# Algy/fast-slic

Measured on AMD Instinct MI355X. Metric: megapixels/sec @10 iters (1280x720 & 4K, K=1600); % HBM roofline, higher is better.
Workload: dtype u8/u16/i32 (integer SLIC); 1 GPU; 1280x720 RGB, K=1600, 10 iters (configs[1]), 8 frames/GPU; frames_per_gpu=8, global_frames=8, slots_per_gpu=6, submissions_per_launch_group=up to 2 (dynamic batching of the pipeline), inputs=device-resident uint8 RGB, device int16 labels, parallelism=frames sharded across GPUs, no collective

## Files before the change

### fast_slic_amd/_binding.py

```python
import ctypes as C
import os
import subprocess
import threading

import numpy as np

ARCH_NAME = "hip/gfx950"
_HERE = os.path.dirname(os.path.abspath(__file__))
_LIB_PATH = os.path.join(_HERE, "libfslic_hip.so")

CLUSTER_DTYPE = np.dtype([
    ("y", "<f4"), ("x", "<f4"), ("r", "<f4"), ("g", "<f4"), ("b", "<f4"), ("a", "<f4"),
    ("number", "<u2"), ("is_active", "u1"), ("is_updatable", "u1"), ("num_members", "<u4"),
])
assert CLUSTER_DTYPE.itemsize == 32

FSLIC_OK, FSLIC_E_INVALID, FSLIC_E_UNSUPPORTED, FSLIC_E_HIP, FSLIC_E_INTERNAL = range(5)


class Params(C.Structure):
    _fields_ = [
        ("max_iter", C.c_int32), ("compactness", C.c_float), ("min_size_factor", C.c_float),
        ("subsample_stride", C.c_int32), ("convert_to_lab", C.c_int32),
        ("manhattan_spatial_dist", C.c_int32), ("preemptive", C.c_int32),
        ("preemptive_thres", C.c_float), ("num_threads", C.c_int32), ("debug_mode", C.c_int32),
        ("abi", C.c_int32), ("variant", C.c_int32), ("reserved", C.c_int32 * 4),
    ]


EXPORTS = [
    "fslic_hip_device_count", "fslic_hip_create", "fslic_hip_destroy", "fslic_hip_initialize_clusters",
    "fslic_hip_iterate", "fslic_hip_iterate_device", "fslic_hip_iterate_batch", "fslic_hip_submit_group",
    "fslic_hip_wait_group", "fslic_hip_rgb_to_lab",
    "fslic_hip_enforce_connectivity", "fslic_hip_enforce_connectivity_nodes", "fslic_hip_last_prelabels", "fslic_hip_last_timing_report",
    "fslic_hip_last_device_times", "fslic_hip_set_launch_timing", "fslic_hip_last_assign_loop", "fslic_hip_last_group_frames", "fslic_hip_last_path", "fslic_hip_last_launch_mode", "fslic_hip_group_done", "fslic_hip_last_error", "fslic_hip_version",
    "fslic_hip_get_connectivity", "fslic_hip_knn_connectivity", "fslic_hip_get_mask_density", "fslic_hip_cluster_density_to_mask",
    "fslic_hip_pipeline_submit", "fslic_hip_pipeline_drain", "fslic_hip_pipeline_batching", "fslic_hip_last_host_topk_frames",
    "fslic_hip_separate_pass_redos", "fslic_hip_copy_bandwidth", "fslic_hip_last_recorder_report",
    "fslic_hip_crf_new", "fslic_hip_crf_free", "fslic_hip_crf_copy", "fslic_hip_crf_get_params", "fslic_hip_crf_set_params",
    "fslic_hip_crf_set_compat", "fslic_hip_crf_get_compat", "fslic_hip_crf_num_classes", "fslic_hip_crf_first_time",
    "fslic_hip_crf_last_time", "fslic_hip_crf_num_frames", "fslic_hip_crf_pop_frame", "fslic_hip_crf_push_frame", "fslic_hip_crf_frame",
    "fslic_hip_crf_frame_time", "fslic_hip_crf_frame_set_clusters", "fslic_hip_crf_frame_get_clusters",
    "fslic_hip_crf_frame_set_connectivity", "fslic_hip_crf_frame_set_connectivity_csr", "fslic_hip_crf_frame_get_connectivity",
    "fslic_hip_crf_frame_set_mask", "fslic_hip_crf_frame_set_proba", "fslic_hip_crf_frame_set_unbiased", "fslic_hip_crf_frame_set_unary",
    "fslic_hip_crf_frame_get_unary", "fslic_hip_crf_frame_spatial_energy", "fslic_hip_crf_frame_temporal_energy",
    "fslic_hip_crf_frame_get_inferred", "fslic_hip_crf_frame_reset_inferred", "fslic_hip_crf_initialize", "fslic_hip_crf_inference",
    "fslic_hip_crf_expf_host", "fslic_hip_crf_expf_device",
    "fslic_hip_pool_workspace_size", "fslic_hip_pool", "fslic_hip_pool_finalize", "fslic_hip_unpool",
    "fslic_hip_rag_workspace_size", "fslic_hip_rag_accumulate", "fslic_hip_rag_compact",
    "fslic_hip_crf_tensor_workspace_size", "fslic_hip_crf_tensor_inference",
    "fslic_hip_crf_tensor_grad_workspace_size", "fslic_hip_crf_tensor_inference_saved", "fslic_hip_crf_tensor_backward",
]

_lib = None
_lib_lock = threading.Lock()


def build_library(force=False):
    csrc = os.path.join(_HERE, "csrc")
    args = ["make", "-s", "-C", csrc]
    if force:
        args.append("-B")
    subprocess.check_call(args)
    return _LIB_PATH


def _preload_torch_hip_runtime():
    import importlib.util
    import sys
    if "torch" in sys.modules:
        return
    try:
        spec = importlib.util.find_spec("torch")
    except (ImportError, ValueError):
        spec = None
    if spec is None or not spec.origin:
        return
    cand = os.path.join(os.path.dirname(spec.origin), "lib", "libamdhip64.so")
    if os.path.exists(cand):
        try:
            C.CDLL(cand, mode=C.RTLD_GLOBAL)
        except OSError:
            pass


def load_library():
    global _lib
    with _lib_lock:
        if _lib is not None:
            return _lib
        _preload_torch_hip_runtime()
        if not os.path.exists(_LIB_PATH):
            raise ImportError(
                "fast_slic_amd: %s is missing; build it with `python -c 'import __graft_entry__ as g; g.build()'` "
                "or `make -C fast_slic_amd/csrc` (there is no CPU fallback)" % _LIB_PATH)
        lib = C.CDLL(os.environ.get("FSLIC_LIB") or _LIB_PATH)
        vp, i32 = C.c_void_p, C.c_int
        lib.fslic_hip_device_count.restype = i32
        lib.fslic_hip_create.argtypes = [i32, i32, C.POINTER(vp)]
        lib.fslic_hip_destroy.argtypes = [vp]
        lib.fslic_hip_destroy.restype = None
        lib.fslic_hip_initialize_clusters.argtypes = [i32, i32, i32, vp, vp]
        lib.fslic_hip_iterate.argtypes = [vp, C.POINTER(Params), i32, i32, i32, vp, vp, vp]
        lib.fslic_hip_iterate_device.argtypes = [vp, i32, C.POINTER(Params), i32, i32, i32, vp, vp, vp]
        lib.fslic_hip_iterate_batch.argtypes = [vp, C.POINTER(Params), i32, i32, i32, i32, vp, vp, vp, i32]
        lib.fslic_hip_submit_group.argtypes = [vp, i32, C.POINTER(Params), i32, i32, i32, i32, vp, vp, vp]
        lib.fslic_hip_wait_group.argtypes = [vp, i32]
        lib.fslic_hip_pipeline_submit.argtypes = [vp, C.POINTER(Params), i32, i32, i32, i32, vp, vp, vp]
        lib.fslic_hip_pipeline_drain.argtypes = [vp, C.POINTER(C.c_double), C.POINTER(C.c_longlong), C.POINTER(C.c_longlong), C.POINTER(C.c_longlong)]
        lib.fslic_hip_pipeline_batching.argtypes = [vp, i32]
        lib.fslic_hip_last_host_topk_frames.argtypes = [vp, i32]
        lib.fslic_hip_separate_pass_redos.argtypes = [vp, i32]
        if hasattr(lib, "fslic_hip_copy_bandwidth"):
            lib.fslic_hip_copy_bandwidth.argtypes = [vp, C.c_size_t, i32, C.POINTER(C.c_double)]
        lib.fslic_hip_group_done.argtypes = [vp, i32]
        lib.fslic_hip_rgb_to_lab.argtypes = [vp, i32, i32, vp, i32, vp]
        lib.fslic_hip_enforce_connectivity.argtypes = [vp, vp, i32, i32, i32, i32]
        if hasattr(lib, "fslic_hip_enforce_connectivity_nodes"):
            lib.fslic_hip_enforce_connectivity_nodes.argtypes = [vp, vp, i32, i32, i32, i32, C.POINTER(C.c_uint32)]
        lib.fslic_hip_last_prelabels.argtypes = [vp, i32, vp]
        lib.fslic_hip_last_timing_report.argtypes = [vp]
        lib.fslic_hip_last_timing_report.restype = C.c_char_p
        if hasattr(lib, "fslic_hip_last_recorder_report"):
            lib.fslic_hip_last_recorder_report.argtypes = [vp, C.POINTER(C.c_char_p), C.POINTER(C.c_size_t)]
        lib.fslic_hip_last_device_times.argtypes = [vp, i32, C.POINTER(C.c_float), C.POINTER(C.c_float)]
        lib.fslic_hip_set_launch_timing.argtypes = [vp, i32]
        lib.fslic_hip_last_assign_loop.argtypes = [vp, i32, C.POINTER(C.c_float), C.POINTER(C.c_double), C.POINTER(C.c_int)]
        lib.fslic_hip_last_group_frames.argtypes = [vp, i32]
        lib.fslic_hip_last_path.argtypes = [vp, i32]
        lib.fslic_hip_last_launch_mode.argtypes = [vp, i32]
        if hasattr(lib, "fslic_hip_lab_force_generic"):
            lib.fslic_hip_lab_force_generic.argtypes = [vp, i32]
        lib.fslic_hip_last_error.restype = C.c_char_p
        lib.fslic_hip_version.restype = C.c_char_p
        lib.fslic_hip_get_connectivity.argtypes = [vp, i32, i32, i32, vp, vp, vp]
        lib.fslic_hip_knn_connectivity.argtypes = [i32, i32, i32, vp, C.c_size_t, vp, vp]
        lib.fslic_hip_get_mask_density.argtypes = [vp, i32, i32, i32, vp, vp, vp, vp]
        lib.fslic_hip_cluster_density_to_mask.argtypes = [vp, i32, i32, i32, vp, vp, vp]
        if hasattr(lib, "fslic_hip_crf_new"):
            _declare_crf(lib)
        if hasattr(lib, "fslic_hip_pool"):
            _declare_pool(lib)
        if hasattr(lib, "fslic_hip_rag_accumulate"):
            _declare_rag(lib)
        if hasattr(lib, "fslic_hip_crf_tensor_inference"):
            _declare_crf_tensor(lib)
        _lib = lib
        return lib


def _declare_crf(lib):
    vp, i32, sz, f32 = C.c_void_p, C.c_int, C.c_size_t, C.c_float
    for name, args in [
        ("new", [sz, sz, C.POINTER(vp)]), ("copy", [vp, C.POINTER(vp)]), ("get_params", [vp, vp]), ("set_params", [vp, vp]),
        ("set_compat", [vp, i32, f32]), ("get_compat", [vp, i32, C.POINTER(f32)]), ("num_classes", [vp, C.POINTER(sz), C.POINTER(sz)]),
        ("first_time", [vp]), ("last_time", [vp]), ("pop_frame", [vp]), ("push_frame", [vp, C.POINTER(vp)]),
        ("frame", [vp, i32, C.POINTER(vp)]), ("frame_time", [vp]), ("frame_set_clusters", [vp, vp]), ("frame_get_clusters", [vp, vp]),
        ("frame_set_connectivity", [vp, i32, vp, vp, sz]), ("frame_set_connectivity_csr", [vp, i32, vp, vp]),
        ("frame_get_connectivity", [vp, vp, vp]), ("frame_set_mask", [vp, vp, f32]), ("frame_set_proba", [vp, vp]),
        ("frame_set_unbiased", [vp]), ("frame_set_unary", [vp, vp]), ("frame_get_unary", [vp, vp]),
        ("frame_spatial_energy", [vp, i32, i32, C.POINTER(f32)]), ("frame_temporal_energy", [vp, vp, i32, C.POINTER(f32)]),
        ("frame_get_inferred", [vp, vp]), ("frame_reset_inferred", [vp]), ("initialize", [vp]), ("inference", [vp, vp, sz]),
        ("expf_host", [vp, vp, sz, i32]), ("expf_device", [vp, vp, vp, sz]),
    ]:
        f = getattr(lib, "fslic_hip_crf_" + name)
        f.argtypes = args
        f.restype = i32
    lib.fslic_hip_crf_free.argtypes = [vp]
    lib.fslic_hip_crf_free.restype = None
    lib.fslic_hip_crf_num_frames.argtypes = [vp]
    lib.fslic_hip_crf_num_frames.restype = sz


def _declare_pool(lib):
    vp, i32 = C.c_void_p, C.c_int
    lib.fslic_hip_pool_workspace_size.argtypes = [i32, i32, i32, i32, C.POINTER(C.c_size_t)]
    lib.fslic_hip_pool.argtypes = [i32, vp, i32, i32, i32, i32, i32, i32, vp, vp, i32, vp, C.c_size_t]
    lib.fslic_hip_pool_finalize.argtypes = [i32, vp, i32, i32, i32, i32, vp, C.c_size_t, vp, vp, vp]
    lib.fslic_hip_unpool.argtypes = [i32, vp, i32, i32, i32, i32, i32, vp, vp, i32, vp, C.c_float, vp]
    for name in ("pool_workspace_size", "pool", "pool_finalize", "unpool"):
        getattr(lib, "fslic_hip_" + name).restype = i32


def _declare_rag(lib):
    vp, i32, i64, sz = C.c_void_p, C.c_int, C.c_longlong, C.c_size_t
    lib.fslic_hip_rag_workspace_size.argtypes = [i32, i32, i32, i64, C.POINTER(sz)]
    lib.fslic_hip_rag_accumulate.argtypes = [i32, vp, i32, i32, i32, i32, i32, vp, i32, vp, i32, i64, vp, sz]
    lib.fslic_hip_rag_compact.argtypes = [i32, vp, i32, i32, i64, vp, sz, vp, vp, vp, i64]
    for name in ("rag_workspace_size", "rag_accumulate", "rag_compact"):
        getattr(lib, "fslic_hip_" + name).restype = i32


def _declare_crf_tensor(lib):
    vp, i32, i64, sz = C.c_void_p, C.c_int, C.c_longlong, C.c_size_t
    lib.fslic_hip_crf_tensor_workspace_size.argtypes = [i32, i32, i32, i64, C.POINTER(sz)]
    lib.fslic_hip_crf_tensor_inference.argtypes = [i32, vp, i32, i32, i32, i32, i32, vp, vp, vp, vp, vp, vp, i64, vp, vp, vp, vp, sz]
    for name in ("crf_tensor_workspace_size", "crf_tensor_inference"):
        getattr(lib, "fslic_hip_" + name).restype = i32
    if hasattr(lib, "fslic_hip_crf_tensor_backward"):
        lib.fslic_hip_crf_tensor_grad_workspace_size.argtypes = [i32, i32, i32, i64, i32, i32, C.POINTER(sz)]
        lib.fslic_hip_crf_tensor_inference_saved.argtypes = lib.fslic_hip_crf_tensor_inference.argtypes
        lib.fslic_hip_crf_tensor_backward.argtypes = [i32, vp, i32, i32, i32, i32, i32, vp, vp, vp, vp, vp, vp, i64, vp, vp, vp, vp, vp, vp, vp,
                                                      vp, vp, vp, sz]
        for name in ("crf_tensor_grad_workspace_size", "crf_tensor_inference_saved", "crf_tensor_backward"):
            getattr(lib, "fslic_hip_" + name).restype = i32


def _raise(rc):
    msg = load_library().fslic_hip_last_error().decode("utf-8", "replace")
    if rc == FSLIC_E_INVALID:
        raise ValueError(msg)
    if rc == FSLIC_E_UNSUPPORTED:
        raise NotImplementedError(msg)
    raise RuntimeError(msg)


def _check(rc):
    if rc != FSLIC_OK:
        _raise(rc)


class Engine(object):

    def __init__(self, device=0, n_slots=1):
        lib = load_library()
        h = C.c_void_p()
        _check(lib.fslic_hip_create(int(device), int(n_slots), C.byref(h)))
        self._h = h
        self.device = int(device)
        self.n_slots = int(n_slots)

    def close(self):
        if getattr(self, "_h", None):
            load_library().fslic_hip_destroy(self._h)
            self._h = None

    def __del__(self):
        try:
            self.close()
        except Exception:
            pass

    def rgb_to_lab(self, image, convert=True):
        image = np.ascontiguousarray(image, dtype=np.uint8)
        H, W, ch = image.shape
        if ch != 3:
            raise ValueError("nchan != 3")
        out = np.empty((H, W, 4), np.uint8)
        _check(load_library().fslic_hip_rgb_to_lab(self._h, H, W, image.ctypes.data, int(bool(convert)), out.ctypes.data))
        return out

    def enforce_connectivity(self, labels_u16, K, min_threshold):
        out = np.ascontiguousarray(labels_u16, dtype=np.uint16).copy()
        H, W = out.shape
        _check(load_library().fslic_hip_enforce_connectivity(self._h, out.ctypes.data, H, W, int(K), int(min_threshold)))
        return out

    def enforce_connectivity_nodes(self, labels_u16, K, min_threshold):
        out = np.ascontiguousarray(labels_u16, dtype=np.uint16).copy()
        H, W = out.shape
        n = C.c_uint32(0)
        _check(load_library().fslic_hip_enforce_connectivity_nodes(self._h, out.ctypes.data, H, W, int(K), int(min_threshold), C.byref(n)))
        return out, int(n.value)

    @staticmethod
    def _plane(a, dtype):
        if isinstance(a, (int, np.integer)):
            return C.c_void_p(int(a)), None
        arr = np.ascontiguousarray(a, dtype=dtype)
        return C.c_void_p(arr.ctypes.data), arr

    def get_connectivity(self, labels, H, W, K):
        ptr, keep = self._plane(labels, np.uint16)
        num = np.zeros(K, np.int32)
        nb = np.zeros((K, 12), np.uint32)
        _check(load_library().fslic_hip_get_connectivity(self._h, H, W, int(K), ptr, num.ctypes.data, nb.ctypes.data))
        return num, nb

    def get_mask_density(self, clusters, labels, mask, H, W):
        lp, k1 = self._plane(labels, np.uint16)
        mp, k2 = self._plane(mask, np.uint8)
        cl = np.ascontiguousarray(clusters)
        dens = np.zeros(cl.shape[0], np.uint8)
        _check(load_library().fslic_hip_get_mask_density(self._h, H, W, cl.shape[0], cl.ctypes.data, lp, mp, dens.ctypes.data))
        return dens

    def cluster_density_to_mask(self, labels, densities, H, W, out=None):
        lp, k1 = self._plane(labels, np.uint16)
        d = np.ascontiguousarray(densities, dtype=np.uint8)
        if out is None:
            res = np.empty((H, W), np.uint8)
            op = C.c_void_p(res.ctypes.data)
        else:
            res, op = out, C.c_void_p(int(out))
        _check(load_library().fslic_hip_cluster_density_to_mask(self._h, H, W, d.shape[0], lp, d.ctypes.data, op))
        return res

    def iterate(self, image, clusters, params):
        H, W, _ = image.shape
        labels = np.empty((H, W), np.uint16)
        _check(load_library().fslic_hip_iterate(self._h, C.byref(params), H, W, clusters.shape[0],
                                                image.ctypes.data, clusters.ctypes.data, labels.ctypes.data))
        return labels

    def iterate_device(self, d_rgb_ptr, d_labels_ptr, H, W, clusters, params, slot=0):
        _check(load_library().fslic_hip_iterate_device(self._h, int(slot), C.byref(params), H, W, clusters.shape[0],
                                                       C.c_void_p(d_rgb_ptr), clusters.ctypes.data, C.c_void_p(d_labels_ptr)))

    def iterate_batch(self, rgb_ptrs, cluster_arrays, label_ptrs, H, W, params, device_ptrs):
        n = len(rgb_ptrs)
        K = cluster_arrays[0].shape[0]
        PA = C.c_void_p * n
        a_rgb = PA(*[C.c_void_p(int(p)) for p in rgb_ptrs])
        a_cl = PA(*[C.c_void_p(c.ctypes.data) for c in cluster_arrays])
        a_lab = PA(*[C.c_void_p(int(p)) for p in label_ptrs])
        _check(load_library().fslic_hip_iterate_batch(self._h, C.byref(params), H, W, K, n,
                                                      C.cast(a_rgb, C.c_void_p), C.cast(a_cl, C.c_void_p),
                                                      C.cast(a_lab, C.c_void_p), int(bool(device_ptrs))))

    @staticmethod
    def pointer_array(ptrs):
        PA = C.c_void_p * len(ptrs)
        return PA(*[C.c_void_p(int(p)) for p in ptrs])

    def submit_group(self, slot, a_rgb, a_clusters, a_labels, n, H, W, K, params):
        _check(load_library().fslic_hip_submit_group(self._h, int(slot), C.byref(params), H, W, K, n,
                                                     C.cast(a_rgb, C.c_void_p), C.cast(a_clusters, C.c_void_p),
                                                     C.cast(a_labels, C.c_void_p)))

    def wait_group(self, slot):
        _check(load_library().fslic_hip_wait_group(self._h, int(slot)))

    def pipeline_submit(self, a_rgb, a_clusters, a_labels, n, H, W, K, params):
        _check(load_library().fslic_hip_pipeline_submit(self._h, C.byref(params), H, W, K, n,
                                                        C.cast(a_rgb, C.c_void_p), C.cast(a_clusters, C.c_void_p),
                                                        C.cast(a_labels, C.c_void_p)))

    def pipeline_batching(self, max_frames_per_group):
        _check(load_library().fslic_hip_pipeline_batching(self._h, int(max_frames_per_group)))

    def pipeline_drain(self):
        ms, g, f, h = C.c_double(), C.c_longlong(), C.c_longlong(), C.c_longlong()
        _check(load_library().fslic_hip_pipeline_drain(self._h, C.byref(ms), C.byref(g), C.byref(f), C.byref(h)))
        return {"device_ms": ms.value, "groups": g.value, "frames": f.value, "host_topk_frames": h.value}

    def last_host_topk_frames(self, slot=0):
        return int(load_library().fslic_hip_last_host_topk_frames(self._h, int(slot)))

    def separate_pass_redos(self):
        return sum(int(load_library().fslic_hip_separate_pass_redos(self._h, s)) for s in range(self.n_slots))

    def copy_bandwidth(self, nbytes=1 << 30, reps=5):
        v = C.c_double()
        _check(load_library().fslic_hip_copy_bandwidth(self._h, C.c_size_t(int(nbytes)), int(reps), C.byref(v)))
        return v.value

    def group_done(self, slot):
        return load_library().fslic_hip_group_done(self._h, int(slot)) != 0

    def last_launch_mode(self, slot=0):
        return int(load_library().fslic_hip_last_launch_mode(self._h, int(slot)))

    def last_prelabels(self, H, W, slot=0):
        out = np.empty((H, W), np.uint16)
        _check(load_library().fslic_hip_last_prelabels(self._h, int(slot), out.ctypes.data))
        return out

    def last_timing_report(self):
        return load_library().fslic_hip_last_timing_report(self._h).decode("utf-8")

    def last_recorder_report(self):
        p, n = C.c_char_p(), C.c_size_t()
        _check(load_library().fslic_hip_last_recorder_report(self._h, C.byref(p), C.byref(n)))
        return C.string_at(p, n.value) if n.value else b""

    def last_device_times(self, slot=0):
        t, f = C.c_float(), C.c_float()
        _check(load_library().fslic_hip_last_device_times(self._h, int(slot), C.byref(t), C.byref(f)))
        return t.value, f.value

    def set_launch_timing(self, on):
        _check(load_library().fslic_hip_set_launch_timing(self._h, int(bool(on))))

    def last_assign_loop(self, slot=0):
        ms, px, n = C.c_float(), C.c_double(), C.c_int()
        _check(load_library().fslic_hip_last_assign_loop(self._h, int(slot), C.byref(ms), C.byref(px), C.byref(n)))
        return ms.value, px.value, n.value

    def last_group_frames(self, slot=0):
        return load_library().fslic_hip_last_group_frames(self._h, int(slot))

    def last_path(self, slot=0):
        return load_library().fslic_hip_last_path(self._h, int(slot))

    def lab_force_generic(self, on):
        _check(load_library().fslic_hip_lab_force_generic(self._h, int(bool(on))))


_default_engines = {}
_engine_lock = threading.Lock()


DEFAULT_ENGINE_SLOTS = 8


def default_engine(device=0):
    with _engine_lock:
        e = _default_engines.get(device)
        if e is None:
            e = Engine(device, DEFAULT_ENGINE_SLOTS)
            _default_engines[device] = e
        return e


def device_count():
    return load_library().fslic_hip_device_count()


def is_supported_arch(arch_name):
    return arch_name == ARCH_NAME


def get_supported_archs():
    return [ARCH_NAME]


def make_params(max_iter, compactness, min_size_factor, subsample_stride, convert_to_lab=True,
                manhattan_spatial_dist=True, preemptive=False, preemptive_thres=0.05, num_threads=-1,
                debug_mode=False, variant=0):
    p = Params()
    p.abi = PARAMS_ABI
    p.variant = int(variant)
    p.max_iter = int(max_iter)
    p.compactness = float(compactness)
    p.min_size_factor = float(min_size_factor)
    p.subsample_stride = int(subsample_stride)
    p.convert_to_lab = int(bool(convert_to_lab))
    p.manhattan_spatial_dist = int(bool(manhattan_spatial_dist))
    p.preemptive = int(bool(preemptive))
    p.preemptive_thres = float(preemptive_thres)
    p.num_threads = int(num_threads)
    p.debug_mode = int(bool(debug_mode))
    return p


PARAMS_ABI = 0x46533033
VARIANT_SLIC, VARIANT_LSC, VARIANT_REALDIST, VARIANT_REALDIST_L2, VARIANT_REALDIST_NOQ = 0, 1, 2, 3, 4
_REAL_DIST_VARIANTS = {"standard": VARIANT_REALDIST, "l2": VARIANT_REALDIST_L2, "noq": VARIANT_REALDIST_NOQ, "lsc": VARIANT_LSC}


class SlicModel(object):

    def __init__(self, num_components, arch_name=ARCH_NAME, real_dist=False, device=0):
        if isinstance(arch_name, bytes):
            arch_name = arch_name.decode("utf-8")
        if not is_supported_arch(arch_name):
            raise NotImplementedError("Unsupported arch " + repr(arch_name))
        if num_components >= 65534:
            raise ValueError("num_components cannot exceed 65534")
        elif num_components <= 0:
            raise ValueError("num_components should be a non-negative integer")
        self.num_components = int(num_components)
        self.num_threads = -1
        self.arch_name = arch_name
        self.real_dist = real_dist
        self.real_dist_type = "standard"
        self.convert_to_lab = False
        self.float_color = True
        self.debug_mode = False
        self.initialized = False
        self.preemptive = False
        self.preemptive_thres = 0.05
        self.manhattan_spatial_dist = True
        self.last_timing_report = ""
        self.last_recorder_report = ""
        self.device = int(device)
        self._clusters = np.zeros(self.num_components, CLUSTER_DTYPE)
        self._engine = default_engine(self.device)

    def copy(self):
        result = SlicModel(self.num_components, self.arch_name, device=self.device)
        result.real_dist = self.real_dist
        result.real_dist_type = self.real_dist_type
        result._clusters[:] = self._clusters
        result.initialized = self.initialized
        return result

    @property
    def clusters(self):
        out = []
        for c in self._clusters:
            out.append(dict(
                number=int(c["number"]),
                yx=(float(c["y"]), float(c["x"])),
                color=(float(c["r"]), float(c["g"]), float(c["b"])),
                num_members=int(c["num_members"]),
            ))
        return out

    @clusters.setter
    def clusters(self, clusters):
        n = len(clusters)
        new = np.zeros(n, CLUSTER_DTYPE)
        for i, d in enumerate(clusters):
# ... 127 lines not shown
```

### fast_slic_amd/csrc/assign.hip

```cpp
#include "device_common.h"
#include <type_traits>

namespace fslic {



template <int R, bool FUSE, bool LUT>
__global__ __launch_bounds__(256) void k_assign(FrameDev f, int rem, int stride, int Hv, int buf, int sbuf) {
    extern __shared__ uint32_t s_lut[];
    __shared__ uint32_t s_rawbuf[kWavesPerBlock][3 * 64];
    __shared__ uint4 s_listbuf[kWavesPerBlock][64];
    __shared__ uint32_t s_accbuf[FUSE ? kWavesPerBlock * kAccSlots * 6 * kAccCopies : 1];

    f.select(blockIdx.z);
    const uint32_t gen = f.generation();
    const int tid = threadIdx.x;
    const int lane = tid & 63;
    const int wave = (int)rfl((uint32_t)(tid >> 6));
    uint32_t* const s_raw = s_rawbuf[wave];
    uint4* const s_list = s_listbuf[wave];
    uint32_t* const s_acc = s_accbuf + (FUSE ? wave * (kAccSlots * 6 * kAccCopies) : 0);
    const int W = f.W, S = f.S;
    const int x0 = blockIdx.x * kTileW;
    const int x = x0 + lane;
// ... 246 lines not shown
        const int nacc = min(n, kAccSlots) * 6;
        for (int i = lane; i < nacc; i += 64) {
            uint32_t v = 0;
#pragma unroll
            for (int c = 0; c < kAccCopies; ++c) v += s_acc[i * kAccCopies + c];
            if (v) {
                const int sl = i / 6;
                atomicAdd(f.sums[0] + 6 * (size_t)s_list[sl].z + (i - sl * 6), v);
            }
        }
    }
}

typedef unsigned short us2 __attribute__((ext_vector_type(2)));

constexpr uint32_t kNoSlot = 0xFFFFFFFFu;
constexpr int kRawBuffer = 0x00020000;
constexpr int kAuxSc1 = 16;

static __device__ __forceinline__ us2 key_pair(uint32_t dist01, uint32_t idx01) {
    uint32_t r;
    asm("v_pk_mad_u16 %0, %1, 64, %2 op_sel_hi:[1,0,1] clamp" : "=v"(r) : "v"(dist01), "s"(idx01));
    return __builtin_bit_cast(us2, r);
}


static __device__ __forceinline__ unsigned long long sbitrep(uint32_t v) {
    unsigned long long r;
    asm("s_bitreplicate_b64_b32 %0, %1" : "=s"(r) : "s"(v));
    return r;
}
static __device__ __forceinline__ void min_in_place(us2& best, us2 key) {
    uint32_t b = __builtin_bit_cast(uint32_t, best);
    asm("v_pk_min_u16 %0, %0, %1" : "+v"(b) : "v"(__builtin_bit_cast(uint32_t, key)));
    best = __builtin_bit_cast(us2, b);
}

template <int R>
static __device__ __forceinline__ void row_masks(uint32_t inv, uint32_t (&m)[R / 2]) {
    static_assert(R == 8 || R == 16 || R == 32, "row masks are built for 8, 16 or 32 rows");
    if constexpr (R == 32) {
        uint32_t lo[8], hi[8];
        row_masks<16>(inv & 0xFFFFu, lo);
        row_masks<16>(inv >> 16, hi);
#pragma unroll
        for (int q = 0; q < 8; ++q) { m[q] = lo[q]; m[8 + q] = hi[q]; }
        return;
    }
    const unsigned long long r1 = sbitrep(inv);
    const unsigned long long r2 = sbitrep((uint32_t)r1);
    if (R == 8) {
        const unsigned long long r3 = sbitrep((uint32_t)r2);
        const unsigned long long a = sbitrep((uint32_t)r3), b = sbitrep((uint32_t)(r3 >> 32));
        m[0] = (uint32_t)a; m[1] = (uint32_t)(a >> 32); m[2] = (uint32_t)b; m[3] = (uint32_t)(b >> 32);
    } else {
        const unsigned long long r3a = sbitrep((uint32_t)r2), r3b = sbitrep((uint32_t)(r2 >> 32));
        const unsigned long long q0 = sbitrep((uint32_t)r3a), q1 = sbitrep((uint32_t)(r3a >> 32));
        const unsigned long long q2 = sbitrep((uint32_t)r3b), q3 = sbitrep((uint32_t)(r3b >> 32));
        m[0] = (uint32_t)q0; m[1] = (uint32_t)(q0 >> 32); m[2] = (uint32_t)q1; m[3] = (uint32_t)(q1 >> 32);
        m[R / 2 - 4] = (uint32_t)q2; m[R / 2 - 3] = (uint32_t)(q2 >> 32); m[R / 2 - 2] = (uint32_t)q3; m[R / 2 - 1] = (uint32_t)(q3 >> 32);
    }
}

#if defined(FSLIC_LAB) && FSLIC_LAB == 4
#define ASG_STAMP(i_, cond_) do { if ((cond_) && lane == 0) { asm volatile("" ::: "memory"); asg_w[(i_)] = (uint32_t)__builtin_amdgcn_s_memrealtime() - asg_t0; asm volatile("" ::: "memory"); } } while (0)
#define ASG_PUT(i_, cond_, v_) do { if ((cond_) && lane == 0) asg_w[(i_)] = (uint32_t)(v_); } while (0)
#else
#define ASG_STAMP(i_, cond_) do { } while (0)
#define ASG_PUT(i_, cond_, v_) do { } while (0)
#endif
#ifdef FSLIC_MARKS
#define ASG_MARK(name_) asm volatile("; @@MARK " name_ ::: "memory")
#else
#define ASG_MARK(name_) do { } while (0)
#endif
static __device__ __forceinline__ void lds_dma_16(const void* gsrc, uint32_t lds_byte_addr) {
    uint32_t keep;
    asm volatile("s_mov_b32 %0, m0\n\ts_mov_b32 m0, %2\n\ts_nop 0\n\tglobal_load_lds_dwordx4 %1, off\n\ts_mov_b32 m0, %0"
                 : "=&s"(keep) : "v"(gsrc), "s"(lds_byte_addr) : "memory");
}

static __device__ __forceinline__ uint32_t ld_agent(const uint32_t* p) { return __hip_atomic_load(p, __ATOMIC_RELAXED, __HIP_MEMORY_SCOPE_AGENT); }
static __device__ __forceinline__ unsigned long long ld_agent64(const void* p) {
    return __hip_atomic_load(reinterpret_cast<const unsigned long long*>(p), __ATOMIC_RELAXED, __HIP_MEMORY_SCOPE_AGENT);
}
static __device__ __forceinline__ void bin_insert_next(const FrameDev& f, uint32_t k, uint32_t yx, uint32_t lab) {
    const int y = (int)(yx >> 16), x = (int)(yx & 0xFFFFu);
    const uint32_t phase = 2u * (div_by((uint32_t)y, (uint32_t)f.T, f.T_rcp) & 1u) + (div_by((uint32_t)x, (uint32_t)f.T, f.T_rcp) & 1u);
    ClusterRec rec;
    rec.yx = yx; rec.lab = lab; rec.tag = (phase << 16) | k; rec.pad = f.generation() + 1u;
    f.cl_tag[k] = rec.tag;
    const int cell = (y >> f.cs_shift) * f.ncx + (x >> f.cs_shift);
    const uint32_t slot = atomicAdd(&f.cell_cnt[1][cell], 1u);
    if (slot < (uint32_t)kCellCap) f.cell_items[1][(size_t)cell * kCellCap + slot] = rec;
    else f.ovf_items[1][atomicAdd(f.ovf_cnt[1], 1u)] = rec;
}
static __device__ __forceinline__ void fused_finalize(const FrameDev& f, uint32_t k, uint32_t yx, uint32_t lab, uint32_t nx, uint32_t ny, uint32_t b0, uint32_t ymask) {
    uint32_t* const s0 = f.sums[0] + 6 * (size_t)k;
    uint32_t s[6];
#pragma unroll
    for (int q = 0; q < 6; ++q) s[q] = ld_agent(s0 + q);
    const char* const cp = reinterpret_cast<const char*>(f.cpart + (size_t)k * f.cpart_ns * 6);
    const uint32_t ne = nx * ny;
    const uint32_t inv_nx = (uint32_t)(65536.0f * __builtin_amdgcn_rcpf((float)nx)) + 1u;
    constexpr int kBatch = 4;
    for (uint32_t e0 = 0; e0 < ne; e0 += kBatch) {
        unsigned long long v[kBatch][3];
#pragma unroll
        for (int u = 0; u < kBatch; ++u) {
            const uint32_t e = e0 + (uint32_t)u;
            uint32_t ey = __umul24(e, inv_nx) >> 16;
            if (__umul24(ey, nx) > e) ey--;
            const uint32_t ex = e - __umul24(ey, nx);
            v[u][0] = v[u][1] = v[u][2] = 0ull;
            if (e < ne) {
                const char* p = cp + __umul24(cpart_slot((b0 >> 16) + ey, (b0 & 0xFFFFu) + ex, ymask, (uint32_t)f.nbx), 24u);
                v[u][0] = ld_agent64(p); v[u][1] = ld_agent64(p + 8); v[u][2] = ld_agent64(p + 16);
            }
        }
#pragma unroll
        for (int u = 0; u < kBatch; ++u) {
            s[0] += (uint32_t)v[u][0]; s[1] += (uint32_t)(v[u][0] >> 32); s[2] += (uint32_t)v[u][1]; s[3] += (uint32_t)(v[u][1] >> 32);
            s[4] += (uint32_t)v[u][2]; s[5] += (uint32_t)(v[u][2] >> 32);
        }
    }
    const uint32_t n = s[0];
    f.cl_n[k] = n;
    if (n != 0) {
        const uint32_t h = n >> 1, r = 0xFFFFFFFFu / n;
        int y = (int)div_by(s[1] + h, n, r), x = (int)div_by(s[2] + h, n, r);
        y = min(max(y, 0), f.H - 1);
        x = min(max(x, 0), f.W - 1);
        const uint32_t L = div_by(s[3] + h, n, r), a = div_by(s[4] + h, n, r), b = div_by(s[5] + h, n, r);
        yx = ((uint32_t)y << 16) | (uint32_t)x;
        lab = (L & 255u) | ((a & 255u) << 8) | ((b & 255u) << 16);
        f.cl_lab[k] = lab;
        f.cl_moved[k] = 1;
        f.cl_yx[k] = yx;
    }
#pragma unroll
    for (int q = 0; q < 6; ++q) s0[q] = 0u;
    f.cl_arrive[k] = 0u;
    bin_insert_next(f, k, yx, lab);
    if (n != 0 && k + 1u < (uint32_t)f.K && f.cl_shadow[k + 1u]) {
        f.cl_shadow[k + 1u] = 0u;
        bin_insert_next(f, k + 1u, f.cl_yx[k + 1u], f.cl_lab[k + 1u]);
    }
}

struct BlkMap { uint32_t gx, gy; };
static inline BlkMap blk_map(dim3 g) { BlkMap m; m.gx = g.x; m.gy = g.y; return m; }
static inline dim3 blk_grid(dim3 g) { return dim3(g.x, g.z, g.y); }

template <int R, bool FUSE, int STRIDE, bool VT, bool FBIN = false, bool PRE = false>
static __device__ __forceinline__ void assign_blk2_body(FrameDev& f, int rem, int Hv, const BlkMap& bm) {
    static_assert(!FBIN || FUSE, "the cluster pass rides on the fused centroid sums");
    static_assert(!PRE || (FUSE && !FBIN), "preemptive mode: the fused pass with its own flush");
    const uint32_t bxi = blockIdx.x, byi = blockIdx.z, bzi = blockIdx.y;
    extern __shared__ __attribute__((aligned(16))) uint32_t s_dyn[];
    __shared__ __attribute__((aligned(16))) uint4 s_raw[kWavesPerBlock][64];
    __shared__ __attribute__((aligned(16))) uint32_t s_part[64][4];
    __shared__ __attribute__((aligned(16))) uint32_t s_wcnt[4];
    __shared__ __attribute__((aligned(16))) uint32_t s_entry[FUSE ? 64 : 4];
    __shared__ __attribute__((aligned(16))) uint16_t s_klab[64];
    __shared__ __attribute__((aligned(16))) unsigned long long s_acc[FUSE ? 64 * kBlkCopies * 2 : 2];
    static_assert(R % 2 == 0, "rows are processed in pairs");
    constexpr int BH = kWavesPerBlock * R;
    static_assert(!FUSE || (BH * 64 * 255 < (1 << 20) && (BH - 1) * STRIDE * BH * 64 < (1 << 20)), "accumulator fields overflow");

    ASG_MARK("entry");
    f.select((int)bzi);
    const uint32_t gen = f.generation();
    const int tid = threadIdx.x;
    if (FBIN) {

        const uint32_t gi = (byi * bm.gx + bxi) * 256u + (uint32_t)tid;
        if (gi < (uint32_t)f.ncell) f.cell_cnt[0][gi] = 0u;
        if (gi == 0u) *f.ovf_cnt[2] = 0u;
    }
    const int lane = tid & 63;
    const int wave = (int)rfl((uint32_t)(tid >> 6));
    const int W = f.W, S = f.S;
    const int x0 = (int)bxi * kTileW;
    const int x = x0 + lane;
    const int vrow_b0 = (int)byi * BH;
    const int vrow_w0 = vrow_b0 + wave * R;
    const bool okx = x < W;
    const int nrows = (int)rfl((uint32_t)max(0, min(R, Hv - vrow_w0)));
    const int yw_lo = rem + vrow_w0 * STRIDE;
#if defined(FSLIC_LAB) && FSLIC_LAB == 4
    const uint32_t asg_t0 = (uint32_t)__builtin_amdgcn_s_memrealtime();
    volatile uint32_t* const asg_w = f.lab_stamps + ((size_t)(f.gen_off - 1u) * 2048u + (size_t)(byi * bm.gx + bxi)) * 16u;
    ASG_PUT(0, wave == 0, asg_t0);
#endif

    constexpr int kPixelLoads = R;
    uint32_t pix[R];
    auto load_pixels = [&]() {
        const uint32_t xc = (uint32_t)min(x, W - 1);
        const int nr1 = (int)rfl((uint32_t)(max(nrows, 1) - 1));
        const int ybase = (int)rfl((uint32_t)(nrows > 0 ? yw_lo : rem + (Hv - 1) * STRIDE));
        const __amdgpu_buffer_rsrc_t rs = __builtin_amdgcn_make_buffer_rsrc(const_cast<uint32_t*>(f.lab), 0, (int)((uint32_t)f.N * 4u), kRawBuffer);
        const uint32_t pitch = (uint32_t)(STRIDE * W) * 4u, soff0 = (uint32_t)ybase * (uint32_t)W * 4u;
        const int vo = (int)(xc * 4u);
        static_assert(kPixelLoads == R, "one buffer load per visited row: see the contract above");
#pragma unroll
        for (int r = 0; r < R; ++r) pix[r] = __builtin_amdgcn_raw_buffer_load_b32(rs, vo, (int)(soff0 + (uint32_t)min(r, nr1) * pitch), 0);
    };

    ASG_MARK("gather");
    const int sh = f.cs_shift;
    TileWindow win;
    {
        const int vlast = min(vrow_b0 + BH - 1, Hv - 1);
        win.wy_lo = rem + vrow_b0 * STRIDE - S; win.wy_hi = rem + vlast * STRIDE + S;
        win.wx_lo = x0 - S;                     win.wx_hi = min(x0 + kTileW - 1, W - 1) + S;
    }
    const int cxa = max(win.wx_lo, 0) >> sh, cxb = min(win.wx_hi, W - 1) >> sh;
    const int cya = max(win.wy_lo, 0) >> sh, cyb = min(win.wy_hi, f.H - 1) >> sh;
    const uint32_t ncxr = (uint32_t)(cxb - cxa + 1);
    const uint32_t nslots = ncxr * (uint32_t)(cyb - cya + 1) * (uint32_t)kCellCap;
    const uint32_t inv = (uint32_t)(65536.0f * __builtin_amdgcn_rcpf((float)ncxr)) + 1u;
    const char* const cbase = reinterpret_cast<const char*>(f.cell_items[0]);
    auto slot_ptr = [&](uint32_t e) -> const ClusterRec* {
        const uint32_t cell = e < nslots ? e >> 3 : 0u;
        uint32_t cyi = __umul24(cell, inv) >> 16;
        const uint32_t back = __umul24(cyi, ncxr);
        if (back > cell) cyi--;
        const uint32_t cxi = cell - __umul24(cyi, ncxr);
        const uint32_t off = (__umul24((uint32_t)cya + cyi, (uint32_t)f.ncx) + (uint32_t)cxa + cxi) * (uint32_t)(kCellCap * sizeof(ClusterRec)) + (e & 7u) * (uint32_t)sizeof(ClusterRec);
        return reinterpret_cast<const ClusterRec*>(cbase + off);
    };
    const ClusterRec rec0 = *slot_ptr((uint32_t)tid);
    const uint32_t novf = *f.ovf_cnt[0];
    ClusterRec rec1;
    rec1.yx = 0; rec1.lab = 0; rec1.tag = 0; rec1.pad = 0;
    if (nslots > 256u) rec1 = *slot_ptr(256u + (uint32_t)tid);
    {
        const uint32_t lds0 = (uint32_t)(size_t)(__attribute__((address_space(3))) uint32_t*)s_dyn;
        const int nq = f.tab_words >> 2, nkb = (nq + 63) >> 6;
        for (int i = wave; i < nkb; i += kWavesPerBlock)
            lds_dma_16(reinterpret_cast<const uint4*>(f.tab) + min(i * 64 + lane, nq - 1), lds0 + (uint32_t)i * 1024u);
    }
    if (FUSE) {
#pragma unroll
        for (int i = 0; i < kBlkCopies / 4; ++i) reinterpret_cast<uint4*>(s_acc)[tid + 256 * i] = make_uint4(0u, 0u, 0u, 0u);
    }
    static_assert(kBlkCopies % 4 == 0 && 64 * kBlkCopies * 2 * 8 == 256 * 16 * (kBlkCopies / 4), "16-byte stores of all threads clear the accumulators");
    load_pixels();
    {
        int cnt = 0;
        uint4* const myraw = s_raw[wave];
        auto visit = [&](const ClusterRec& rec, unsigned long long among) {
            const int cy = (int)(rec.yx >> 16), cx = (int)(rec.yx & 0xFFFFu);
            const unsigned long long m = among & ballot(cy >= win.wy_lo) & ballot(cy <= win.wy_hi) & ballot(cx >= win.wx_lo) & ballot(cx <= win.wx_hi);
            const int pos = (int)__builtin_amdgcn_mbcnt_hi((uint32_t)(m >> 32), __builtin_amdgcn_mbcnt_lo((uint32_t)m, (uint32_t)cnt));
            if (lanes(m & ballot(pos < 64))) myraw[pos] = make_uint4(rec.yx, rec.lab, rec.tag, 0u);
            cnt += __popcll(m);
        };
        auto first_lanes = [](int n) -> unsigned long long { return n >= 64 ? ~0ull : n <= 0 ? 0ull : (1ull << n) - 1ull; };
        const int w64 = wave * 64;
        visit(rec0, first_lanes((int)nslots - w64) & ballot(rec0.pad == gen));
        if (nslots > 256u) visit(rec1, first_lanes((int)nslots - 256 - w64) & ballot(rec1.pad == gen));
        for (uint32_t e0 = 512u; e0 < nslots; e0 += 256u) {
            const ClusterRec rec = *slot_ptr(e0 + (uint32_t)tid);
            visit(rec, first_lanes((int)nslots - (int)e0 - w64) & ballot(rec.pad == gen));
        }
        if (wave == kWavesPerBlock - 1) {
            const ClusterRec* __restrict__ oitems = f.ovf_items[0];
            for (uint32_t i0 = 0; i0 < novf; i0 += 64) {
                const uint32_t i = i0 + (uint32_t)lane;
                ClusterRec rec;
                rec.yx = 0; rec.lab = 0; rec.tag = 0; rec.pad = 0;
                if (i < novf) rec = oitems[i];
                visit(rec, first_lanes((int)novf - (int)i0));
            }
        }
        if (lane == 0) s_wcnt[wave] = (uint32_t)cnt;
    }
    ASG_STAMP(1, wave == 0);
    ASG_MARK("wait_table");
#if defined(FSLIC_LAB) && FSLIC_LAB == 5
    asm volatile("s_waitcnt vmcnt(0)" ::: "memory");
#else
    asm volatile("s_waitcnt vmcnt(%0)" :: "n"(kPixelLoads) : "memory");
#endif
    lds_barrier();
    ASG_STAMP(2, wave == 0);
    ASG_MARK("list_rank");
    int bn;
    uint4 mine;
    {
        const uint4 wc = *reinterpret_cast<const uint4*>(s_wcnt);
        const int c0 = (int)rfl(wc.x), c1 = (int)rfl(wc.y), c2 = (int)rfl(wc.z), c3 = (int)rfl(wc.w);
        bn = c0 + c1 + c2 + c3;
        if (bn > 64) {
            if (tid == 0) atomicOr(f.err_flag, kFlagListOverflow);
            if constexpr (!FBIN) {
                if (okx) {
                    uint16_t* rowp = f.labels + (size_t)yw_lo * W + (uint32_t)x;
                    for (int r = 0; r < nrows; ++r, rowp += (size_t)STRIDE * W)
                        if (FUSE ? f.fv_mod == 1 : f.first_visit(yw_lo + r * STRIDE)) st_stream(rowp, (uint16_t)0xFFFFu);
                }
            }
            return;
        }
        const int p1 = c0, p2 = c0 + c1, p3 = c0 + c1 + c2;
        const int idx = lane + (lane >= p1 ? 64 - c0 : 0) + (lane >= p2 ? 64 - c1 : 0) + (lane >= p3 ? 64 - c2 : 0);
        mine = (&s_raw[0][0])[lane < bn ? idx : 0];
        if (lane >= bn) mine.z = 0xFFFFFFFFu;
    }
    {
        const uint32_t tag_j = mine.z;
        uint32_t part = 0;
        for (int i = wave; i < bn; i += kWavesPerBlock) part += (uint32_t)(__builtin_amdgcn_readlane(tag_j, i) < tag_j);
        s_part[lane][wave] = part;
    }
    lds_barrier();
    uint32_t rank_j;
    {
        const uint4 pr = *reinterpret_cast<const uint4*>(s_part[lane]);
        rank_j = pr.x + pr.y + pr.z + pr.w;
    }
    if (lane < bn) s_klab[(int)rank_j] = (uint16_t)(mine.z & 0xFFFFu);
    uint32_t fin_nx = 0, fin_ny = 0, fin_b0 = 0;
    if (PRE && wave == 0) {
        if (lane < bn) s_entry[rank_j] = mine.z & 0xFFFFu;
    } else if (FUSE && wave == 0) {
        const uint32_t e1 = __umul24(mine.z & 0xFFFFu, (uint32_t)f.cpart_ns) + cpart_slot(byi, bxi, cpart_rows_mask(S, STRIDE, BH), (uint32_t)f.nbx);
        const uint32_t entry = (e1 << 2) + (e1 << 1);
        if constexpr (FBIN) {
            const SlotGeom g = slot_geom((int)(mine.x >> 16), (int)(mine.x & 0xFFFFu), S, f.H, W, rem, STRIDE, BH, Hv);
            if (lane < bn) { fin_nx = (uint32_t)(g.bx1 - g.bx0 + 1); fin_ny = (uint32_t)(g.by1 - g.by0 + 1); fin_b0 = ((uint32_t)g.by0 << 16) | (uint32_t)g.bx0; }
        }
        if (lane < bn) s_entry[rank_j] = entry;
    }
    ASG_STAMP(3, wave == 0);
    ASG_MARK("masks");

    const uint32_t yx_j = mine.x, lab_j = mine.y | (rank_j << 24);
    const int yw_hi = yw_lo + (nrows - 1) * STRIDE;
    unsigned long long todo;
    {
        const int cyj = (int)(yx_j >> 16);
        todo = nrows > 0 ? (bn >= 64 ? ~0ull : (1ull << bn) - 1ull) & ballot(cyj >= yw_lo - S) & ballot(cyj <= yw_hi + S) : 0ull;
    }

    us2 best[R / 2];
#pragma unroll
    for (int q = 0; q < R / 2; ++q) best[q] = (us2){0xFFFF, 0xFFFF};
    const uint32_t nrpad = (uint32_t)f.tab_nrpad;
    const int dyoff = f.tab_dyoff;
    if constexpr (VT) {
        const int Cc = f.tab_dyoff;
        const uint32_t xout = (uint32_t)f.tab_xout;
        constexpr int BIAS = 1024;
        static_assert(STRIDE >= 1 && STRIDE <= 3, "row-range divisions");
        auto div_stride = [](int n) -> int { return STRIDE == 1 ? n : STRIDE == 2 ? (n >> 1) : (int)(__umul24((uint32_t)n, 21846u) >> 16); };
        constexpr uint32_t full = R >= 32 ? 0xFFFFFFFFu : (1u << (R & 31)) - 1u;
        auto low_bits = [](int n) -> uint32_t { return n >= 32 ? 0xFFFFFFFFu : (1u << n) - 1u; };
        uint32_t va_j, vb_j;
        {
            const int dy0 = yw_lo - (int)(yx_j >> 16);
            const int rs = min(max(div_stride(-dy0 + STRIDE * BIAS + STRIDE - 1) - BIAS, 0), R);
            const int ra = min(max(div_stride(-S - dy0 + STRIDE * BIAS + STRIDE - 1) - BIAS, 0), R);
            const int rb = min(max(div_stride(S - dy0 + STRIDE * BIAS) - BIAS, -1), R - 1);
            const uint32_t upto_rs = low_bits(rs);
            const uint32_t in_win = rb < 0 ? 0u : (low_bits(rb + 1) & ~low_bits(ra) & full);
            va_j = in_win & upto_rs;
            vb_j = in_win & ~upto_rs;
        }
        const uint4* const s_rv = reinterpret_cast<const uint4*>(s_dyn);
        auto pass = [&](uint32_t clab, uint32_t base, uint32_t idx01, const uint32_t* mq) {
            uint32_t spw[R / 2];
            {
                const uint4 e0 = s_rv[base];
                spw[0] = e0.x; spw[1] = e0.y; spw[2] = e0.z; spw[3] = e0.w;
#pragma unroll
                for (int h = 1; h < R / 8; ++h) {
                    const uint4 e1 = s_rv[base + 8 * h * STRIDE];
                    spw[4 * h] = e1.x; spw[4 * h + 1] = e1.y; spw[4 * h + 2] = e1.z; spw[4 * h + 3] = e1.w;
                }
            }
            uint32_t t[R / 2];
#pragma unroll
            for (int q = 0; q < R / 2; ++q) {
                const uint32_t s0 = __builtin_amdgcn_sad_u8(pix[2 * q], clab, spw[q]);
                t[q] = __builtin_amdgcn_sad_hi_u8(pix[2 * q + 1], clab, s0);
            }
            us2 key[R / 2];
#pragma unroll
            for (int q = 0; q < R / 2; ++q) key[q] = key_pair(t[q], mq ? (mq[q] | idx01) : idx01);
#pragma unroll
            for (int q = 0; q < R / 2; ++q) min_in_place(best[q], key[q]);
        };
        unsigned long long todo_wa = todo & ballot(va_j == full);
        unsigned long long todo_wb = todo & ballot(vb_j == full);
        unsigned long long todo_above = todo & ballot(va_j != 0u) & ~todo_wa;
        unsigned long long todo_below = todo & ballot(vb_j != 0u) & ~todo_wb;
        auto fetch = [&](int c, uint32_t& clab, uint32_t& uxc, uint32_t& k0, uint32_t& idx01, auto clamp_tag) {
            constexpr bool CLAMP = decltype(clamp_tag)::value;
            const uint32_t cyx = __builtin_amdgcn_readlane(yx_j, c);
            const uint32_t clabx = __builtin_amdgcn_readlane(lab_j, c);
            clab = clabx & 0x00FFFFFFu;
            const int cy = (int)(cyx >> 16), cx = (int)(cyx & 0xFFFFu);
            const uint32_t ux = __builtin_amdgcn_sad_u16((uint32_t)x, (uint32_t)cx, 0u);
            uxc = CLAMP ? (ux <= (uint32_t)S ? ux : xout) : ux;
            k0 = (uint32_t)(Cc + yw_lo - cy);
            idx01 = (clabx >> 24) * 0x10001u;
        };
#pragma unroll 1
        while (todo_wa) {
            const int c = __builtin_ctzll(todo_wa);
            todo_wa &= todo_wa - 1ull;
            uint32_t clab, uxc, k0, idx01;
            fetch(c, clab, uxc, k0, idx01, std::false_type{});
            if (uxc <= (uint32_t)S) pass(clab, k0 - uxc, idx01, nullptr);
        }
#pragma unroll 1
        while (todo_wb) {
            const int c = __builtin_ctzll(todo_wb);
            todo_wb &= todo_wb - 1ull;
            uint32_t clab, uxc, k0, idx01;
            fetch(c, clab, uxc, k0, idx01, std::false_type{});
            if (uxc <= (uint32_t)S) pass(clab, k0 + uxc, idx01, nullptr);
        }
        if constexpr (R == 16 && FUSE) {
            auto pass_half = [&](auto half_tag, uint32_t clab, uint32_t base, uint32_t idx01, const uint32_t* mq4) {
                constexpr int HF = decltype(half_tag)::value;
                const uint4 e0 = s_rv[base + 8 * HF * STRIDE];
                const uint32_t spw[4] = {e0.x, e0.y, e0.z, e0.w};
                uint32_t t[4];
#pragma unroll
                for (int q = 0; q < 4; ++q) {
                    const uint32_t s0 = __builtin_amdgcn_sad_u8(pix[2 * (4 * HF + q)], clab, spw[q]);
                    t[q] = __builtin_amdgcn_sad_hi_u8(pix[2 * (4 * HF + q) + 1], clab, s0);
                }
                us2 key[4];
#pragma unroll
                for (int q = 0; q < 4; ++q) key[q] = key_pair(t[q], mq4[q] | idx01);
#pragma unroll
                for (int q = 0; q < 4; ++q) min_in_place(best[4 * HF + q], key[q]);
            };
            auto masked = [&](unsigned long long m, const uint32_t rows_j, auto sign_tag) {
                constexpr int SG = decltype(sign_tag)::value;
                unsigned long long m_lo = m & ballot((rows_j & 0xFF00u) == 0u);
                unsigned long long m_hi = m & ballot((rows_j & 0x00FFu) == 0u) & ~m_lo;
                unsigned long long m_both = m & ~m_lo & ~m_hi;
#pragma unroll 1
                while (m_lo) {
                    const int c = __builtin_ctzll(m_lo);
                    m_lo &= m_lo - 1ull;
                    uint32_t clab, uxc, k0, idx01, mq[4];
                    fetch(c, clab, uxc, k0, idx01, std::true_type{});
                    row_masks<8>(~__builtin_amdgcn_readlane(rows_j, c) & 0xFFu, mq);
                    pass_half(std::integral_constant<int, 0>{}, clab, SG < 0 ? k0 - uxc : k0 + uxc, idx01, mq);
                }
#pragma unroll 1
                while (m_hi) {
                    const int c = __builtin_ctzll(m_hi);
                    m_hi &= m_hi - 1ull;
                    uint32_t clab, uxc, k0, idx01, mq[4];
                    fetch(c, clab, uxc, k0, idx01, std::true_type{});
                    row_masks<8>(~(__builtin_amdgcn_readlane(rows_j, c) >> 8) & 0xFFu, mq);
                    pass_half(std::integral_constant<int, 1>{}, clab, SG < 0 ? k0 - uxc : k0 + uxc, idx01, mq);
                }
#pragma unroll 1
                while (m_both) {
                    const int c = __builtin_ctzll(m_both);
                    m_both &= m_both - 1ull;
                    uint32_t clab, uxc, k0, idx01, mq[R / 2];
                    fetch(c, clab, uxc, k0, idx01, std::true_type{});
                    row_masks<R>(~__builtin_amdgcn_readlane(rows_j, c) & full, mq);
                    pass(clab, SG < 0 ? k0 - uxc : k0 + uxc, idx01, mq);
                }
            };
            masked(todo_above, va_j, std::integral_constant<int, -1>{});
            masked(todo_below, vb_j, std::integral_constant<int, 1>{});
        } else {
#pragma unroll 1
            while (todo_above) {
                const int c = __builtin_ctzll(todo_above);
                todo_above &= todo_above - 1ull;
                uint32_t clab, uxc, k0, idx01, mq[R / 2];
                fetch(c, clab, uxc, k0, idx01, std::true_type{});
                row_masks<R>(~__builtin_amdgcn_readlane(va_j, c) & full, mq);
                pass(clab, k0 - uxc, idx01, mq);
            }
#pragma unroll 1
            while (todo_below) {
                const int c = __builtin_ctzll(todo_below);
                todo_below &= todo_below - 1ull;
                uint32_t clab, uxc, k0, idx01, mq[R / 2];
                fetch(c, clab, uxc, k0, idx01, std::true_type{});
                row_masks<R>(~__builtin_amdgcn_readlane(vb_j, c) & full, mq);
                pass(clab, k0 + uxc, idx01, mq);
            }
        }
    } else {
        constexpr int HQ = R / 4;
        static_assert(R % 4 == 0, "two halves of whole row pairs");
        unsigned long long todo_b, todo_u, todo_l;
        {
            const int cyj = (int)(yx_j >> 16);
            const int yh = yw_lo + (R / 2) * STRIDE;
            const unsigned long long up = todo & ballot(cyj <= yw_lo + (R / 2 - 1) * STRIDE + S);
            const unsigned long long lo = todo & ballot(cyj >= yh - S) & ballot(cyj <= yh + (R / 2 - 1) * STRIDE + S);
            todo_b = up & lo;
            todo_u = up & ~lo;
            todo_l = lo & ~up;
        }
        uint32_t pitch_v;
        asm volatile("v_mov_b32 %0, %1" : "=v"(pitch_v) : "s"(nrpad * 4u));
        const char* const tab_b = reinterpret_cast<const char*>(s_dyn);
        auto walk = [&](unsigned long long m, auto q0_tag, auto nq_tag) {
            constexpr int Q0 = decltype(q0_tag)::value, NQ = decltype(nq_tag)::value;
#pragma unroll 1
            while (m) {
                const int c = __builtin_ctzll(m);
                m &= m - 1ull;
                const uint32_t cyx = __builtin_amdgcn_readlane(yx_j, c);
                const uint32_t clabx = __builtin_amdgcn_readlane(lab_j, c);
                const uint32_t clab = clabx & 0x00FFFFFFu;
                const int cy = (int)(cyx >> 16), cx = (int)(cyx & 0xFFFFu);
                const uint32_t ux = __builtin_amdgcn_sad_u16((uint32_t)x, (uint32_t)cx, 0u);
                const uint32_t uxc = min(ux, (uint32_t)(S + 1));
                const uint32_t a0 = __umul24(uxc, pitch_v) + (uint32_t)(yw_lo - cy + dyoff) * 4u;
                const uint32_t idx01 = (clabx >> 24) * 0x10001u;
                uint32_t t[NQ];
#pragma unroll
                for (int q = 0; q < NQ; ++q) {
                    const uint32_t sp = *reinterpret_cast<const uint32_t*>(tab_b + a0 + (uint32_t)((2 * (Q0 + q)) * STRIDE * 4));
                    const uint32_t s0 = __builtin_amdgcn_sad_u8(pix[2 * (Q0 + q)], clab, sp);
                    t[q] = __builtin_amdgcn_sad_hi_u8(pix[2 * (Q0 + q) + 1], clab, s0);
                }
                us2 key[NQ];
#pragma unroll
                for (int q = 0; q < NQ; ++q) key[q] = key_pair(t[q], idx01);
#pragma unroll
                for (int q = 0; q < NQ; ++q) min_in_place(best[Q0 + q], key[q]);
            }
        };
        if constexpr (R == 16 && FUSE) {
            (void)todo_b; (void)todo_u; (void)todo_l;
            unsigned long long cov[4];
            {
                const int cyj = (int)(yx_j >> 16);
#pragma unroll
                for (int q = 0; q < 4; ++q) {
                    const int ylo = yw_lo + q * (R / 4) * STRIDE, yhi = ylo + (R / 4 - 1) * STRIDE;
                    cov[q] = todo & ballot(cyj >= ylo - S) & ballot(cyj <= yhi + S);
                }
            }
            constexpr int P = R / 8;
            auto quarters = [&](unsigned long long m, auto q0, auto nq) {
                walk(m, std::integral_constant<int, decltype(q0)::value * P>{}, std::integral_constant<int, decltype(nq)::value * P>{});
            };
            using I0 = std::integral_constant<int, 0>; using I1 = std::integral_constant<int, 1>; using I2 = std::integral_constant<int, 2>;
            using I3 = std::integral_constant<int, 3>; using I4 = std::integral_constant<int, 4>;
            quarters(cov[0] & cov[3], I0{}, I4{});
            quarters(cov[0] & cov[2] & ~cov[3], I0{}, I3{});
            quarters(cov[1] & cov[3] & ~cov[0], I1{}, I3{});
            quarters(cov[0] & cov[1] & ~cov[2], I0{}, I2{});
            quarters(cov[1] & cov[2] & ~cov[0] & ~cov[3], I1{}, I2{});
            quarters(cov[2] & cov[3] & ~cov[1], I2{}, I2{});
            quarters(cov[0] & ~cov[1], I0{}, I1{});
            quarters(cov[1] & ~cov[0] & ~cov[2], I1{}, I1{});
            quarters(cov[2] & ~cov[1] & ~cov[3], I2{}, I1{});
            quarters(cov[3] & ~cov[2], I3{}, I1{});
        } else {
            walk(todo_b, std::integral_constant<int, 0>{}, std::integral_constant<int, 2 * HQ>{});
            walk(todo_u, std::integral_constant<int, 0>{}, std::integral_constant<int, HQ>{});
            walk(todo_l, std::integral_constant<int, HQ>{}, std::integral_constant<int, HQ>{});
        }
    }

    ASG_MARK("after_walk");
    ASG_STAMP(4, wave == 0);
    ASG_PUT(9, wave == 0, __popcll(todo));
    ASG_PUT(10, wave == 0, bn);
    __builtin_amdgcn_s_waitcnt(0x0F70);
    bool epilogue_done = false;
    {
        us2 worst = best[0];
#pragma unroll
        for (int q = 1; q < R / 2; ++q) worst = __builtin_elementwise_max(worst, best[q]);
        const bool all_found = (ballot(worst.x == 0xFFFF) | ballot(worst.y == 0xFFFF)) == 0ull;
        bool fast_ok = all_found && nrows == R;
        if constexpr (PRE) fast_ok = fast_ok && rfl(f.pre_flags[0]) != 0u;
        if (fast_ok) {
            ASG_MARK("labels");
            epilogue_done = true;
            if (okx) {
                uint32_t kk[R];
                const char* const ktab = reinterpret_cast<const char*>(s_klab);
#pragma unroll
                for (int q = 0; q < R / 2; ++q) {
                    const uint32_t b = __builtin_bit_cast(uint32_t, best[q]) & 0x003F003Fu;
                    kk[2 * q] = *reinterpret_cast<const uint16_t*>(ktab + ((b & 0xFFu) << 1));
                    kk[2 * q + 1] = *reinterpret_cast<const uint16_t*>(ktab + (((b >> 16) & 0xFFu) << 1));
                }
                const __amdgpu_buffer_rsrc_t ws = __builtin_amdgcn_make_buffer_rsrc(f.labels, 0, (int)((uint32_t)f.N * 2u), kRawBuffer);
                const uint32_t so0 = (uint32_t)yw_lo * (uint32_t)W * 2u, pitch2 = (uint32_t)(STRIDE * W) * 2u;
#pragma unroll
                for (int r = 0; r < R; ++r)
                    __builtin_amdgcn_raw_buffer_store_b16((uint16_t)kk[r], ws, (int)((uint32_t)x * 2u), (int)(so0 + (uint32_t)r * pitch2), kAuxSc1);
                ASG_STAMP(5, wave == 0);
                ASG_MARK("sums");
                if (FUSE) {
                    const uint32_t copy16 = ((uint32_t)lane & (kBlkCopies - 1)) * 16u;
                    const uint32_t dyw = (uint32_t)(wave * R * STRIDE);
                    char* const accb = reinterpret_cast<char*>(s_acc);
                    uint32_t sL = 0, sa = 0, sb = 0;
                    uint32_t wq[R / 2];
#pragma unroll
                    for (int q = 0; q < R / 2; ++q) wq[q] = __builtin_bit_cast(uint32_t, best[q]) & 0x003F003Fu;
                    auto words = [&](int cnt, unsigned long long& A, unsigned long long& B) {
                        const uint32_t a_lo = sL | (sa << 20), a_hi = (sa >> 12) | (sb << 8);
                        const uint32_t ys = (uint32_t)cnt * dyw + (uint32_t)(STRIDE * (cnt * (cnt - 1) / 2));
                        const uint32_t b_lo = __umul24((uint32_t)lane, (uint32_t)cnt) + (ys << 20), b_hi = (uint32_t)cnt << 8;
                        A = (unsigned long long)a_lo | ((unsigned long long)a_hi << 32);
                        B = (unsigned long long)b_lo | ((unsigned long long)b_hi << 32);
                    };
                    unsigned long long prevA = 0ull, prevB = 0ull;
#pragma unroll
                    for (int r = 0; r < R; ++r) {
                        const uint32_t p = pix[r];
                        sL = __builtin_amdgcn_udot4(p, 0x00000001u, sL, false);
                        sa = __builtin_amdgcn_udot4(p, 0x00000100u, sa, false);
                        sb = __builtin_amdgcn_udot4(p, 0x00010000u, sb, false);
                        if (r == R - 1) break;
                        const uint32_t cur = (r & 1) ? (wq[r / 2] >> 16) : (wq[r / 2] & 0xFFFFu);
                        const uint32_t nxt = (r & 1) ? (wq[r / 2 + 1] & 0xFFFFu) : (wq[r / 2] >> 16);
#if FSLIC_EXP & 1
                        if (false) {
#else
                        if (cur != nxt) {
#endif
                            unsigned long long A, B;
                            words(r + 1, A, B);
                            unsigned long long* const run = reinterpret_cast<unsigned long long*>(accb + (cur * (uint32_t)(kBlkCopies * 16) + copy16));
                            atomicAdd(run, A - prevA);
                            atomicAdd(run + 1, B - prevB);
                            prevA = A; prevB = B;
                        }
                    }
                    {
                        unsigned long long A, B;
                        words(R, A, B);
                        unsigned long long* const last = reinterpret_cast<unsigned long long*>(accb + ((wq[R / 2 - 1] >> 16) * (uint32_t)(kBlkCopies * 16) + copy16));
                        atomicAdd(last, A - prevA);
                        atomicAdd(last + 1, B - prevB);
                    }
                }
            }
        }
    }
    ASG_MARK("slow_epilogue");
    if (!epilogue_done) {
        uint32_t slot[R];
        uint16_t* rowp = f.labels + (size_t)yw_lo * W;
        const uint32_t xo = (uint32_t)x;
#pragma unroll
        for (int r = 0; r < R; ++r) {
            const bool ok = okx && r < nrows;
            const uint32_t key = (r & 1) ? (uint32_t)best[r / 2].y : (uint32_t)best[r / 2].x;
            const bool found = key != 0xFFFFu;
            slot[r] = kNoSlot;
            if (ok && found) st_stream(rowp + xo, s_klab[key & 63u]);
            const bool unlabelled = !FBIN && ok && !found && (FUSE ? f.fv_mod == 1 : f.first_visit(yw_lo + r * STRIDE));
            if (unlabelled) st_stream(rowp + xo, (uint16_t)0xFFFFu);
            bool summed = FUSE && ok && !unlabelled;
            if constexpr (PRE) summed = summed && in_update(f, yw_lo + r * STRIDE, x);
            if (summed) {
                if (found) slot[r] = key & 63u;
                else {
                    const uint32_t old = rowp[xo];
                    if (old != 0xFFFFu) {
                        global_accumulate(f.sums[0], old, (uint32_t)(yw_lo + r * STRIDE), xo, pix[r]);
                        if (FBIN) atomicOr(f.err_flag, kFlagStalePixel);
                    }
                }
            }
            rowp += (size_t)STRIDE * W;
        }
        ASG_STAMP(5, wave == 0);
        if (FUSE) {
            const uint32_t copy = (uint32_t)lane & (kBlkCopies - 1);
            const uint32_t dyw = (uint32_t)(wave * R * STRIDE);
            uint32_t cur = slot[0], a_lo = 0, a_hi = 0, b_lo = 0, b_hi = 0;
            auto flush = [&]() {
                if (cur != kNoSlot) {
                    unsigned long long* a = s_acc + (cur * kBlkCopies + copy) * 2;
                    atomicAdd(a, (unsigned long long)a_lo | ((unsigned long long)a_hi << 32));
                    atomicAdd(a + 1, (unsigned long long)b_lo | ((unsigned long long)b_hi << 32));
                }
            };
#pragma unroll
            for (int r = 0; r < R; ++r) {
                if (r > 0 && slot[r] != cur) {
                    flush();
                    cur = slot[r]; a_lo = 0; a_hi = 0; b_lo = 0; b_hi = 0;
                }
                const uint32_t p = pix[r];
                a_lo += (p & 255u) | ((p & 0xFF00u) << 12);
                a_hi += (p >> 8) & 0xFF00u;
                b_lo += (uint32_t)lane | ((dyw + (uint32_t)(r * STRIDE)) << 20);
                b_hi += 256u;
            }
            flush();
        }
    }
    ASG_MARK("block_flush");
    if (FUSE) {
        ASG_STAMP(6, wave == 0);
        lds_barrier();
        ASG_STAMP(7, wave == 0);
        if (wave == 0 && lane < bn) {
            const uint32_t entry = s_entry[lane];
            if (entry != kNoSlot) {
                unsigned long long A = 0, B = 0;
#pragma unroll
                for (int cpy = 0; cpy < kBlkCopies; ++cpy) { A += s_acc[(lane * kBlkCopies + cpy) * 2]; B += s_acc[(lane * kBlkCopies + cpy) * 2 + 1]; }
                const uint32_t yb0 = (uint32_t)(rem + vrow_b0 * STRIDE);
                const uint32_t cnt = (uint32_t)(B >> 40);
                const uint2 q01 = make_uint2(cnt, ((uint32_t)(B >> 20) & 0xFFFFFu) + __umul24(yb0, cnt));
                const uint2 q23 = make_uint2(((uint32_t)B & 0xFFFFFu) + __umul24((uint32_t)x0, cnt), (uint32_t)A & 0xFFFFFu);
                const uint2 q45 = make_uint2((uint32_t)(A >> 20) & 0xFFFFFu, (uint32_t)(A >> 40));
                if constexpr (PRE) {
                    uint32_t* const sm = f.sums[0] + 6 * (size_t)entry;
                    if (cnt) { atomicAdd(sm, q01.x); atomicAdd(sm + 1, q01.y); atomicAdd(sm + 2, q23.x); atomicAdd(sm + 3, q23.y); atomicAdd(sm + 4, q45.x); atomicAdd(sm + 5, q45.y); }
                } else {
                    uint2* const dst = reinterpret_cast<uint2*>(f.cpart + (size_t)entry);
                    if (FBIN) { st_stream(dst, q01); st_stream(dst + 1, q23); st_stream(dst + 2, q45); }
                    else { dst[0] = q01; dst[1] = q23; dst[2] = q45; }
                }
            }
        }
        if (FBIN) {
            asm volatile("s_waitcnt vmcnt(0)" ::: "memory");
            __syncthreads();
            if (wave == 0 && fin_nx != 0u) {
                const uint32_t k = mine.z & 0xFFFFu;
                const uint32_t before = __hip_atomic_fetch_add(f.cl_arrive + k, 1u, __ATOMIC_RELAXED, __HIP_MEMORY_SCOPE_AGENT);
                if (before + 1u == fin_nx * fin_ny) fused_finalize(f, k, mine.x, mine.y, fin_nx, fin_ny, fin_b0, cpart_rows_mask(S, STRIDE, BH));
            }
        }
    }
    ASG_STAMP(8, wave == 0);
}

template <int R, bool FUSE, int STRIDE, bool VT>
__global__ __launch_bounds__(256) __attribute__((amdgpu_num_sgpr(80), amdgpu_waves_per_eu(7, 8))) void k_assign_blk2(FrameDev f, int rem, int Hv, BlkMap bm) {
    assign_blk2_body<R, FUSE, STRIDE, VT>(f, rem, Hv, bm);
}
template <int R, bool FUSE, int STRIDE, bool VT>
__global__ __launch_bounds__(256) __attribute__((amdgpu_num_sgpr(80), amdgpu_waves_per_eu(8, 8))) void k_assign_blk2_w8(FrameDev f, int rem, int Hv, BlkMap bm) {
    assign_blk2_body<R, FUSE, STRIDE, VT>(f, rem, Hv, bm);
}
template <int R, bool FUSE, int STRIDE, bool VT>
__global__ __launch_bounds__(256) __attribute__((amdgpu_num_sgpr(80), amdgpu_waves_per_eu(6, 8))) void k_assign_blk2_w6(FrameDev f, int rem, int Hv, BlkMap bm) {
    assign_blk2_body<R, FUSE, STRIDE, VT>(f, rem, Hv, bm);
}

template <int R, int STRIDE, bool VT>
__global__ __launch_bounds__(256) __attribute__((amdgpu_num_sgpr(80), amdgpu_waves_per_eu(7, 8))) void k_assign_bin(FrameDev f, int rem, int Hv, BlkMap bm) {
    assign_blk2_body<R, true, STRIDE, VT, true>(f, rem, Hv, bm);
}
template <int R, int STRIDE, bool VT>
__global__ __launch_bounds__(256) __attribute__((amdgpu_num_sgpr(80), amdgpu_waves_per_eu(6, 8))) void k_assign_bin_w6(FrameDev f, int rem, int Hv, BlkMap bm) {
    assign_blk2_body<R, true, STRIDE, VT, true>(f, rem, Hv, bm);
}

template <int R, int STRIDE, bool VT>
__global__ __launch_bounds__(256) __attribute__((amdgpu_num_sgpr(80), amdgpu_waves_per_eu(7, 8))) void k_assign_pre(FrameDev f, int rem, int Hv, BlkMap bm) {
    assign_blk2_body<R, true, STRIDE, VT, false, true>(f, rem, Hv, bm);
}

static FrameDev with_subsampled_table(FrameDev f) {
    f.tab = f.tabs; f.tab_words = f.tabs_words; f.tab_dyoff = f.tabs_dyoff; f.tab_nrpad = f.tabs_nrpad;
    return f;
}

template <int R, bool FUSE, int STRIDE>
static void launch_assign_blk_t(const FrameDev& f_, int nframes, int rem, int Hv, hipStream_t st) {
    FrameDev f = FUSE ? with_subsampled_table(f_) : f_;
    if (FUSE && R == 16 && !f.tab_vmode) { f.tab = f.tabs16; f.tab_words = f.tabs16_words; f.tab_dyoff = f.tabs16_dyoff; f.tab_nrpad = f.tabs16_nrpad; }
    if (!FUSE && R <= 16 && f.tab_vmode && f.tabv16_words > 0) { f.tab = f.tabv16; f.tab_words = f.tabv16_words; f.tab_dyoff = f.tabv16_dyoff; }
    dim3 grid((f.W + kTileW - 1) / kTileW, (Hv + kWavesPerBlock * R - 1) / (kWavesPerBlock * R), nframes);
    const size_t lds2 = ((size_t)f.tab_words * sizeof(uint32_t) + 1023) / 1024 * 1024;
    if constexpr (R == 32) {
        static_assert(!FUSE, "32 rows per wavefront: full pass only");
        launch((k_assign_blk2_w6<R, FUSE, STRIDE, true>), blk_grid(grid), dim3(256), lds2, st, f, rem, Hv, blk_map(grid));
    } else if constexpr (R == 16 && !FUSE) {
        if (f.tab_vmode) launch((k_assign_blk2_w8<R, FUSE, STRIDE, true>), blk_grid(grid), dim3(256), lds2, st, f, rem, Hv, blk_map(grid));
        else launch((k_assign_blk2_w8<R, FUSE, STRIDE, false>), blk_grid(grid), dim3(256), lds2, st, f, rem, Hv, blk_map(grid));
    } else if constexpr (R == 16 && FUSE) {
        if (f.tab_vmode) launch((k_assign_blk2_w6<R, FUSE, STRIDE, true>), blk_grid(grid), dim3(256), lds2, st, f, rem, Hv, blk_map(grid));
        else launch((k_assign_blk2_w6<R, FUSE, STRIDE, false>), blk_grid(grid), dim3(256), lds2, st, f, rem, Hv, blk_map(grid));
    } else {
        if (f.tab_vmode) launch((k_assign_blk2<R, FUSE, STRIDE, true>), blk_grid(grid), dim3(256), lds2, st, f, rem, Hv, blk_map(grid));
        else launch((k_assign_blk2<R, FUSE, STRIDE, false>), blk_grid(grid), dim3(256), lds2, st, f, rem, Hv, blk_map(grid));
    }
}

template <int R, int STRIDE>
static void launch_assign_bin_t(const FrameDev& f_, int nframes, int rem, int Hv, hipStream_t st) {
    const FrameDev f = with_subsampled_table(f_);
    dim3 grid((f.W + kTileW - 1) / kTileW, (Hv + kWavesPerBlock * R - 1) / (kWavesPerBlock * R), nframes);
    const size_t lds2 = ((size_t)f.tab_words * sizeof(uint32_t) + 1023) / 1024 * 1024;
    if constexpr (R == 16) {
        launch((k_assign_bin_w6<R, STRIDE, true>), blk_grid(grid), dim3(256), lds2, st, f, rem, Hv, blk_map(grid));
    } else if constexpr (R == 4) {
        launch((k_assign_bin<R, STRIDE, false>), blk_grid(grid), dim3(256), lds2, st, f, rem, Hv, blk_map(grid));
    } else {
        if (f.tab_vmode) launch((k_assign_bin<R, STRIDE, true>), blk_grid(grid), dim3(256), lds2, st, f, rem, Hv, blk_map(grid));
        else launch((k_assign_bin<R, STRIDE, false>), blk_grid(grid), dim3(256), lds2, st, f, rem, Hv, blk_map(grid));
    }
}

template <int STRIDE>
static void launch_assign_pre_t(const FrameDev& f_, int nframes, int rem, int Hv, hipStream_t st) {
    const FrameDev f = with_subsampled_table(f_);
    dim3 grid((f.W + kTileW - 1) / kTileW, (Hv + kWavesPerBlock * 8 - 1) / (kWavesPerBlock * 8), nframes);
    const size_t lds2 = ((size_t)f.tab_words * sizeof(uint32_t) + 1023) / 1024 * 1024;
    if (f.tab_vmode) launch((k_assign_pre<8, STRIDE, true>), blk_grid(grid), dim3(256), lds2, st, f, rem, Hv, blk_map(grid));
    else launch((k_assign_pre<8, STRIDE, false>), blk_grid(grid), dim3(256), lds2, st, f, rem, Hv, blk_map(grid));
}
bool blk_kernel_applies(const FrameDev& f, int stride) {
    return f.tab_words > 0 && stride >= 1 && stride <= 3 && (unsigned long long)f.N * 4ull < 0x7FFFFFFFull;
}

bool launch_assign_pre(const FrameDev& f_, int nframes, int rem, int stride, int buf, int sbuf, hipStream_t st) {
    const FrameDev f = rotated(f_, buf, sbuf);
    const int Hv = visited_rows(f.H, rem, stride);
    if (!blk_kernel_applies(f, stride)) return false;
    if (Hv <= 0) return true;
    if (stride == 1) launch_assign_pre_t<1>(f, nframes, rem, Hv, st);
    else if (stride == 2) launch_assign_pre_t<2>(f, nframes, rem, Hv, st);
    else launch_assign_pre_t<3>(f, nframes, rem, Hv, st);
    return true;
}

void launch_assign_fused_bin(const FrameDev& f_, int nframes, int rem, int stride, int it, hipStream_t st) {
    const FrameDev f = rotated(f_, it & 1, it & 1, it % 3);
    const int Hv = visited_rows(f.H, rem, stride);
    if (Hv <= 0) return;
    const int blocks8 = assign_blocks8(f.W, Hv, nframes);
    const bool r16 = f.tab_vmode && blocks8 > 3072;
    const bool r4 = !f.tab_vmode && stride == 3 && blocks8 <= 384;
    if (r4) {
        launch_assign_bin_t<4, 3>(f, nframes, rem, Hv, st);
    } else if (r16) {
        if (stride == 1) launch_assign_bin_t<16, 1>(f, nframes, rem, Hv, st);
        else if (stride == 2) launch_assign_bin_t<16, 2>(f, nframes, rem, Hv, st);
        else launch_assign_bin_t<16, 3>(f, nframes, rem, Hv, st);
    } else {
        if (stride == 1) launch_assign_bin_t<8, 1>(f, nframes, rem, Hv, st);
        else if (stride == 2) launch_assign_bin_t<8, 2>(f, nframes, rem, Hv, st);
        else launch_assign_bin_t<8, 3>(f, nframes, rem, Hv, st);
    }
}

static int assign_rows_per_wave(const FrameDev& f, int nframes, int Hv, bool fuse_update) {
    const int blocks8 = assign_blocks8(f.W, Hv, nframes);
    if (!fuse_update && f.tab_vmode && f.tab_rows32 && blocks8 > 4 * 6144) return 32;
    return (!fuse_update && blocks8 > 3072) ? 16 : 8;
}

template <int R>
static void launch_assign_r(const FrameDev& f, int nframes, int rem, int stride, int Hv, int buf, int sbuf, bool fuse_update, hipStream_t st) {
    dim3 grid((f.W + kTileW - 1) / kTileW, (Hv + kWavesPerBlock * R - 1) / (kWavesPerBlock * R), nframes);
    const size_t lds = (size_t)f.lut_words * sizeof(uint32_t);
    if (f.lut_words > 0) {
        if (fuse_update) launch((k_assign<R, true, true>), grid, dim3(256), lds, st, f, rem, stride, Hv, buf, sbuf);
        else launch((k_assign<R, false, true>), grid, dim3(256), lds, st, f, rem, stride, Hv, buf, sbuf);
    } else {
        if (fuse_update) launch((k_assign<R, true, false>), grid, dim3(256), 0, st, f, rem, stride, Hv, buf, sbuf);
        else launch((k_assign<R, false, false>), grid, dim3(256), 0, st, f, rem, stride, Hv, buf, sbuf);
    }
}

PassGeom launch_assign(const FrameDev& f_, int nframes, int rem, int stride, int buf, int sbuf, bool fuse_update, hipStream_t st, int obuf) {
    const FrameDev f = rotated(f_, buf, sbuf, obuf);
    const int Hv = visited_rows(f.H, rem, stride);
    PassGeom pg;
    pg.rem = rem; pg.stride = stride; pg.Hv = Hv; pg.BH = kWavesPerBlock * 8; pg.use_slots = 0;
    if (Hv <= 0) return pg;
    if (blk_kernel_applies(f, stride)) {
        if (!fuse_update && stride == 1) {
            const int rpw = assign_rows_per_wave(f, nframes, Hv, false);
            if (rpw == 32) launch_assign_blk_t<32, false, 1>(f, nframes, rem, Hv, st);
            else if (rpw == 16) launch_assign_blk_t<16, false, 1>(f, nframes, rem, Hv, st);
            else launch_assign_blk_t<8, false, 1>(f, nframes, rem, Hv, st);
            return pg;
        }
        if (fuse_update) {
            pg.use_slots = 1;
            const int fblocks8 = assign_blocks8(f.W, Hv, nframes);
            const bool r16 = (f.tab_vmode && fblocks8 > 3072) || (!f.tab_vmode && f.tabs16_words > 0 && fblocks8 > 2048);
            if (r16) {
                pg.BH = kWavesPerBlock * 16;
                if (stride == 1) launch_assign_blk_t<16, true, 1>(f, nframes, rem, Hv, st);
                else if (stride == 2) launch_assign_blk_t<16, true, 2>(f, nframes, rem, Hv, st);
                else launch_assign_blk_t<16, true, 3>(f, nframes, rem, Hv, st);
                return pg;
            }
            if (stride == 1) launch_assign_blk_t<8, true, 1>(f, nframes, rem, Hv, st);
            else if (stride == 2) launch_assign_blk_t<8, true, 2>(f, nframes, rem, Hv, st);
            else launch_assign_blk_t<8, true, 3>(f, nframes, rem, Hv, st);
            return pg;
        }
    }
    if (assign_rows_per_wave(f, nframes, Hv, fuse_update) >= 16) launch_assign_r<16>(f, nframes, rem, stride, Hv, buf, sbuf, fuse_update, st);
    else launch_assign_r<8>(f, nframes, rem, stride, Hv, buf, sbuf, fuse_update, st);
    return pg;
}

static __device__ __forceinline__ void generic_test(const ClusterRec& rec, int y, int x, int S, int P, uint32_t pix,
                                                    const uint16_t* __restrict__ patch, unsigned long long& best) {
    const int dy = y - (int)(rec.yx >> 16), dx = x - (int)(rec.yx & 0xFFFFu);
    if (dy < -S || dy > S || dx < -S || dx > S) return;
    const uint32_t sp = patch[(dy + S) * P + (dx + S)];
    const uint32_t d = (sp + __builtin_amdgcn_sad_u8(pix, rec.lab, 0u)) & 0xFFFFu;
    const unsigned long long key = ((unsigned long long)d << 32) | rec.tag;
    best = key < best ? key : best;
}

template <bool FUSE, bool REC>
static __device__ __forceinline__ void assign_generic_body(FrameDev& f, int rem, int stride, int Hv, uint16_t* __restrict__ dist) {
    f.select(blockIdx.y);
    const size_t i = (size_t)blockIdx.x * blockDim.x + threadIdx.x;
    if (i >= (size_t)Hv * f.W) return;
    const int v = (int)(i / f.W), x = (int)(i - (size_t)v * f.W);
    const int y = rem + v * stride;
    const size_t p = (size_t)y * f.W + x;
    const uint32_t pix = f.lab[p];
    const int S = f.S, P = 2 * S + 1, sh = f.cs_shift;
    unsigned long long best = ~0ull;
    const int cxa = max(x - S, 0) >> sh, cxb = min(x + S, f.W - 1) >> sh;
    const int cya = max(y - S, 0) >> sh, cyb = min(y + S, f.H - 1) >> sh;
    for (int cyi = cya; cyi <= cyb; ++cyi)
        for (int cxi = cxa; cxi <= cxb; ++cxi) {
            const int cell = cyi * f.ncx + cxi;
            const uint32_t cnt = min(f.cell_cnt[0][cell], (uint32_t)kCellCap);
            for (uint32_t s = 0; s < cnt; ++s)
                generic_test(f.cell_items[0][(size_t)cell * kCellCap + s], y, x, S, P, pix, f.patch2d, best);
        }
    const uint32_t novf = *f.ovf_cnt[0];
    for (uint32_t s = 0; s < novf; ++s) generic_test(f.ovf_items[0][s], y, x, S, P, pix, f.patch2d, best);
    uint32_t lbl;
    if (best != ~0ull) { lbl = (uint32_t)(best & 0xFFFFull); f.labels[p] = (uint16_t)lbl; }
    else lbl = f.labels[p];
    if (REC) dist[p] = best != ~0ull ? (uint16_t)(best >> 32) : (uint16_t)0xFFFFu;
    if (FUSE && lbl != 0xFFFFu && (!f.cell_act || f.pre_flags[0] || f.cell_act[(y / (2 * S)) * f.pre_cw + x / (2 * S)]))
        global_accumulate(f.sums[0], lbl, (uint32_t)y, (uint32_t)x, pix);
}

template <bool FUSE>
__global__ __launch_bounds__(256) void k_assign_generic(FrameDev f, int rem, int stride, int Hv, int buf, int sbuf) {
    assign_generic_body<FUSE, false>(f, rem, stride, Hv, nullptr);
}
__global__ __launch_bounds__(256) void k_assign_generic_rec(FrameDev f, int rem, int stride, int Hv, uint16_t* dist) {
    assign_generic_body<true, true>(f, rem, stride, Hv, dist);
}

void launch_assign_generic(const FrameDev& f_, int nframes, int rem, int stride, int buf, int sbuf, bool fuse_update, hipStream_t st, uint16_t* rec_dist) {
    const FrameDev f = rotated(f_, buf, sbuf);
    const int Hv = visited_rows(f.H, rem, stride);
    if (Hv <= 0) return;
    const size_t n = (size_t)Hv * f.W;
    const int blocks = (int)((n + 255) / 256);
    if (rec_dist) launch(k_assign_generic_rec, dim3(blocks, 1), dim3(256), 0, st, f, rem, stride, Hv, rec_dist);
    else if (fuse_update) launch(k_assign_generic<true>, dim3(blocks, nframes), dim3(256), 0, st, f, rem, stride, Hv, buf, sbuf);
    else launch(k_assign_generic<false>, dim3(blocks, nframes), dim3(256), 0, st, f, rem, stride, Hv, buf, sbuf);
}

}
```

### fast_slic_amd/csrc/capi.cpp

```cpp
#include "engine_internal.h"
#include "crf.h"

#include <algorithm>
#include <cstdio>
#include <cstdlib>
#include <cstring>
#include <mutex>

using namespace fslic;

static_assert(sizeof(fslic_cluster) == 32, "Cluster ABI (src/fast-slic-common.h:10-23)");

extern "C" {

const char* fslic_hip_last_error(void) { return last_error().c_str(); }
const char* fslic_hip_version(void) { return "fast_slic_amd 0.3 (gfx950)"; }

int fslic_hip_device_count(void) {
    int n = 0;
    if (hipGetDeviceCount(&n) != hipSuccess) return 0;
    return n;
}

int fslic_hip_create(int device, int n_slots, fslic_engine** out) {
// ... 100 lines not shown
    const std::string& r = thread_recorder_report();
    *report = r.c_str();
    *length = r.size();
    return FSLIC_OK;
}

int fslic_hip_iterate_batch(fslic_engine* e, const fslic_params* p, int H, int W, int K, int n_frames,
                            const uint8_t* const* rgb, fslic_cluster* const* clusters,
                            uint16_t* const* labels, int device_ptrs) {
    if (!e) return fail(FSLIC_E_INVALID, "engine is NULL");
    if (n_frames < 0 || (n_frames > 0 && (!rgb || !clusters || !labels))) return fail(FSLIC_E_INVALID, "bad batch arguments");
    HIPCHK(hipSetDevice(e->device));
    const int ns = (int)e->slots.size();
    const size_t N = (size_t)H * W;
    int S = 0;
    int rc = validate(p, H, W, K, S);
    if (rc) return rc;
    int G = std::min(std::max(e->group_size, 1), (int)kMaxGroup);
    if (n_frames < G * ns) G = std::max(1, (n_frames + ns - 1) / ns);
    std::vector<GroupJob> jobs((size_t)(n_frames + G - 1) / G);
    for (size_t g = 0; g < jobs.size(); g++) {
        const int first = (int)g * G;
        if ((rc = fill_job(jobs[g], p, H, W, K, std::min(G, n_frames - first), rgb + first, clusters + first, labels + first)) || (rc = check_job(jobs[g], S))) return rc;
    }
    rc = acquire_all_slots(e);
    if (rc) return rc;
    struct Pending { int slot, first, n; };
    std::vector<Pending> inflight;
    auto finish_one = [&](const Pending& pd) -> int {
        Slot& s = e->slots[pd.slot];
        int r = group_finish(e, s);
        if (r) return r;
        if (!device_ptrs) {
            for (int i = 0; i < pd.n; i++)
                HIPCHK(hipMemcpyAsync(labels[pd.first + i], s.at(s.d_out_stage, i), N * 2, hipMemcpyDeviceToHost, s.st));
            HIPCHK(hipStreamSynchronize(s.st));
        }
        return FSLIC_OK;
    };
    auto bail = [&](int code) -> int {
        for (const Pending& pd : inflight) drain_failed(e->slots[pd.slot]);
        release_all_slots(e);
        return code;
    };
    int next_slot = 0;
    for (int first = 0; first < n_frames; first += G) {
        const int n = std::min(G, n_frames - first);
        const int si = next_slot;
        next_slot = (next_slot + 1) % ns;
        for (size_t q = 0; q < inflight.size(); q++)
            if (inflight[q].slot == si) {
                const Pending pd = inflight[q];
                inflight.erase(inflight.begin() + q);
                rc = finish_one(pd);
                if (rc) return bail(rc);
                break;
            }
        Slot& s = e->slots[si];
        GroupJob& job = jobs[(size_t)(first / G)];
        if (!device_ptrs) {
            rc = ensure_prepared(e, s, H, W, K, S, n);
            if (rc) return bail(rc);
            for (int i = 0; i < n; i++) {
                if (hipMemcpyAsync(s.at(s.d_rgb_stage, i), rgb[first + i], N * 3, hipMemcpyHostToDevice, s.st) != hipSuccess)
                    return bail(fail(FSLIC_E_HIP, "frame upload failed"));
                job.d_rgb[i] = s.at(s.d_rgb_stage, i);
                job.d_out[i] = s.at(s.d_out_stage, i);
            }
        }
        s.launch_timing = e->launch_timing;
        inflight.push_back({si, first, n});
        rc = group_begin(e, s, job);
        if (rc) return bail(rc);
    }
    while (!inflight.empty()) {
        const Pending pd = inflight.front();
        inflight.erase(inflight.begin());
        rc = finish_one(pd);
        if (rc) return bail(rc);
    }
    if (n_frames > 0) set_thread_timing_report(make_timing_report(e->slots[0]));
    release_all_slots(e);
    return FSLIC_OK;
}

int fslic_hip_last_prelabels(fslic_engine* e, int slot, uint16_t* prelabels) {
    if (!e || !prelabels) return fail(FSLIC_E_INVALID, "NULL pointer argument");
    if (slot < 0 || slot >= (int)e->slots.size()) return fail(FSLIC_E_INVALID, "slot out of range");
    HIPCHK(hipSetDevice(e->device));
    SlotLease lease(e);
    int rc = lease.take(slot);
    if (rc) return rc;
    Slot& s = e->slots[slot];
    if (!s.have_pre || s.keyH == 0) return fail(FSLIC_E_INVALID, "no frame has been processed on this slot");
    HIPCHK(hipMemcpy(prelabels, s.f.labels, (size_t)s.f.N * 2, hipMemcpyDeviceToHost));
    return FSLIC_OK;
}

const char* fslic_hip_last_timing_report(fslic_engine* e) { return e ? thread_timing_report().c_str() : ""; }

int fslic_hip_last_device_times(fslic_engine* e, int slot, float* total_ms, float* full_assign_ms) {
    if (!e || slot < 0 || slot >= (int)e->slots.size()) return fail(FSLIC_E_INVALID, "bad engine/slot");
    if (total_ms) *total_ms = e->slots[slot].total_ms;
    if (full_assign_ms) *full_assign_ms = e->slots[slot].fa_ms;
    return FSLIC_OK;
}

int fslic_hip_set_launch_timing(fslic_engine* e, int on) {
    if (!e) return fail(FSLIC_E_INVALID, "engine is NULL");
    e->launch_timing = on != 0;
    return FSLIC_OK;
}

int fslic_hip_lab_force_generic(fslic_engine* e, int on) {
    if (!e) return fail(FSLIC_E_INVALID, "engine is NULL");
    e->lab_force_generic.store(on != 0);
    return FSLIC_OK;
}

int fslic_hip_last_assign_loop(fslic_engine* e, int slot, float* sum_ms, double* visited_px, int* launches) {
    if (!e || slot < 0 || slot >= (int)e->slots.size()) return fail(FSLIC_E_INVALID, "bad engine/slot");
    const Slot& s = e->slots[slot];
    if (sum_ms) *sum_ms = s.assign_loop_ms;
    if (visited_px) *visited_px = s.assign_loop_px;
    if (launches) *launches = s.n_timed_iters;
    return FSLIC_OK;
}

int fslic_hip_last_group_frames(fslic_engine* e, int slot) {
    if (!e || slot < 0 || slot >= (int)e->slots.size()) return -1;
    return e->slots[slot].nframes;
}

int fslic_hip_last_launch_mode(fslic_engine* e, int slot) {
    if (!e || slot < 0 || slot >= (int)e->slots.size()) return -1;
    return e->slots[slot].last_launch_mode;
}

int fslic_hip_last_path(fslic_engine* e, int slot) {
    if (!e || slot < 0 || slot >= (int)e->slots.size()) return -1;
    return e->slots[slot].last_path;
}

int fslic_hip_last_host_topk_frames(fslic_engine* e, int slot) {
    if (!e || slot < 0 || slot >= (int)e->slots.size()) return -1;
    return e->slots[slot].n_host_topk;
}

int fslic_hip_separate_pass_redos(fslic_engine* e, int slot) {
    if (!e || slot < 0 || slot >= (int)e->slots.size()) return -1;
    return __atomic_load_n(&e->slots[slot].n_separate_redo, __ATOMIC_RELAXED);
}

#define CRF_LOCK(crf) std::lock_guard<std::mutex> crf_lock__((crf)->mu)

static fslic_crf_frame* crf_frame_at(fslic_crf* crf, int time) {
    if (crf->frames.empty()) return nullptr;
    const long long d = (long long)time - crf->frames.front()->time;
    if (d < 0 || d >= (long long)crf->frames.size()) return nullptr;
    return crf->frames[(size_t)d].get();
}
static void crf_touch_unary(fslic_crf_frame* f) { f->dirty_unary = true; }
static void crf_touch_q(fslic_crf_frame* f) { f->q_on_device = false; f->dirty_q = true; }

int fslic_hip_crf_new(size_t num_classes, size_t num_nodes, fslic_crf** out) {
    if (!out) return fail(FSLIC_E_INVALID, "out is NULL");
    *out = nullptr;
    if (num_classes == 0 || num_nodes == 0) return fail(FSLIC_E_INVALID, "num_classes and num_nodes must be positive");
    if (num_classes >= (1ull << 31) || num_nodes >= (1ull << 31) || (unsigned long long)num_classes * num_nodes >= (1ull << 31))
        return fail(FSLIC_E_INVALID, "num_classes * num_nodes must be below 2^31");
    fslic_crf* crf = new fslic_crf();
    crf->C = num_classes;
    crf->K = num_nodes;
    crf->compat.assign(num_classes, 1.0f);
    crf->params.spatial_w = 10; crf->params.temporal_w = 10;
    crf->params.spatial_srgb = 13; crf->params.temporal_srgb = 13;
    crf->params.spatial_sxy = 80;
    crf->params.spatial_smooth_w = 0; crf->params.spatial_smooth_sxy = 3;
    *out = crf;
    return FSLIC_OK;
}

void fslic_hip_crf_free(fslic_crf* crf) {
    if (!crf) return;
    crf_release_device(crf);
    delete crf;
}

int fslic_hip_crf_copy(fslic_crf* crf, fslic_crf** out) {
    if (!crf || !out) return fail(FSLIC_E_INVALID, "NULL pointer argument");
    *out = nullptr;
    CRF_LOCK(crf);
    for (auto& f : crf->frames) {
        int rc = crf_pull_q(crf, f.get());
        if (rc) return rc;
    }
    fslic_crf* c = new fslic_crf();
    c->C = crf->C; c->K = crf->K; c->next_time = crf->next_time; c->compat = crf->compat; c->params = crf->params;
    for (auto& f : crf->frames) {
        std::unique_ptr<fslic_crf_frame> g(new fslic_crf_frame());
        g->parent = c; g->time = f->time; g->clusters = f->clusters; g->edges = f->edges; g->unaries = f->unaries; g->q = f->q;
        c->frames.push_back(std::move(g));
    }
    *out = c;
    return FSLIC_OK;
}

int fslic_hip_crf_get_params(fslic_crf* crf, fslic_crf_params* out) {
    if (!crf || !out) return fail(FSLIC_E_INVALID, "NULL pointer argument");
    CRF_LOCK(crf);
    *out = crf->params;
    return FSLIC_OK;
}

int fslic_hip_crf_set_params(fslic_crf* crf, const fslic_crf_params* params) {
    if (!crf || !params) return fail(FSLIC_E_INVALID, "NULL pointer argument");
    CRF_LOCK(crf);
    crf->params = *params;
    return FSLIC_OK;
}

int fslic_hip_crf_set_compat(fslic_crf* crf, int cls, float compat_value) {
    if (!crf) return fail(FSLIC_E_INVALID, "NULL pointer argument");
    CRF_LOCK(crf);
    if (cls < 0 || (size_t)cls >= crf->C) return fail(FSLIC_E_INVALID, "class out of range");
    crf->compat[(size_t)cls] = compat_value;
    return FSLIC_OK;
}

int fslic_hip_crf_get_compat(fslic_crf* crf, int cls, float* out) {
    if (!crf || !out) return fail(FSLIC_E_INVALID, "NULL pointer argument");
    CRF_LOCK(crf);
    if (cls < 0 || (size_t)cls >= crf->C) return fail(FSLIC_E_INVALID, "class out of range");
    *out = crf->compat[(size_t)cls];
    return FSLIC_OK;
}

int fslic_hip_crf_num_classes(fslic_crf* crf, size_t* num_classes, size_t* num_nodes) {
    if (!crf) return fail(FSLIC_E_INVALID, "NULL pointer argument");
    if (num_classes) *num_classes = crf->C;
    if (num_nodes) *num_nodes = crf->K;
    return FSLIC_OK;
}

int fslic_hip_crf_first_time(fslic_crf* crf) {
    if (!crf) return -1;
    CRF_LOCK(crf);
    return crf->frames.empty() ? -1 : crf->frames.front()->time;
}

int fslic_hip_crf_last_time(fslic_crf* crf) {
    if (!crf) return -1;
    CRF_LOCK(crf);
    return crf->frames.empty() ? -1 : crf->frames.back()->time;
}

size_t fslic_hip_crf_num_frames(fslic_crf* crf) {
    if (!crf) return 0;
    CRF_LOCK(crf);
    return crf->frames.size();
}

int fslic_hip_crf_pop_frame(fslic_crf* crf) {
    if (!crf) return -1;
    CRF_LOCK(crf);
    if (crf->frames.empty()) return -1;
    const int t = crf->frames.front()->time;
    crf->frames.pop_front();
    return t;
}

int fslic_hip_crf_push_frame(fslic_crf* crf, fslic_crf_frame** out) {
    if (!crf || !out) return fail(FSLIC_E_INVALID, "NULL pointer argument");
    *out = nullptr;
    CRF_LOCK(crf);
    if (crf->next_time == INT32_MAX) return fail(FSLIC_E_INVALID, "frame times exhausted");
    std::unique_ptr<fslic_crf_frame> f(new fslic_crf_frame());
    f->parent = crf;
    f->time = crf->next_time++;
    fslic_cluster one{};
    one.num_members = 1;
    f->clusters.assign(crf->K, one);
    f->edges.resize(crf->K);
    f->unaries.assign(crf->C * crf->K, 0.0f);
    f->q.assign(crf->C * crf->K, 0.0f);
    *out = f.get();
    crf->frames.push_back(std::move(f));
    return FSLIC_OK;
}

int fslic_hip_crf_frame(fslic_crf* crf, int time, fslic_crf_frame** out) {
    if (!crf || !out) return fail(FSLIC_E_INVALID, "NULL pointer argument");
    CRF_LOCK(crf);
    *out = crf_frame_at(crf, time);
    if (!*out) return fail(FSLIC_E_INVALID, "Time out of range");
    return FSLIC_OK;
}

int fslic_hip_crf_frame_time(fslic_crf_frame* frame) { return frame ? frame->time : -1; }

int fslic_hip_crf_frame_set_clusters(fslic_crf_frame* frame, const fslic_cluster* clusters) {
    if (!frame || !clusters) return fail(FSLIC_E_INVALID, "NULL pointer argument");
    CRF_LOCK(frame->parent);
    std::copy(clusters, clusters + frame->clusters.size(), frame->clusters.begin());
    frame->dirty_graph = true;
    return FSLIC_OK;
// ... 196 lines not shown
```

### fast_slic_amd/csrc/engine_internal.h

```cpp
#pragma once
#include "kernels.h"
#include "launch.h"
#include "../../include/fslic_hip.h"

#include <algorithm>
#include <atomic>
#include <condition_variable>
#include <deque>
#include <cstdint>
#include <memory>
#include <mutex>
#include <string>
#include <thread>
#include <vector>

namespace fslic {

int fail(int code, const std::string& msg);
const std::string& last_error();
void set_last_error(const std::string& msg);

#define HIPCHK(expr)                                                                            \
    do {                                                                                        \
        hipError_t e__ = (expr);                                                                \
        if (e__ != hipSuccess)                                                                  \
            return ::fslic::fail(FSLIC_E_HIP, std::string(#expr) + ": " + hipGetErrorString(e__)); \
    } while (0)

inline int clampi(int v, int lo, int hi) { return v < lo ? lo : (v > hi ? hi : v); }
inline float clampf(float v, float lo, float hi) { return v < lo ? lo : (v > hi ? hi : v); }
inline size_t align_up(size_t v, size_t a) { return (v + a - 1) / a * a; }
double now_us();

template <class T, bool kDevice>
class Buffer {
    T* p_ = nullptr;
    size_t cap_ = 0;
public:
    Buffer() = default;
    Buffer(Buffer&& o) noexcept : p_(o.p_), cap_(o.cap_) { o.p_ = nullptr; o.cap_ = 0; }
    Buffer& operator=(Buffer&& o) noexcept { std::swap(p_, o.p_); std::swap(cap_, o.cap_); return *this; }
    ~Buffer() { release(); }
    operator T*() const { return p_; }
    T* get() const { return p_; }
    void release() {
        if (p_) (void)(kDevice ? hipFree(p_) : hipHostFree(p_));
        p_ = nullptr; cap_ = 0;
    }
    int reserve(size_t count) {
        if (p_ && cap_ >= count) return FSLIC_OK;
        release();
        const size_t bytes = std::max<size_t>(count * sizeof(T), 16);
        const hipError_t err = kDevice ? hipMalloc((void**)&p_, bytes) : hipHostMalloc((void**)&p_, bytes);
        if (err != hipSuccess) {
            p_ = nullptr;
            return fail(FSLIC_E_HIP, std::string(kDevice ? "hipMalloc(" : "hipHostMalloc(") + std::to_string(bytes) + " bytes): " + hipGetErrorString(err));
        }
        cap_ = count;
        return FSLIC_OK;
    }
};
template <class T> using Pinned = Buffer<T, false>;
template <class T> using Device = Buffer<T, true>;

struct GroupJob {
    fslic_params p{};
    int H = 0, W = 0, K = 0, n = 0;
    const uint8_t* d_rgb[kMaxGroup] = {};
    fslic_cluster* clusters[kMaxGroup] = {};
    uint16_t* d_out[kMaxGroup] = {};
    void append(const GroupJob& j) {
        for (int i = 0; i < j.n; i++) { d_rgb[n + i] = j.d_rgb[i]; clusters[n + i] = j.clusters[i]; d_out[n + i] = j.d_out[i]; }
        n += j.n;
    }
};

struct Knobs {
    int group_size;
    bool use_graphs, poison, host_timing;
    int fuse_bin;
};
const Knobs& knobs();

constexpr int kDenseCap = 8192;
constexpr size_t kTabMaxBytes = 40960;
constexpr size_t kLutMaxWords = 12288;

struct HostTables {
    uint16_t gamma[256];
    uint16_t lab[8194];
    int cb[9];
};
const HostTables& host_tables();

struct Slot {
    hipStream_t st = nullptr;
    hipEvent_t ev[6] = {nullptr, nullptr, nullptr, nullptr, nullptr, nullptr};
    static constexpr int kMaxTimedIters = 16;
    hipEvent_t ev_it[2 * kMaxTimedIters] = {};
    int n_timed_iters = 0;
    float assign_loop_ms = 0;
    double assign_loop_px = 0;
    Device<char> arena;
    int cap_frames = 0;
    size_t frame_bytes = 0;
    FrameDev f{};
    CcaDev c{};
    char* zero_block = nullptr;
    size_t zero_bytes = 0;
    char* stamp_block = nullptr;
    size_t stamp_bytes = 0;
    uint32_t* d_misc = nullptr;
    uint32_t* d_yx_alt[2] = {nullptr, nullptr};
    uint8_t* d_rgb_stage = nullptr;
    uint16_t* d_out_stage = nullptr;
    int32_t* d_keep_leader = nullptr;
    uint16_t* d_keep_label = nullptr;
    Device<void*> d_ptrs;
    Pinned<void*> h_ptrs;
    uint16_t* d_patch = nullptr;
    uint32_t* d_lut = nullptr;
    Pinned<uint32_t> h_lut;
    uint16_t* d_tab = nullptr;
    Pinned<uint16_t> h_tab;
    Pinned<uint32_t> h_cl;
    Pinned<uint32_t> h_misc;
    Pinned<uint16_t> h_patch;
    Pinned<int32_t> h_cand_leader;
    Pinned<uint32_t> h_cand_area;
    Device<uint32_t> d_gen;
    uint64_t gen_host = 0;
    uint32_t gen_span_prev = 0;
    uint32_t gen_step = 0;
    int keyH = 0, keyW = 0, keyK = 0;
    struct GraphEntry {
        std::vector<unsigned char> key;
        hipGraph_t graph = nullptr;
        hipGraphExec_t exec = nullptr;
        int seen = 0;
        bool failed = false;
    };
    std::vector<GraphEntry> graphs;
    int last_launch_mode = 0;
    bool launch_timing = false;
    double t_begun_us = 0;
    bool nap_wait = false;
    double recent_wait_us[4] = {1e30, 1e30, 1e30, 1e30};
    unsigned recent_wait_i = 0;
    unsigned long long recent_wait_key = 0;
    int H = 0, W = 0, K = 0, S = 0;
    int nframes = 0;
    bool generic = false;
    fslic_params p{};
    fslic_cluster* clusters[kMaxGroup] = {};
    float total_ms = 0, fa_ms = 0, lab_ms = 0, loop_ms = 0, cca_ms = 0;
    int last_path = 0;
    int n_host_topk = 0;
    int n_separate_redo = 0;
    bool have_pre = false;
    bool busy = false;
    bool pending = false;
    int wanted = 0;
    struct Async {
        std::thread worker;
        bool has_job = false, done = false, quit = false;
        GroupJob job;
        int rc = 0;
        std::string err;
        bool from_queue = false;
        int jobs = 0;
    };
    std::unique_ptr<Async> async;
    uint32_t* d_pre = nullptr;
    Pinned<uint32_t> h_upd;
    float* d_clf = nullptr;
    Pinned<float> h_clf;
    float* d_patchf = nullptr;
    Pinned<float> h_patchf;
    int pf_S = 0, pf_shift = -1, pf_variant = -1;
    float pf_compactness = -1.0f;
    bool pf_manhattan = true;
    Device<char> lsc_arena;
    size_t lsc_frame_bytes = 0, lsc_zero_bytes = 0;
    char* lsc_zero = nullptr;
    LscDev l{};
    Pinned<float> h_lsc_lut;
    int lsc_H = 0, lsc_W = 0, lsc_K = 0, lsc_G = 0, lsc_S = 0;
    float lsc_compactness = -1.0f;
    bool sp_valid = false, sp_tiled_ok = false, sp_manhattan = true, sp_patch_uploaded = false;
    int sp_S = 0, sp_shift = 0, sp_stride = 0;
    float sp_compactness = 0.0f;
    bool recording = false;
    Device<char> d_rec;
    std::vector<fslic_cluster> rec_clusters;

    template <class T> T* at(T* p, int frame) const { return reinterpret_cast<T*>(reinterpret_cast<char*>(p) + (size_t)frame * frame_bytes); }
};

inline uint32_t* status(const Slot& s, int frame) { return s.h_misc + (size_t)kStatusWords * frame; }

inline void cluster_position(bool moved, uint32_t yx, const float* centroid, const fslic_cluster& in, int H, int W, float& y, float& x) {
    if (moved && centroid) { y = centroid[0]; x = centroid[1]; }
    else if (moved) { y = (float)(yx >> 16); x = (float)(yx & 0xFFFFu); }
    else { x = clampf(in.x, 0.0f, (float)(W - 1)); y = clampf(in.y, 0.0f, (float)(H - 1)); }
}

}

struct fslic_engine {
    int device = 0;
    int group_size = 8;
    bool launch_timing = false;
    std::vector<fslic::Slot> slots;
    fslic::Device<uint16_t> d_gamma, d_labtbl;
    fslic::LabTables tables{};
    std::mutex mu;
    std::condition_variable cv;
    std::condition_variable cv_work;
    int pipe_rc = 0;
    std::string pipe_err;
    double pipe_device_ms = 0;
    long long pipe_groups = 0, pipe_frames = 0, pipe_host_topk = 0;
    std::deque<fslic::GroupJob> pipe_q;
    int pipe_inflight = 0;
    int pipe_batch_frames = 0;
    bool pipe_gathering = false;
    double pipe_last_submit_us = 0;
    std::atomic<int> reserve_frames{0};
    int sync_waiters = 0;
    std::atomic<int> lab_force_generic{0};
};

extern "C" int fslic_hip_lab_force_generic(fslic_engine* e, int on);

namespace fslic {

int configure_spatial(Slot& s, int S, const fslic_params* p);
int configure_patchf(Slot& s, int S, const fslic_params* p);

void free_slot(Slot& s);
int prepare(fslic_engine* e, Slot& s, int H, int W, int K, int S, int G);
int ensure_prepared(fslic_engine* e, Slot& s, int H, int W, int K, int S, int G);
int prepare_lsc(Slot& s, int H, int W, int K, int S, int G, float compactness);

int validate(const fslic_params* p, int H, int W, int K, int& S);
int fill_job(GroupJob& j, const fslic_params* p, int H, int W, int K, int n,
             const uint8_t* const* d_rgb, fslic_cluster* const* clusters, uint16_t* const* d_out);
int check_job(const GroupJob& j, int& S);
int upload_ptrs(Slot& s, int n, const uint8_t* const* d_rgb, uint16_t* const* d_out);
CcaDev cca_view(const Slot& s, int i0, const uint16_t* d_in0, size_t in_stride, int K, int min_threshold);
void cca_enqueue(Slot& s, const CcaDev& c, int i0, int n, const ExportDev* ex = nullptr);
int cca_finish_group(Slot& s, int first, int n, const uint16_t* d_in0, size_t in_stride, int K, int thres);
int group_begin(fslic_engine* e, Slot& s, const GroupJob& job, bool record = false);
int group_finish(fslic_engine* e, Slot& s);
void drain_failed(Slot& s);
int run_group(fslic_engine* e, Slot& s, const GroupJob& job, bool record = false);
std::string make_timing_report(const Slot& s);
void set_thread_timing_report(const std::string& json);
const std::string& thread_timing_report();
int make_recorder_report(Slot& s, std::string& out);
void set_thread_recorder_report(std::string&& json);
const std::string& thread_recorder_report();

int acquire_slot(fslic_engine* e, int want, int& slot);
int acquire_all_slots(fslic_engine* e);
void release_slot(fslic_engine* e, int slot);
void release_all_slots(fslic_engine* e);
void stop_slot_thread(fslic_engine* e, Slot& s);
struct SlotLease {
    fslic_engine* e;
    int slot = -1;
    explicit SlotLease(fslic_engine* e_) : e(e_) {}
    int take(int want = -1) { return acquire_slot(e, want, slot); }
    ~SlotLease() { if (slot >= 0) release_slot(e, slot); }
};

}
```

### fast_slic_amd/csrc/group.cpp

```cpp
#include "engine_internal.h"

#include <time.h>

#include <algorithm>
#include <charconv>
#include <chrono>
#include <cmath>
#include <cstdio>
#include <cstring>
#include <numeric>

namespace fslic {

double now_us() {
    return std::chrono::duration<double, std::micro>(std::chrono::steady_clock::now().time_since_epoch()).count();
}

int validate(const fslic_params* p, int H, int W, int K, int& S) {
    if (!p) return fail(FSLIC_E_INVALID, "params is NULL");
    static_assert(sizeof(fslic_params) == 64 && offsetof(fslic_params, abi) == 40 && offsetof(fslic_params, variant) == 44, "fslic_params layout (include/fslic_hip.h)");
    if (p->abi != FSLIC_PARAMS_ABI) return fail(FSLIC_E_INVALID, "fslic_params.abi != FSLIC_PARAMS_ABI: the caller was built against another layout of the struct (include/fslic_hip.h)");
    if (p->reserved[0] | p->reserved[1] | p->reserved[2] | p->reserved[3]) return fail(FSLIC_E_INVALID, "fslic_params.reserved must be 0");
    if (H <= 0 || W <= 0) return fail(FSLIC_E_INVALID, "H and W must be positive");
    if (H > 32767 || W > 32767) return fail(FSLIC_E_INVALID, "H and W must fit int16 (src/context.cpp:262)");
// ... 15 lines not shown
    if (!p) return fail(FSLIC_E_INVALID, "params is NULL");
    j.p = *p; j.H = H; j.W = W; j.K = K; j.n = n;
    for (int i = 0; i < n; i++) { j.d_rgb[i] = d_rgb[i]; j.clusters[i] = clusters[i]; j.d_out[i] = d_out[i]; }
    return FSLIC_OK;
}

int check_job(const GroupJob& j, int& S) {
    if (j.n < 1 || j.n > (int)kMaxGroup) return fail(FSLIC_E_INVALID, "bad group arguments");
    const int rc = validate(&j.p, j.H, j.W, j.K, S);
    if (rc) return rc;
    for (int i = 0; i < j.n; i++)
        if (!j.clusters[i] || !j.d_rgb[i] || !j.d_out[i]) return fail(FSLIC_E_INVALID, "NULL pointer argument");
    return FSLIC_OK;
}

void select_kept_sorted(const int32_t* leader, const uint32_t* area, uint32_t M, int K,
                        int32_t* keep_leader, uint16_t* keep_label, uint32_t& n_keep) {
    if ((size_t)K >= (size_t)M) {
        for (uint32_t i = 0; i < M; i++) { keep_leader[i] = leader[i]; keep_label[i] = (uint16_t)i; }
        n_keep = M;
        return;
    }
    std::vector<uint32_t> order(M);
    std::iota(order.begin(), order.end(), 0u);
    auto by_area = [&](uint32_t a, uint32_t b) { return area[a] > area[b]; };
    std::partial_sort(order.begin(), order.begin() + K, order.end(), by_area);
    std::vector<uint8_t> kept(M, 0);
    for (int i = 0; i < K; i++) kept[order[i]] = 1;
    uint32_t n = 0;
    for (uint32_t i = 0; i < M; i++)
        if (kept[i]) { keep_leader[n] = leader[i]; keep_label[n] = (uint16_t)n; n++; }
    n_keep = n;
}

CcaDev cca_view(const Slot& s, int i0, const uint16_t* d_in0, size_t in_stride, int K, int min_threshold) {
    CcaDev c = s.c;
    c.in = d_in0; c.in_stride = in_stride; c.K = K; c.min_threshold = min_threshold;
    c.outs = nullptr;
    c.out = nullptr;
    FrameDev::adv(c.in, (size_t)i0 * in_stride);
    const size_t d = (size_t)i0 * c.frame_bytes;
    FrameDev::adv(c.lid, d); FrameDev::adv(c.nrec, d); FrameDev::adv(c.narea, d);
    FrameDev::adv(c.nfinal, d); FrameDev::adv(c.vedge, d); FrameDev::adv(c.roots, d);
    FrameDev::adv(c.counters, d);
    FrameDev::adv(c.cand_leader, d); FrameDev::adv(c.cand_area, d);
    c.outs = reinterpret_cast<uint16_t* const*>(s.d_ptrs + kMaxGroup + i0);
    return c;
}

int upload_ptrs(Slot& s, int n, const uint8_t* const* d_rgb, uint16_t* const* d_out) {
    for (int i = 0; i < kMaxGroup; i++) {
        s.h_ptrs[i] = (i < n && d_rgb) ? const_cast<uint8_t*>(d_rgb[i]) : nullptr;
        s.h_ptrs[kMaxGroup + i] = (i < n && d_out) ? d_out[i] : nullptr;
    }
    HIPCHK(hipMemcpyAsync(s.d_ptrs, s.h_ptrs, sizeof(void*) * 2 * kMaxGroup, hipMemcpyHostToDevice, s.st));
    return FSLIC_OK;
}

void cca_enqueue(Slot& s, const CcaDev& c, int i0, int n, const ExportDev* ex) {
    (void)i0;
    launch_cca_phase1(c, n, s.st);
    launch_cca_select(c, n, s.st);
    launch_cca_phase2(c, n, s.st, ex);
}

int cca_finish_group(Slot& s, int first, int n, const uint16_t* d_in0, size_t in_stride, int K, int thres) {
    int n_slow = 0;
    for (int i = first; i < first + n; i++) n_slow += status(s, i)[kStSelect] == kSelectHost;
    if (n_slow == 0) return FSLIC_OK;
    for (int i = first; i < first + n && n_slow; i++) {
        const uint32_t* hm = status(s, i);
        if (hm[kStSelect] != kSelectHost) continue;
        const CcaDev c1 = cca_view(s, i, d_in0, in_stride, K, thres);
        int32_t* d_dl = s.at(s.c.cand_leader, i);
        uint32_t* d_da = s.at(s.c.cand_area, i);
        const uint32_t M = hm[kStCands];
        const size_t cap = std::max<size_t>((size_t)M * 2, 16384);
        int rc;
        if ((rc = s.h_cand_leader.reserve(cap)) || (rc = s.h_cand_area.reserve(cap))) return rc;
        launch_cca_gather_area(c1, s.st);
        HIPCHK(hipMemcpyAsync(s.h_cand_leader, d_dl, sizeof(int32_t) * M, hipMemcpyDeviceToHost, s.st));
        HIPCHK(hipMemcpyAsync(s.h_cand_area, d_da, sizeof(uint32_t) * M, hipMemcpyDeviceToHost, s.st));
        HIPCHK(hipStreamSynchronize(s.st));
        std::vector<uint32_t> order(M);
        std::iota(order.begin(), order.end(), 0u);
        std::sort(order.begin(), order.end(), [&](uint32_t a, uint32_t b) { return s.h_cand_leader[a] < s.h_cand_leader[b]; });
        int32_t* sl = s.h_cand_leader + M;
        uint32_t* sa = s.h_cand_area + M;
        for (uint32_t q = 0; q < M; q++) { sl[q] = s.h_cand_leader[order[q]]; sa[q] = s.h_cand_area[order[q]]; }
        int32_t* kl = s.h_cand_leader;
        uint16_t* kb = reinterpret_cast<uint16_t*>(s.h_cand_area.get());
        uint32_t n_keep = 0;
        select_kept_sorted(sl, sa, M, K, kl, kb, n_keep);
        int32_t* d_kl = s.at(s.d_keep_leader, i);
        uint16_t* d_kb = s.at(s.d_keep_label, i);
        if (n_keep) {
            HIPCHK(hipMemcpyAsync(d_kl, kl, sizeof(int32_t) * n_keep, hipMemcpyHostToDevice, s.st));
            HIPCHK(hipMemcpyAsync(d_kb, kb, sizeof(uint16_t) * n_keep, hipMemcpyHostToDevice, s.st));
        }
        launch_cca_set_kept(c1, d_kl, d_kb, (int)n_keep, s.st);
        launch_cca_phase2(c1, 1, s.st);
    }
    HIPCHK(hipStreamSynchronize(s.st));
    return FSLIC_OK;
}

void stage_group(fslic_engine* e, Slot& s, int i0, int n, bool timed) {
    const int H = s.H, W = s.W, K = s.K;
    for (int z = 0; z < n; z++) {
        const fslic_cluster* cl = s.clusters[i0 + z];
        uint32_t* h = s.h_cl + (size_t)(i0 + z) * 4 * K;
        for (int k = 0; k < K; k++) {
            const int y = clampi((int)cl[k].y, 0, H - 1), x = clampi((int)cl[k].x, 0, W - 1);
            h[k] = ((uint32_t)y << 16) | (uint32_t)x;
        }
    }
    if (s.p.variant == FSLIC_VARIANT_REALDIST_NOQ) {
        for (int z = 0; z < n; z++) {
            const fslic_cluster* cl = s.clusters[i0 + z];
            float* h = s.h_clf + (size_t)(i0 + z) * 8 * K;
            for (int k = 0; k < K; k++) {
                h[8 * k + 0] = clampf(cl[k].y, 0.0f, (float)(H - 1));
                h[8 * k + 1] = clampf(cl[k].x, 0.0f, (float)(W - 1));
                for (int q = 2; q < 8; q++) h[8 * k + q] = 0.0f;
            }
        }
    }
    if (timed) {
        s.n_timed_iters = 0; s.assign_loop_px = 0;
        const int stride = s.p.subsample_stride;
        int rem = 0;
        for (int it = 0; it < s.p.max_iter && s.launch_timing && it < Slot::kMaxTimedIters; it++) {
            s.n_timed_iters = it + 1;
            s.assign_loop_px += (double)visited_rows(H, rem, stride) * W * n;
            rem = (rem + 1) % stride;
        }
    }
}

static bool cluster_pass_fused(const FrameDev& f, const fslic_params& p, int n, int W, int H, bool generic, bool separate_cluster_pass) {
    const int stride = p.subsample_stride;
    const int assign_blocks = assign_blocks8(W, visited_rows(H, 0, stride), n);
#if defined(FSLIC_LAB) && FSLIC_LAB == 3
    const bool fuse_wanted = false;
    (void)assign_blocks;
#else
    const bool fuse_wanted = knobs().fuse_bin == 2 || (knobs().fuse_bin == 1 && assign_blocks <= 640);
#endif
    const bool plain_slic = p.variant == FSLIC_VARIANT_SLIC && p.preemptive == 0;
    const bool every_pass_has_rows = H >= stride;
    return fuse_wanted && !separate_cluster_pass && plain_slic && !generic && every_pass_has_rows && blk_kernel_applies(f, stride);
}

static int min_size_threshold(const Slot& s) { return (int)round((double)(s.S * s.S) * (double)s.p.min_size_factor); }

constexpr int kRecWords = 16;
struct RecLayout {
    size_t N, K, nsnap, dsize, dist_off, cl_off, bytes;
};
static RecLayout rec_layout(const Slot& s) {
    RecLayout L{};
    L.N = (size_t)s.H * s.W; L.K = (size_t)s.K; L.nsnap = (size_t)s.p.max_iter + 1;
    L.dsize = s.p.variant == FSLIC_VARIANT_SLIC ? 2 : 4;
    auto up = [](size_t v) { return (v + 255) & ~(size_t)255; };
    L.dist_off = up(L.nsnap * L.N * 2);
    L.cl_off = L.dist_off + up(L.nsnap * L.N * L.dsize);
    L.bytes = L.cl_off + up(L.nsnap * kRecWords * L.K * 4);
    return L;
}

int enqueue_frames(fslic_engine* e, Slot& s, int i0, int n, bool generic, bool timed, bool separate_cluster_pass = false) {
    const fslic_params* p = &s.p;
    const int K = s.K, S = s.S;
    FrameDev f = s.f;
    f.rgbs = nullptr;
    f.select(i0);
    f.rgbs = reinterpret_cast<const uint8_t* const*>(s.d_ptrs + i0);
    const size_t fb = s.frame_bytes;

    const bool need_patch = generic || (p->preemptive != 0 && p->variant == FSLIC_VARIANT_SLIC && !blk_kernel_applies(f, p->subsample_stride));
    if ((p->preemptive != 0 || p->variant == FSLIC_VARIANT_REALDIST_NOQ || (need_patch && !s.sp_patch_uploaded)) && recording_unsupported()) return FSLIC_OK;
    if (need_patch && !s.sp_patch_uploaded) {
        HIPCHK(hipMemcpyAsync(s.d_patch, s.h_patch, (size_t)(2 * S + 1) * (2 * S + 1) * sizeof(uint16_t), hipMemcpyHostToDevice, s.st));
        s.sp_patch_uploaded = true;
    }
    const bool pre = p->preemptive != 0;
    if (pre) {
        uint32_t* base = s.at(s.d_pre, i0);
        f.cl_upd = base; f.cl_act = base + K; f.cell_act = base + 2 * (size_t)K; f.pre_flags = f.cell_act + (size_t)f.pre_cw * f.pre_ch;
        for (int z = 0; z < n; z++) {
            uint32_t* bz = s.at(s.d_pre, i0 + z);
            HIPCHK(hipMemsetD32Async((hipDeviceptr_t)bz, 2, (size_t)K, s.st));
            HIPCHK(hipMemsetD32Async((hipDeviceptr_t)(bz + 2 * (size_t)K + (size_t)f.pre_cw * f.pre_ch), 1, 1, s.st));
        }
    }
    const bool noq = p->variant == FSLIC_VARIANT_REALDIST_NOQ;
    if (noq) {
        f.cl_f = s.at(s.d_clf, i0);
        HIPCHK(hipMemcpy2DAsync(f.cl_f, fb, s.h_clf + (size_t)i0 * 8 * K, sizeof(float) * 8 * (size_t)K,
                                sizeof(float) * 8 * (size_t)K, (size_t)n, hipMemcpyHostToDevice, s.st));
    }

    if (timed) HIPCHK(hipEventRecord(s.ev[0], s.st));
    f.gen_base = s.d_gen;
    const bool fusebin = cluster_pass_fused(f, *p, n, s.W, s.H, generic, separate_cluster_pass);
    const bool lazy_labels = p->variant == FSLIC_VARIANT_SLIC && !generic && p->preemptive == 0 && !fusebin;
    launch_rgb_to_lab(f, n, p->convert_to_lab, e->tables, !lazy_labels, s.st, s.gen_step,
                      s.at(s.zero_block, i0), s.zero_bytes, f.cl_n, 2 * (size_t)K, s.h_cl + (size_t)i0 * 4 * K, 4 * (size_t)K);
    if (timed) HIPCHK(hipEventRecord(s.ev[1], s.st));
    f.gen_off = 1;
    PassGeom pg{};
    uint32_t* const yx_up = f.cl_yx;
    uint32_t* const yx_a = yx_up + 6 * (size_t)K;
    uint32_t* const yx_b = yx_up + 7 * (size_t)K;
    f.cl_yx = yx_up; f.cl_yx_out = yx_a;
    const int stride = p->subsample_stride;
    const bool lsc = p->variant == FSLIC_VARIANT_LSC;
    launch_bin_clusters(f, n, 0, 0, 0, pg, s.st);
    uint32_t* yx_cur = yx_a;
    int rem = 0;
    LscDev l = s.l;
    if (lsc) {
        l.select(i0);
        HIPCHK(clear_rows(s.lsc_zero + (size_t)i0 * s.lsc_frame_bytes, s.lsc_frame_bytes, s.lsc_zero_bytes, (size_t)n, s.st));
        launch_lsc_prepare(f, l, n, s.st);
    }
    const bool rec = s.recording && n == 1;
    const RecLayout rl = rec ? rec_layout(s) : RecLayout{};
    auto rec_dist = [&](int idx) -> void* { return rec ? s.d_rec + rl.dist_off + (size_t)idx * rl.N * rl.dsize : nullptr; };
    auto snapshot = [&](int idx, const uint32_t* yx) -> int {
        HIPCHK(hipMemcpyAsync(s.d_rec + (size_t)idx * rl.N * 2, f.labels, rl.N * 2, hipMemcpyDeviceToDevice, s.st));
        uint32_t* c = reinterpret_cast<uint32_t*>(s.d_rec + rl.cl_off) + (size_t)idx * kRecWords * K;
        const size_t kb = sizeof(uint32_t) * (size_t)K;
        HIPCHK(hipMemcpyAsync(c, yx, kb, hipMemcpyDeviceToDevice, s.st));
        HIPCHK(hipMemcpyAsync(c + K, f.cl_lab, kb, hipMemcpyDeviceToDevice, s.st));
        HIPCHK(hipMemcpyAsync(c + 2 * (size_t)K, f.cl_n, kb, hipMemcpyDeviceToDevice, s.st));
        HIPCHK(hipMemcpyAsync(c + 3 * (size_t)K, f.cl_moved, kb, hipMemcpyDeviceToDevice, s.st));
        if (pre) {
            HIPCHK(hipMemcpyAsync(c + 4 * (size_t)K, f.cl_upd, kb, hipMemcpyDeviceToDevice, s.st));
            HIPCHK(hipMemcpyAsync(c + 5 * (size_t)K, f.cl_act, kb, hipMemcpyDeviceToDevice, s.st));
        }
        if (noq) HIPCHK(hipMemcpyAsync(c + 6 * (size_t)K, f.cl_f, 8 * kb, hipMemcpyDeviceToDevice, s.st));
        return FSLIC_OK;
    };
    if (rec) {
        HIPCHK(hipMemsetAsync(s.d_rec + rl.dist_off, 0, rl.N * rl.dsize, s.st));
        if (p->max_iter > 0) {
            if (rl.dsize == 2) HIPCHK(hipMemsetAsync(rec_dist(1), 0xFF, (size_t)p->max_iter * rl.N * 2, s.st));
            else HIPCHK(hipMemsetD32Async((hipDeviceptr_t)rec_dist(1), 0x7F7FFFFFu, (size_t)p->max_iter * rl.N, s.st));
        }
        HIPCHK(hipMemsetAsync(s.d_rec + rl.cl_off, 0, rl.nsnap * kRecWords * rl.K * 4, s.st));
        const int rc = snapshot(0, yx_up);
        if (rc) return rc;
    }
    const bool rd = p->variant == FSLIC_VARIANT_REALDIST || p->variant == FSLIC_VARIANT_REALDIST_L2 || noq;
    const bool rd_l2 = p->variant == FSLIC_VARIANT_REALDIST_L2;
    float noq_coef = 1.0f / ((float)S / p->compactness);
    noq_coef *= (1 << (p->convert_to_lab ? 1 : 0));
    const bool noq_manhattan = p->manhattan_spatial_dist != 0;
    const float pre_l1_thres = std::max(roundf(2 * S * p->preemptive_thres), 1.0f);
    for (int it = 0; rd && it < p->max_iter; it++) {
        const bool tme = timed && s.launch_timing && it < Slot::kMaxTimedIters;
        f.cl_yx = yx_cur; f.cl_yx_out = (yx_cur == yx_a) ? yx_b : yx_a;
        if (tme) HIPCHK(hipEventRecord(s.ev_it[2 * it], s.st));
        float* const dist = static_cast<float*>(rec_dist(it + 1));
        if (noq) launch_noq_assign(f, noq_coef, noq_manhattan, n, rem, stride, it & 1, it & 1, true, s.st, dist);
        else launch_rd_assign(f, s.d_patchf, rd_l2, n, rem, stride, it & 1, it & 1, true, s.st, dist);
        if (tme) HIPCHK(hipEventRecord(s.ev_it[2 * it + 1], s.st));
        launch_member_sums(f, n, rem, stride, it & 1, noq ? 1 : 0, s.st);
        f.gen_off++;
        pg = PassGeom{};
        if (pre) launch_preempt_update(f, n, (it + 1) & 1, it & 1, false, pre_l1_thres, s.st);
        else launch_bin_clusters(f, n, 1, (it + 1) & 1, it & 1, pg, s.st);
        yx_cur = f.cl_yx_out;
        if (rec) { const int rc = snapshot(it + 1, yx_cur); if (rc) return rc; }
        rem = (rem + 1) % stride;
    }
    for (int it = 0; lsc && it < p->max_iter; it++) {
        const bool tme = timed && s.launch_timing && it < Slot::kMaxTimedIters;
        f.cl_yx = yx_cur; f.cl_yx_out = (yx_cur == yx_a) ? yx_b : yx_a;
        if (tme) HIPCHK(hipEventRecord(s.ev_it[2 * it], s.st));
        launch_lsc_assign(f, l, n, rem, stride, it & 1, it & 1, !pre, s.st, static_cast<float*>(rec_dist(it + 1)));
        if (tme) HIPCHK(hipEventRecord(s.ev_it[2 * it + 1], s.st));
        if (pre) {
            launch_lsc_pre_sums(f, n, rem, stride, it & 1, s.st);
            f.gen_off++;
            launch_preempt_update(f, n, (it + 1) & 1, it & 1, false, pre_l1_thres, s.st);
            launch_lsc_pre_feats(f, l, n, rem, stride, s.st);
        } else {
            f.gen_off++;
            pg = PassGeom{};
            launch_bin_clusters_lsc(f, l, n, (it + 1) & 1, it & 1, s.st);
        }
        yx_cur = f.cl_yx_out;
        if (rec) { const int rc = snapshot(it + 1, yx_cur); if (rc) return rc; }
        rem = (rem + 1) % stride;
    }
    int full_obuf = -1;
    for (int it = 0; fusebin && it < p->max_iter; it++) {
        const bool tme = timed && s.launch_timing && it < Slot::kMaxTimedIters;
        f.cl_yx = yx_a; f.cl_yx_out = yx_a;
        f.fv_mod = lazy_labels && it < stride ? 1 : 0; f.fv_from = 0;
        if (tme) HIPCHK(hipEventRecord(s.ev_it[2 * it], s.st));
        launch_assign_fused_bin(f, n, rem, stride, it, s.st);
        if (tme) HIPCHK(hipEventRecord(s.ev_it[2 * it + 1], s.st));
        f.gen_off++;
        yx_cur = yx_a;
        rem = (rem + 1) % stride;
        full_obuf = (it + 1) % 3;
    }
    if (fusebin && full_obuf < 0) full_obuf = 0;
    for (int it = 0; !fusebin && !lsc && !rd && it < p->max_iter; it++) {
        pg = PassGeom{};
        const bool tme = timed && s.launch_timing && it < Slot::kMaxTimedIters;
        if (tme) HIPCHK(hipEventRecord(s.ev_it[2 * it], s.st));
        f.fv_mod = lazy_labels && it < stride ? 1 : 0; f.fv_from = 0;
        if (rec) launch_assign_generic(f, n, rem, stride, it & 1, it & 1, true, s.st, static_cast<uint16_t*>(rec_dist(it + 1)));
        else if (generic || (pre && !launch_assign_pre(f, n, rem, stride, it & 1, it & 1, s.st))) launch_assign_generic(f, n, rem, stride, it & 1, it & 1, true, s.st);
        else if (!pre) pg = launch_assign(f, n, rem, stride, it & 1, it & 1, true, s.st);
        if (tme) HIPCHK(hipEventRecord(s.ev_it[2 * it + 1], s.st));
        f.gen_off++;
        f.cl_yx = yx_cur; f.cl_yx_out = (yx_cur == yx_a) ? yx_b : yx_a;
        if (pre) launch_preempt_update(f, n, (it + 1) & 1, it & 1, false, pre_l1_thres, s.st);
        else launch_bin_clusters(f, n, 1, (it + 1) & 1, it & 1, pg, s.st);
        yx_cur = f.cl_yx_out;
        if (rec) { const int rc = snapshot(it + 1, yx_cur); if (rc) return rc; }
        rem = (rem + 1) % stride;
    }
    int full_buf = p->max_iter & 1;
    if (pre) {
        f.gen_off++;
        f.cl_yx = yx_cur;
        launch_preempt_update(f, n, (p->max_iter + 1) & 1, 0, true, pre_l1_thres, s.st);
        full_buf = (p->max_iter + 1) & 1;
    }
    if (timed) HIPCHK(hipEventRecord(s.ev[2], s.st));
    f.fv_mod = lazy_labels && p->max_iter < stride ? stride : 0; f.fv_from = p->max_iter < stride ? std::max(p->max_iter, 0) : 0;
    f.fv_rcp = f.fv_mod > 1 ? 0xFFFFFFFFu / (uint32_t)f.fv_mod : 0u;
    if (lsc) { f.cl_yx = yx_cur; launch_lsc_assign(f, l, n, 0, 1, full_buf, 0, false, s.st); }
    else if (noq) { f.cl_yx = yx_cur; launch_noq_assign(f, noq_coef, noq_manhattan, n, 0, 1, full_buf, 0, false, s.st); }
    else if (rd) { f.cl_yx = yx_cur; launch_rd_assign(f, s.d_patchf, rd_l2, n, 0, 1, full_buf, 0, false, s.st); }
    else if (generic) launch_assign_generic(f, n, 0, 1, full_buf, 0, false, s.st);
    else (void)launch_assign(f, n, 0, 1, full_buf, 0, false, s.st, full_obuf);
    if (timed) HIPCHK(hipEventRecord(s.ev[3], s.st));
    const CcaDev c = cca_view(s, i0, s.f.labels, fb, K, min_size_threshold(s));
    ExportDev ex{};
    ex.frame_bytes = fb; ex.K = K; ex.yx_cur = yx_cur; ex.lab_n_moved = yx_up + K; ex.misc0 = s.at(s.d_misc, i0);
    ex.h_cl = s.h_cl + (size_t)i0 * 4 * K; ex.h_stride = 4 * (size_t)K; ex.h_misc = status(s, i0);
    cca_enqueue(s, c, i0, n, &ex);
    if (timed) HIPCHK(hipEventRecord(s.ev[4], s.st));
    if (pre) HIPCHK(hipMemcpy2DAsync(s.h_upd + (size_t)i0 * K, sizeof(uint32_t) * (size_t)K, f.cl_upd, fb,
                                     sizeof(uint32_t) * (size_t)K, (size_t)n, hipMemcpyDeviceToHost, s.st));
    if (noq) HIPCHK(hipMemcpy2DAsync(s.h_clf + (size_t)i0 * 8 * K, sizeof(float) * 8 * (size_t)K, f.cl_f, fb,
                                     sizeof(float) * 8 * (size_t)K, (size_t)n, hipMemcpyDeviceToHost, s.st));
    return FSLIC_OK;
}

GraphRecorder*& current_recorder() {
    static thread_local GraphRecorder* rec = nullptr;
    return rec;
}

int launch_group(fslic_engine* e, Slot& s, int n) {
    s.last_launch_mode = 0;
    {
        const uint64_t span = (uint64_t)s.p.max_iter + 3u;
        if (s.gen_host + 2 * (s.gen_span_prev + span) >= 0xC0000000ull) {
            HIPCHK(hipMemsetAsync(s.d_gen, 0, 256, s.st));
            HIPCHK(hipMemset2DAsync(s.stamp_block, s.frame_bytes, 0, s.stamp_bytes, (size_t)s.cap_frames, s.st));
            s.gen_host = 0;
        }
        s.gen_step = s.gen_span_prev ? s.gen_span_prev : (uint32_t)span;
        s.gen_span_prev = (uint32_t)span;
        s.gen_host += s.gen_step;
    }
    if (s.recording) return enqueue_frames(e, s, 0, n, s.generic, true, true);
    if (!knobs().use_graphs || s.launch_timing) return enqueue_frames(e, s, 0, n, s.generic, true);
    std::vector<unsigned char> key;
    auto put = [&](const void* p, size_t bytes) { const unsigned char* b = (const unsigned char*)p; key.insert(key.end(), b, b + bytes); };
    const int hdr[8] = {s.H, s.W, s.K, s.S, n, s.generic ? 1 : 0, (int)s.gen_step, s.sp_patch_uploaded ? 1 : 0};
    const void* const ptrs[9] = {s.h_cl, s.h_misc, s.d_ptrs, s.h_patch, s.d_gen, s.lsc_zero, s.d_patchf, s.h_clf, s.h_upd};
    put(hdr, sizeof hdr); put(ptrs, sizeof ptrs); put(&s.p, sizeof s.p); put(&s.f, sizeof s.f); put(&s.c, sizeof s.c);
    if (s.p.variant == FSLIC_VARIANT_LSC) put(&s.l, sizeof s.l);
    Slot::GraphEntry* ge = nullptr;
    for (auto& g : s.graphs) if (g.key == key) { ge = &g; break; }
    if (!ge) {
        if (s.graphs.size() >= 8) {
            if (s.graphs.front().exec) hipGraphExecDestroy(s.graphs.front().exec);
            if (s.graphs.front().graph) hipGraphDestroy(s.graphs.front().graph);
            s.graphs.erase(s.graphs.begin());
        }
        s.graphs.emplace_back();
        ge = &s.graphs.back();
        ge->key = key;
    }
    if (!ge->exec) {
        if (ge->failed || ge->seen++ == 0) return enqueue_frames(e, s, 0, n, s.generic, true);
        GraphRecorder rec;
        if (hipGraphCreate(&rec.graph, 0) != hipSuccess) { ge->failed = true; (void)hipGetLastError(); return enqueue_frames(e, s, 0, n, s.generic, true); }
        current_recorder() = &rec;
        const int rc = enqueue_frames(e, s, 0, n, s.generic, false);
        current_recorder() = nullptr;
        if (rc != FSLIC_OK || rec.err != hipSuccess || rec.nodes == 0 || hipGraphInstantiate(&ge->exec, rec.graph, nullptr, nullptr, 0) != hipSuccess) {
            hipGraphDestroy(rec.graph);
            ge->exec = nullptr; ge->failed = true;
            (void)hipGetLastError();
            if (rc != FSLIC_OK) return rc;
            return enqueue_frames(e, s, 0, n, s.generic, true);
        }
        ge->graph = rec.graph;
        s.last_launch_mode = 1;
    } else {
        s.last_launch_mode = 2;
    }
    HIPCHK(hipEventRecord(s.ev[0], s.st));
    HIPCHK(hipGraphLaunch(ge->exec, s.st));
    HIPCHK(hipEventRecord(s.ev[4], s.st));
    return FSLIC_OK;
}

int group_begin(fslic_engine* e, Slot& s, const GroupJob& job, bool record) {
    const double t_begin = now_us();
    const fslic_params* p = &job.p;
    const int H = job.H, W = job.W, K = job.K, n = job.n;
    int S = 0;
    s.recording = false;
    int rc = check_job(job, S);
    if (rc) return rc;
    if (record && n != 1) return fail(FSLIC_E_INTERNAL, "a recording group holds one frame");
    rc = ensure_prepared(e, s, H, W, K, S, n);
    if (rc) return rc;
    const int cap_frames = s.cap_frames;
    s.H = H; s.W = W; s.K = K; s.S = S; s.p = *p; s.nframes = n;
    std::copy(job.clusters, job.clusters + n, s.clusters);
    rc = configure_spatial(s, S, p);
    if (rc) return rc;
    if (p->variant == FSLIC_VARIANT_LSC) {
        rc = prepare_lsc(s, H, W, K, S, cap_frames, p->compactness);
        if (rc) return rc;
    }
    if (p->variant == FSLIC_VARIANT_REALDIST || p->variant == FSLIC_VARIANT_REALDIST_L2) {
        rc = configure_patchf(s, S, p);
        if (rc) return rc;
    }
    if (p->variant == FSLIC_VARIANT_REALDIST_NOQ && (rc = s.h_clf.reserve((size_t)s.cap_frames * K * 8))) return rc;
    rc = upload_ptrs(s, n, job.d_rgb, job.d_out);
    if (rc) return rc;
    if (record) {
        s.rec_clusters.assign(job.clusters[0], job.clusters[0] + K);
        s.recording = true;
        const size_t need = rec_layout(s).bytes;
        if (s.d_rec.reserve(need)) {
            (void)hipGetLastError();
            s.recording = false;
            return fail(FSLIC_E_HIP, "debug_mode: hipMalloc of the snapshot ring (" + std::to_string(need) + " bytes) failed");
        }
    }
    s.generic = p->variant == FSLIC_VARIANT_SLIC && (e->lab_force_generic.load() != 0 || !s.sp_tiled_ok || record);
    if (p->preemptive && (rc = s.h_upd.reserve((size_t)s.cap_frames * K))) return rc;
    stage_group(e, s, 0, n, true);
    rc = launch_group(e, s, n);
    if (rc) return rc;
    s.have_pre = true;
    s.last_path = s.generic ? 1 : 0;
    if (knobs().host_timing) {
        fprintf(stderr, "[fslic host] group_begin n=%d: %.1f us | slot %d begin %.1f .. %.1f\n", n, now_us() - t_begin, (int)(&s - e->slots.data()), t_begin, now_us());
        s.t_begun_us = now_us();
    }
    return FSLIC_OK;
}

static int nap_wait(Slot& s) {
    const double t0 = now_us();
    HIPCHK(hipEventRecord(s.ev[5], s.st));
    const unsigned long long key = ((unsigned long long)(uint32_t)s.H << 48) ^ ((unsigned long long)(uint32_t)s.W << 32) ^ ((unsigned long long)(uint32_t)s.K << 16) ^
                                   ((unsigned long long)(uint32_t)s.nframes << 8) ^ ((unsigned long long)(uint32_t)s.p.max_iter << 4) ^ (unsigned long long)(uint32_t)s.p.variant ^
                                   ((unsigned long long)(uint32_t)s.p.preemptive << 60) ^ ((unsigned long long)(uint32_t)s.p.subsample_stride << 56);
    if (key != s.recent_wait_key) {
        s.recent_wait_key = key;
        for (double& w : s.recent_wait_us) w = 1e30;
    }
    double shortest = 1e30;
    for (double w : s.recent_wait_us) shortest = std::min(shortest, w);
    auto nap = [](double us) { struct timespec ts; ts.tv_sec = 0; ts.tv_nsec = (long)(us * 1000.0); nanosleep(&ts, nullptr); };
    if (shortest < 1e29 && shortest * 0.5 > 30.0) nap(std::min(shortest * 0.5, 20000.0));
    for (;;) {
        const hipError_t q = hipEventQuery(s.ev[5]);
        if (q == hipSuccess) break;
        if (q != hipErrorNotReady) return fail(FSLIC_E_HIP, std::string("hipEventQuery: ") + hipGetErrorString(q));
        nap(10.0);
    }
    s.recent_wait_us[s.recent_wait_i++ & 3] = now_us() - t0;
    return FSLIC_OK;
}

int group_finish(fslic_engine* e, Slot& s) {
    const double t_begin = now_us();
    if (s.nap_wait) { const int rc = nap_wait(s); if (rc) return rc; }
    HIPCHK(hipStreamSynchronize(s.st));
    const double t_sync = now_us();
    const int n = s.nframes, K = s.K, H = s.H, W = s.W;
    auto elapsed = [](float& ms, hipEvent_t a, hipEvent_t b) { if (hipEventElapsedTime(&ms, a, b) != hipSuccess) { ms = 0; (void)hipGetLastError(); } };
    elapsed(s.total_ms, s.ev[0], s.ev[4]);
    if (s.last_launch_mode == 0) {
        elapsed(s.lab_ms, s.ev[0], s.ev[1]);
        elapsed(s.loop_ms, s.ev[1], s.ev[2]);
        elapsed(s.fa_ms, s.ev[2], s.ev[3]);
        elapsed(s.cca_ms, s.ev[3], s.ev[4]);
    } else {
        s.lab_ms = s.loop_ms = s.fa_ms = s.cca_ms = 0;
    }
    s.assign_loop_ms = 0;
    for (int it = 0; it < s.n_timed_iters; it++) {
        float ms = 0;
        elapsed(ms, s.ev_it[2 * it], s.ev_it[2 * it + 1]);
        s.assign_loop_ms += ms;
    }
    const int thres = min_size_threshold(s);
    const double t_ev = now_us();
    int n_host_topk = 0;
    for (int i = 0; i < n; i++) {
        const uint32_t* hm = status(s, i);
        n_host_topk += hm[kStSelect] == kSelectHost;
        for (int attempt = 0; attempt < 2 && !s.generic && hm[kStFlags] != 0; attempt++) {
            const bool overflow = (hm[kStFlags] & kFlagListOverflow) != 0;
            if (knobs().host_timing) fprintf(stderr, "[fslic host] frame %d redone with %s\n", i, overflow ? "the generic kernel (candidate-list overflow)" : "the separate cluster pass (stale pixel)");
            stage_group(e, s, i, 1, false);
            s.gen_step = s.gen_span_prev;
            s.gen_host += s.gen_step;
            int rc = enqueue_frames(e, s, i, 1, overflow, false, true);
            if (rc) return rc;
            HIPCHK(hipStreamSynchronize(s.st));
            if (overflow) {
                if (hm[kStFlags] != 0) return fail(FSLIC_E_INTERNAL, "generic path reported a candidate overflow");
                s.last_path = 1;
            } else {
                __atomic_fetch_add(&s.n_separate_redo, 1, __ATOMIC_RELAXED);
            }
        }
        if (!s.generic && hm[kStFlags] != 0) return fail(FSLIC_E_INTERNAL, "a redone frame still carries a kernel flag");
    }
    {
        int rc = cca_finish_group(s, 0, n, s.f.labels, s.frame_bytes, K, thres);
        if (rc) return rc;
    }
    s.n_host_topk = n_host_topk;
    const double t_cca = now_us();
    const bool noq = s.p.variant == FSLIC_VARIANT_REALDIST_NOQ;
    for (int i = 0; i < n; i++) {
        const uint32_t* yx = s.h_cl + (size_t)i * 4 * K;
        const uint32_t* lab = yx + K;
        const uint32_t* nm = yx + 2 * (size_t)K;
        const uint32_t* moved = yx + 3 * (size_t)K;
        fslic_cluster* cl = s.clusters[i];
        for (int k = 0; k < K; k++) {
            cl[k].r = (float)(lab[k] & 255u);
            cl[k].g = (float)((lab[k] >> 8) & 255u);
            cl[k].b = (float)((lab[k] >> 16) & 255u);
            const float* c = noq ? s.h_clf + ((size_t)i * K + k) * 8 : nullptr;
            if (moved[k] && c) { cl[k].r = c[2]; cl[k].g = c[3]; cl[k].b = c[4]; }
            cluster_position(moved[k] != 0, yx[k], c, cl[k], H, W, cl[k].y, cl[k].x);
            if (s.p.max_iter > 0) cl[k].num_members = nm[k];
            cl[k].is_updatable = s.p.preemptive ? (uint8_t)s.h_upd[(size_t)i * K + k] : 2;
            cl[k].is_active = 1;
        }
    }
    if (knobs().host_timing)
        fprintf(stderr, "[fslic host] group_finish n=%d slot %d at %.1f .. %.1f: sync wait %.1f us, events %.1f us, host top-K (%d frames) %.1f us, write-back %.1f us (device %.1f us)\n",
                n, (int)(&s - e->slots.data()), t_begin, now_us(), t_sync - t_begin, t_ev - t_sync, n_host_topk, t_cca - t_ev, now_us() - t_cca, s.total_ms * 1e3);
    return FSLIC_OK;
}

void drain_failed(Slot& s) {
    const std::string msg = last_error();
    (void)hipStreamSynchronize(s.st);
    (void)hipGetLastError();
    set_last_error(msg);
}

int run_group(fslic_engine* e, Slot& s, const GroupJob& job, bool record) {
    int rc = group_begin(e, s, job, record);
    if (rc == FSLIC_OK) rc = group_finish(e, s);
    if (rc != FSLIC_OK) drain_failed(s);
    return rc;
}

std::string make_timing_report(const Slot& s) {
    char buf[1024];
    auto us = [](float ms) { return (long long)(ms * 1000.0f); };
    snprintf(buf, sizeof buf,
             "{\"name\": \"iterate\", \"duration\": %lld, \"children\": ["
             "{\"name\": \"cielab_conversion\", \"duration\": %lld, \"children\": []},"
             "{\"name\": \"assign_update_loop\", \"duration\": %lld, \"children\": []},"
             "{\"name\": \"full_assign\", \"duration\": %lld, \"children\": []},"
             "{\"name\": \"enforce_connectivity\", \"duration\": %lld, \"children\": []}]}",
             us(s.total_ms), us(s.lab_ms), us(s.loop_ms), us(s.fa_ms), us(s.cca_ms));
    return buf;
}

namespace {
thread_local std::string t_timing;
thread_local std::string t_recorder;

inline char* put_u(char* o, uint64_t v) { return std::to_chars(o, o + 24, v).ptr; }
inline char* put_i(char* o, int64_t v) { return std::to_chars(o, o + 24, v).ptr; }
inline char* put_f(char* o, float v) { return std::to_chars(o, o + 32, (double)v, std::chars_format::general, 6).ptr; }
inline char* put_s(char* o, const char* s) { const size_t n = strlen(s); memcpy(o, s, n); return o + n; }
inline char* header(char* o, int H, int W) {
    o = put_s(o, "{\"height\": "); o = put_i(o, H);
    o = put_s(o, ", \"width\": "); o = put_i(o, W);
    return put_s(o, ", \"snapshots\": [");
}
}

void set_thread_timing_report(const std::string& json) { t_timing = json; }
const std::string& thread_timing_report() { return t_timing; }
void set_thread_recorder_report(std::string&& json) { t_recorder = std::move(json); }
const std::string& thread_recorder_report() { return t_recorder; }

int make_recorder_report(Slot& s, std::string& out) {
    const int H = s.H, W = s.W, K = s.K;
    if (!s.recording) {
        char buf[96];
        char* o = header(buf, H, W);
        o = put_s(o, "]}");
        out.assign(buf, o);
        return FSLIC_OK;
    }
    const RecLayout L = rec_layout(s);
    std::vector<char> ring(L.bytes);
    HIPCHK(hipMemcpyAsync(ring.data(), s.d_rec, L.bytes, hipMemcpyDeviceToHost, s.st));
    HIPCHK(hipStreamSynchronize(s.st));
    const bool pre = s.p.preemptive != 0, noq = s.p.variant == FSLIC_VARIANT_REALDIST_NOQ;
    const size_t per_dist = L.dsize == 2 ? 6 : 16;
    out.resize(96 + L.nsnap * (96 + L.K * 320 + L.N * (6 + per_dist)));
    char* const o0 = &out[0];
    char* o = header(o0, H, W);
    const fslic_cluster* const cin = s.rec_clusters.data();
    for (size_t i = 0; i < L.nsnap; i++) {
        if (i) *o++ = ',';
        o = put_s(o, "{\"iteration\": "); o = put_i(o, (int64_t)i - 1);
        o = put_s(o, ", \"clusters\": [");
        const uint32_t* c = reinterpret_cast<const uint32_t*>(ring.data() + L.cl_off) + i * kRecWords * L.K;
        for (int k = 0; k < K; k++) {
            const fslic_cluster& a = cin[k];
            const uint32_t lab = c[K + k];
            float y = a.y, x = a.x, r = (float)(lab & 255u), g = (float)((lab >> 8) & 255u), b = (float)((lab >> 16) & 255u);
            uint32_t upd = 2, act = a.is_active, nm = a.num_members;
            if (i > 0) {
                const bool moved = c[3 * (size_t)K + k] != 0;
                const float* cf = noq ? reinterpret_cast<const float*>(c + 6 * (size_t)K) + 8 * (size_t)k : nullptr;
                if (moved && cf) { r = cf[2]; g = cf[3]; b = cf[4]; }
                cluster_position(moved, c[k], cf, a, H, W, y, x);
                nm = c[2 * (size_t)K + k];
                if (pre) { upd = c[4 * (size_t)K + k]; act = c[5 * (size_t)K + k]; }
            }
            if (k) *o++ = ',';
            o = put_s(o, "{\"yx\": ["); o = put_f(o, y); *o++ = ','; o = put_f(o, x);
            o = put_s(o, "], \"color\": ["); o = put_f(o, r); *o++ = ','; o = put_f(o, g); *o++ = ','; o = put_f(o, b);
            o = put_s(o, "], \"is_updatable\": "); o = put_u(o, (uint8_t)upd);
            o = put_s(o, ", \"is_active\": "); o = put_u(o, (uint8_t)act);
            o = put_s(o, ", \"number\": "); o = put_u(o, a.number);
            o = put_s(o, ", \"num_members\": "); o = put_u(o, nm);
            *o++ = '}';
        }
        o = put_s(o, "], \"assignment\": [");
        const uint16_t* lb = reinterpret_cast<const uint16_t*>(ring.data()) + i * L.N;
        for (size_t q = 0; q < L.N; q++) {
            if (q) *o++ = ',';
            o = put_u(o, lb[q]);
        }
        o = put_s(o, "], \"min_dists\": [");
        if (L.dsize == 2) {
            const uint16_t* d = reinterpret_cast<const uint16_t*>(ring.data() + L.dist_off) + i * L.N;
            for (size_t q = 0; q < L.N; q++) {
                if (q) *o++ = ',';
                o = put_u(o, d[q]);
            }
        } else {
            const float* d = reinterpret_cast<const float*>(ring.data() + L.dist_off) + i * L.N;
            for (size_t q = 0; q < L.N; q++) {
                if (q) *o++ = ',';
                o = put_f(o, d[q]);
            }
        }
        o = put_s(o, "]}");
    }
    o = put_s(o, "]}");
    out.resize((size_t)(o - o0));
// ... 5 lines not shown
```

### fast_slic_amd/csrc/kernels.h

```cpp
#pragma once
#include <hip/hip_runtime.h>
#include <stdint.h>

#ifndef FSLIC_EXP
#define FSLIC_EXP 0
#endif

namespace fslic {

constexpr int kTileW = 64;
constexpr int kWavesPerBlock = 4;
constexpr int kRowsPerWave = 8;
constexpr int kCellCap = 8;
constexpr int kAccSlots = 16;
constexpr int kAccCopies = 8;
#ifndef FSLIC_BLK_COPIES
#define FSLIC_BLK_COPIES 4
#endif
constexpr int kBlkCopies = FSLIC_BLK_COPIES;
constexpr uint32_t kHuge = 0x40000000u;
constexpr int kCcaTile = 64;
constexpr int kCcaTileH = 32;
constexpr int kCcaTilePx = kCcaTile * kCcaTileH;
#ifndef FSLIC_MAX_GROUP
#define FSLIC_MAX_GROUP 16
#endif
constexpr int kMaxGroup = FSLIC_MAX_GROUP;

enum StatusWord {
    kStSpill0 = 0, kStSpill1 = 1,
    kStFlags = 2,
    kStSpill2 = 3,
    kStCca = 4,
    kStNodes = kStCca + 0,
    kStCands = kStCca + 1,
    kStCandsSeen = kStCca + 2,
    kStSelect = kStCca + 3
};
constexpr int kStatusWords = 16;
constexpr uint32_t kFlagListOverflow = 1u;
constexpr uint32_t kFlagStalePixel = 2u;
constexpr uint32_t kSelectDone = 0u;
constexpr uint32_t kSelectTie = 1u;
constexpr uint32_t kSelectHost = 2u;

struct ClusterRec {
    uint32_t yx, lab, tag, pad;
};

constexpr uint16_t kTabOut = 0x4000;

struct FrameDev {
    size_t frame_bytes;
    const uint8_t* const* rgbs;
    int H, W, N, K, S;
    int T;
    uint32_t T_rcp;
    int cs_shift;
    int ncx, ncy, ncell;
    uint32_t* gen_base;
    uint32_t gen_off;
    __device__ __forceinline__ uint32_t generation() const { return *gen_base + gen_off; }
    uint32_t M, C;
    const uint8_t* rgb;
    uint32_t* lab;
    uint16_t* labels;
    uint32_t* cl_yx;
    uint32_t* cl_yx_out;
    uint32_t* cl_lab;
    uint32_t* cl_tag;
    uint32_t* cl_n;
    uint32_t* cl_moved;
    uint32_t* cl_shadow;
    uint32_t* cl_upd;
    uint32_t* cl_act;
    uint32_t* cell_act;
    uint32_t* pre_flags;
    int pre_cw, pre_ch;
    float* cl_f;
    uint32_t* sums[2];
    uint32_t* cpart;
    int cpart_ns;
    int nbx;
    uint32_t* cell_cnt[2];
    ClusterRec* cell_items[2];
    uint32_t* ovf_cnt[3];
    ClusterRec* ovf_items[3];
    uint32_t* cl_arrive;
    uint32_t* err_flag;
    const uint32_t* lut;
    int lut_words, lut_row, lut_oow;
    const uint16_t* tab;
    int tab_words, tab_nrpad, tab_dyoff;
    int tab_vmode, tab_xout;
    const uint16_t* tabs;
    int tabs_words, tabs_dyoff, tabs_nrpad;
    const uint16_t* tabv16;
    int tabv16_words, tabv16_dyoff, tab_rows32;
    const uint16_t* tabs16;
    int tabs16_words, tabs16_dyoff, tabs16_nrpad;
    const uint16_t* patch2d;
#if defined(FSLIC_LAB) && FSLIC_LAB == 4
    uint32_t* lab_stamps;
#endif
    int fv_mod, fv_from;
    uint32_t fv_rcp;
    __device__ __forceinline__ bool first_visit(int y) const {
        if (fv_mod <= 1) return fv_mod == 1;
        uint32_t q = __umulhi((uint32_t)y, fv_rcp), rest = (uint32_t)y - q * (uint32_t)fv_mod;
        if (rest >= (uint32_t)fv_mod) rest -= (uint32_t)fv_mod;
        if (rest >= (uint32_t)fv_mod) rest -= (uint32_t)fv_mod;
        return (int)rest >= fv_from;
    }

    template <class T> static __host__ __device__ __forceinline__ void adv(T*& p, size_t d) {
        p = reinterpret_cast<T*>(const_cast<char*>(reinterpret_cast<const volatile char*>(p)) + d);
    }
    __host__ __device__ __forceinline__ void select(int z) {
        rgb = rgbs ? rgbs[z] : nullptr;
        const size_t d = (size_t)z * frame_bytes;
        adv(lab, d); adv(labels, d);
        adv(cl_yx, d); adv(cl_yx_out, d); adv(cl_lab, d); adv(cl_tag, d); adv(cl_n, d); adv(cl_moved, d); adv(cl_shadow, d);
        if (cl_f) adv(cl_f, d);
        if (cell_act) { adv(cl_upd, d); adv(cl_act, d); adv(cell_act, d); adv(pre_flags, d); }
        adv(sums[0], d); adv(sums[1], d); adv(cpart, d);
        adv(cell_cnt[0], d); adv(cell_cnt[1], d); adv(cell_items[0], d); adv(cell_items[1], d);
        adv(ovf_cnt[0], d); adv(ovf_cnt[1], d); adv(ovf_cnt[2], d); adv(ovf_items[0], d); adv(ovf_items[1], d); adv(ovf_items[2], d);
        adv(cl_arrive, d);
        adv(err_flag, d);
#if defined(FSLIC_LAB) && FSLIC_LAB == 4
        adv(lab_stamps, d);
#endif
    }
};

struct PassGeom {
    int rem, stride, Hv;
    int BH;
    int use_slots;
};
inline int visited_rows(int H, int rem, int stride) { return (H - rem + stride - 1) / stride; }
inline int assign_blocks8(int W, int Hv, int nframes) { return nframes * ((W + kTileW - 1) / kTileW) * ((Hv + kWavesPerBlock * 8 - 1) / (kWavesPerBlock * 8)); }

struct CcaDev {
    size_t frame_bytes;
    uint16_t* const* outs;
    size_t in_stride;
    int H, W, N, K;
    int min_threshold;
    const uint16_t* in;
    uint16_t* out;
    int tiles_x;
    uint16_t* lid;
    uint4* nrec;
    uint32_t* narea;
    uint16_t* nfinal;
    uint32_t* vedge;
    uint32_t* roots;
    uint32_t* counters;
    int32_t* cand_leader;
    uint32_t* cand_area;
    __host__ __device__ __forceinline__ void select(int z) {
        out = outs[z];
        FrameDev::adv(in, (size_t)z * in_stride);
        const size_t d = (size_t)z * frame_bytes;
        FrameDev::adv(lid, d); FrameDev::adv(nrec, d); FrameDev::adv(narea, d);
        FrameDev::adv(nfinal, d); FrameDev::adv(vedge, d); FrameDev::adv(roots, d);
        FrameDev::adv(counters, d);
        FrameDev::adv(cand_leader, d); FrameDev::adv(cand_area, d);
    }
};

constexpr int kLscFeat = 10;
constexpr int kLscCfPitch = 16;
constexpr int kLscExPitch = 12;
constexpr float kLscFixF = 1048576.0f, kLscFixW = 4096.0f;
struct LscDev {
    size_t frame_bytes;
    uint32_t* hist;
    float* means;
    float* cfeat;
    long long* extra;
    const float* lut_color;
    const float* lut_x;
    const float* lut_y;
    float blk_fix_f, blk_fix_w;
    int blk_shift_f, blk_shift_w;
    float blk_bias_w;
    __host__ __device__ __forceinline__ void select(int z) {
        const size_t d = (size_t)z * frame_bytes;
        FrameDev::adv(hist, d); FrameDev::adv(means, d);
        FrameDev::adv(cfeat, d); FrameDev::adv(extra, d);
    }
};

struct LabTables {
    const uint16_t* gamma;
    const uint16_t* labtbl;
    int cb[9];
};

void launch_rgb_to_lab(const FrameDev& f, int nframes, int convert, const LabTables& t, bool init_labels, hipStream_t st, uint32_t gen_step = 0,
                       void* zero_a = nullptr, size_t zero_a_bytes = 0, uint32_t* zero_b = nullptr, size_t zero_b_words = 0,
                       const uint32_t* stage_yx = nullptr, size_t stage_stride = 0);
void launch_bin_clusters(const FrameDev& f, int nframes, int mode, int buf, int sbuf, const PassGeom& pg, hipStream_t st,
                         const uint32_t* src_yx = nullptr, size_t src_stride = 0);
void launch_bin_clusters_lsc(const FrameDev& f, const LscDev& l, int nframes, int buf, int sbuf, hipStream_t st);

bool blk_kernel_applies(const FrameDev& f, int stride);
PassGeom launch_assign(const FrameDev& f, int nframes, int rem, int stride, int buf, int sbuf, bool fuse_update, hipStream_t st, int obuf = -1);
void launch_assign_fused_bin(const FrameDev& f, int nframes, int rem, int stride, int it, hipStream_t st);
void launch_assign_generic(const FrameDev& f, int nframes, int rem, int stride, int buf, int sbuf, bool fuse_update, hipStream_t st,
                           uint16_t* rec_dist = nullptr);
bool launch_assign_pre(const FrameDev& f, int nframes, int rem, int stride, int buf, int sbuf, hipStream_t st);
void launch_lsc_prepare(const FrameDev& f, const LscDev& l, int nframes, hipStream_t st);
void launch_lsc_assign(const FrameDev& f, const LscDev& l, int nframes, int rem, int stride, int buf, int sbuf, bool stale_sums, hipStream_t st,
                       float* rec_dist = nullptr);
void launch_lsc_pre_sums(const FrameDev& f, int nframes, int rem, int stride, int sbuf, hipStream_t st);
void launch_lsc_pre_feats(const FrameDev& f, const LscDev& l, int nframes, int rem, int stride, hipStream_t st);
void launch_rd_assign(const FrameDev& f, const float* patchf, bool l2, int nframes, int rem, int stride, int buf, int sbuf, bool stale_sums, hipStream_t st,
                      float* rec_dist = nullptr);
void launch_member_sums(const FrameDev& f, int nframes, int rem, int stride, int sbuf, int margin, hipStream_t st);
void launch_noq_assign(const FrameDev& f, float coef, bool manhattan, int nframes, int rem, int stride, int buf, int sbuf, bool stale_sums, hipStream_t st,
                       float* rec_dist = nullptr);
void launch_preempt_update(const FrameDev& f, int nframes, int buf, int sbuf, bool rebin_all, float l1_thres, hipStream_t st);
void launch_cca_phase1(const CcaDev& c, int nframes, hipStream_t st);
void launch_cca_select(const CcaDev& c, int nframes, hipStream_t st);
struct ExportDev {
    size_t frame_bytes;
    int K;
    const uint32_t* yx_cur;
    const uint32_t* lab_n_moved;
    const uint32_t* misc0;
    uint32_t* h_cl;
    size_t h_stride;
    uint32_t* h_misc;
};
void launch_cca_phase2(const CcaDev& c, int nframes, hipStream_t st, const ExportDev* ex = nullptr);
void launch_cca_gather_area(const CcaDev& c, hipStream_t st);
void launch_cca_set_kept(const CcaDev& c, const int32_t* d_leaders, const uint16_t* d_labels, int n, hipStream_t st);

void launch_mask_sums(const uint16_t* labels, const uint8_t* mask, uint32_t* sums, int H, int W, int K, hipStream_t st);
void launch_density_to_mask(const uint16_t* labels, const uint8_t* dens, uint8_t* out, size_t N, int K, hipStream_t st);
void launch_adjacent_pairs(const uint16_t* labels, int H, int W, int K, uint32_t* tab_pair, unsigned long long* tab_key,
                           uint32_t cap, uint32_t* counters, hipStream_t st);

void launch_copy16(const void* src, void* dst, size_t bytes, hipStream_t st);

}
```

### include/fslic_hip.h

```cpp
#ifndef FSLIC_HIP_H
#define FSLIC_HIP_H

#include <stddef.h>
#include <stdint.h>

#ifdef __cplusplus
extern "C" {
#endif

#define FSLIC_HIP_ARCH_NAME "hip/gfx950"

enum {
    FSLIC_OK = 0,
    FSLIC_E_INVALID = 1,
    FSLIC_E_UNSUPPORTED = 2,
    FSLIC_E_HIP = 3,
    FSLIC_E_INTERNAL = 4
};

typedef struct fslic_cluster {
    float y, x, r, g, b, a;
    uint16_t number;
    uint8_t is_active;
    uint8_t is_updatable;
    uint32_t num_members;
} fslic_cluster;

typedef struct fslic_params {
    int32_t max_iter;
    float compactness;
    float min_size_factor;
    int32_t subsample_stride;
    int32_t convert_to_lab;
    int32_t manhattan_spatial_dist;
    int32_t preemptive;
    float preemptive_thres;
    int32_t num_threads;
    int32_t debug_mode;
    int32_t abi;
    int32_t variant;
    int32_t reserved[4];
} fslic_params;
#define FSLIC_PARAMS_ABI 0x46533033

enum {
    FSLIC_VARIANT_SLIC = 0,
    FSLIC_VARIANT_LSC = 1,
    FSLIC_VARIANT_REALDIST = 2,
    FSLIC_VARIANT_REALDIST_L2 = 3,
    FSLIC_VARIANT_REALDIST_NOQ = 4
};

typedef struct fslic_engine fslic_engine;

int fslic_hip_device_count(void);

int fslic_hip_create(int device, int n_slots, fslic_engine** out);
void fslic_hip_destroy(fslic_engine* e);

int fslic_hip_initialize_clusters(int H, int W, int K, const uint8_t* rgb, fslic_cluster* clusters);

int fslic_hip_iterate(fslic_engine* e, const fslic_params* p, int H, int W, int K,
                      const uint8_t* rgb, fslic_cluster* clusters, uint16_t* labels);

int fslic_hip_iterate_device(fslic_engine* e, int slot, const fslic_params* p, int H, int W, int K,
                             const uint8_t* d_rgb, fslic_cluster* clusters, uint16_t* d_labels);

int fslic_hip_iterate_batch(fslic_engine* e, const fslic_params* p, int H, int W, int K, int n_frames,
                            const uint8_t* const* rgb, fslic_cluster* const* clusters,
                            uint16_t* const* labels, int device_ptrs);

int fslic_hip_submit_group(fslic_engine* e, int slot, const fslic_params* p, int H, int W, int K, int n_frames,
                           const uint8_t* const* d_rgb, fslic_cluster* const* clusters, uint16_t* const* d_labels);
int fslic_hip_wait_group(fslic_engine* e, int slot);
int fslic_hip_group_done(fslic_engine* e, int slot);

int fslic_hip_pipeline_submit(fslic_engine* e, const fslic_params* p, int H, int W, int K, int n_frames,
                              const uint8_t* const* d_rgb, fslic_cluster* const* clusters, uint16_t* const* d_labels);
int fslic_hip_pipeline_drain(fslic_engine* e, double* device_ms, long long* groups, long long* frames,
                             long long* host_topk_frames);
int fslic_hip_pipeline_batching(fslic_engine* e, int max_frames_per_group);


int fslic_hip_rgb_to_lab(fslic_engine* e, int H, int W, const uint8_t* rgb, int convert, uint8_t* lab4);

int fslic_hip_enforce_connectivity(fslic_engine* e, uint16_t* labels, int H, int W, int K, int min_threshold);
int fslic_hip_enforce_connectivity_nodes(fslic_engine* e, uint16_t* labels, int H, int W, int K, int min_threshold, uint32_t* n_nodes);


int fslic_hip_get_connectivity(fslic_engine* e, int H, int W, int K, const uint16_t* labels,
                               int* num_neighbors, uint32_t* neighbors);

int fslic_hip_knn_connectivity(int H, int W, int K, const fslic_cluster* clusters, size_t n_neighbors,
                               int* num_neighbors, uint32_t* neighbors);

int fslic_hip_get_mask_density(fslic_engine* e, int H, int W, int K, const fslic_cluster* clusters,
                               const uint16_t* labels, const uint8_t* mask, uint8_t* densities);

int fslic_hip_cluster_density_to_mask(fslic_engine* e, int H, int W, int K, const uint16_t* labels,
                                      const uint8_t* densities, uint8_t* result);

int fslic_hip_last_prelabels(fslic_engine* e, int slot, uint16_t* prelabels);

const char* fslic_hip_last_timing_report(fslic_engine* e);

int fslic_hip_last_recorder_report(fslic_engine* e, const char** report, size_t* length);

int fslic_hip_last_device_times(fslic_engine* e, int slot, float* total_ms, float* full_assign_ms);

int fslic_hip_set_launch_timing(fslic_engine* e, int on);
int fslic_hip_last_assign_loop(fslic_engine* e, int slot, float* sum_ms, double* visited_px, int* launches);

int fslic_hip_last_group_frames(fslic_engine* e, int slot);

int fslic_hip_last_launch_mode(fslic_engine* e, int slot);

int fslic_hip_last_path(fslic_engine* e, int slot);

int fslic_hip_last_host_topk_frames(fslic_engine* e, int slot);

int fslic_hip_separate_pass_redos(fslic_engine* e, int slot);

int fslic_hip_copy_bandwidth(fslic_engine* e, size_t bytes, int reps, double* gb_per_s);

typedef struct fslic_crf fslic_crf;
typedef struct fslic_crf_frame fslic_crf_frame;
typedef struct fslic_crf_params {
    float spatial_w, temporal_w, spatial_srgb, temporal_srgb, spatial_sxy, spatial_smooth_w, spatial_smooth_sxy;
} fslic_crf_params;

int fslic_hip_crf_new(size_t num_classes, size_t num_nodes, fslic_crf** out);
void fslic_hip_crf_free(fslic_crf* crf);
int fslic_hip_crf_copy(fslic_crf* crf, fslic_crf** out);
int fslic_hip_crf_get_params(fslic_crf* crf, fslic_crf_params* out);
int fslic_hip_crf_set_params(fslic_crf* crf, const fslic_crf_params* params);
int fslic_hip_crf_set_compat(fslic_crf* crf, int cls, float compat_value);
int fslic_hip_crf_get_compat(fslic_crf* crf, int cls, float* out);
int fslic_hip_crf_num_classes(fslic_crf* crf, size_t* num_classes, size_t* num_nodes);
int fslic_hip_crf_first_time(fslic_crf* crf);
int fslic_hip_crf_last_time(fslic_crf* crf);
size_t fslic_hip_crf_num_frames(fslic_crf* crf);
int fslic_hip_crf_pop_frame(fslic_crf* crf);
int fslic_hip_crf_push_frame(fslic_crf* crf, fslic_crf_frame** out);
int fslic_hip_crf_frame(fslic_crf* crf, int time, fslic_crf_frame** out);
int fslic_hip_crf_frame_time(fslic_crf_frame* frame);
int fslic_hip_crf_frame_set_clusters(fslic_crf_frame* frame, const fslic_cluster* clusters);
int fslic_hip_crf_frame_get_clusters(fslic_crf_frame* frame, fslic_cluster* clusters);
int fslic_hip_crf_frame_set_connectivity(fslic_crf_frame* frame, int num_rows, const int* num_neighbors, const uint32_t* neighbors,
                                         size_t stride);
int fslic_hip_crf_frame_set_connectivity_csr(fslic_crf_frame* frame, int num_rows, const int64_t* offsets, const uint32_t* indices);
int fslic_hip_crf_frame_get_connectivity(fslic_crf_frame* frame, int64_t* offsets, uint32_t* indices);
int fslic_hip_crf_frame_set_mask(fslic_crf_frame* frame, const int32_t* classes, float confidence);
int fslic_hip_crf_frame_set_proba(fslic_crf_frame* frame, const float* probas);
int fslic_hip_crf_frame_set_unbiased(fslic_crf_frame* frame);
int fslic_hip_crf_frame_set_unary(fslic_crf_frame* frame, const float* unary_energies);
int fslic_hip_crf_frame_get_unary(fslic_crf_frame* frame, float* unary_energies);
int fslic_hip_crf_frame_spatial_energy(fslic_crf_frame* frame, int node_i, int node_j, float* out);
int fslic_hip_crf_frame_temporal_energy(fslic_crf_frame* frame, fslic_crf_frame* other_frame, int node_i, float* out);
int fslic_hip_crf_frame_get_inferred(fslic_crf_frame* frame, float* probas);
int fslic_hip_crf_frame_reset_inferred(fslic_crf_frame* frame);
int fslic_hip_crf_initialize(fslic_crf* crf);
int fslic_hip_crf_inference(fslic_crf* crf, fslic_engine* e, size_t max_iter);
int fslic_hip_crf_expf_host(const float* in, float* out, size_t n, int use_libm);
int fslic_hip_crf_expf_device(fslic_engine* e, const float* in, float* out, size_t n);

enum { FSLIC_POOL_SUM = 0, FSLIC_POOL_MEAN = 1, FSLIC_POOL_MAX = 2 };
enum { FSLIC_LABEL_U16 = 0 , FSLIC_LABEL_I32 = 1, FSLIC_LABEL_I64 = 2 };
int fslic_hip_pool_workspace_size(int N, int C, int K, int reduce, size_t* bytes);
int fslic_hip_pool(int device, void* stream, int N, int C, int H, int W, int K, int reduce, const float* features,
                   const void* labels, int label_type, void* workspace, size_t workspace_bytes);
int fslic_hip_pool_finalize(int device, void* stream, int N, int C, int K, int reduce, const void* workspace, size_t workspace_bytes,
                            float* values, int32_t* counts, int32_t* argmax);
int fslic_hip_unpool(int device, void* stream, int N, int C, int H, int W, int K, const float* values, const void* labels,
                     int label_type, const int32_t* argmax, float fill, float* out);

int fslic_hip_rag_workspace_size(int N, int K, int C, long long capacity, size_t* bytes);
int fslic_hip_rag_accumulate(int device, void* stream, int N, int H, int W, int K, int connectivity, const void* labels, int label_type,
                             const uint8_t* image, int C, long long capacity, void* workspace, size_t workspace_bytes);
int fslic_hip_rag_compact(int device, void* stream, int N, int C, long long capacity, void* workspace, size_t workspace_bytes,
                          int64_t* keys, int32_t* boundary, int64_t* contrast, long long max_edges);

int fslic_hip_crf_tensor_workspace_size(int N, int C, int K, long long nnz, size_t* bytes);
int fslic_hip_crf_tensor_inference(int device, void* stream, int N, int C, int K, int temporal, int max_iter,
                                   const fslic_crf_params* params, const float* compat, const float* yxrgb, const int32_t* members,
                                   const int64_t* offsets, const int32_t* indices, long long nnz,
                                   const float* unaries, const float* q0 , float* q_out,
                                   void* workspace, size_t workspace_bytes);

int fslic_hip_crf_tensor_grad_workspace_size(int N, int C, int K, long long nnz, int backward, int with_compat, size_t* bytes);
int fslic_hip_crf_tensor_inference_saved(int device, void* stream, int N, int C, int K, int temporal, int max_iter,
                                         const fslic_crf_params* params, const float* compat, const float* yxrgb, const int32_t* members,
                                         const int64_t* offsets, const int32_t* indices, long long nnz,
                                         const float* unaries, const float* q0 , float* q_all,
                                         void* workspace, size_t workspace_bytes);
int fslic_hip_crf_tensor_backward(int device, void* stream, int N, int C, int K, int temporal, int max_iter,
                                  const fslic_crf_params* params, const float* compat, const float* yxrgb, const int32_t* members,
                                  const int64_t* offsets, const int32_t* indices, long long nnz,
                                  const int64_t* t_offsets, const int32_t* t_entries, const int32_t* t_rows,
                                  const float* unaries, const float* q_all, const float* grad_q,
                                  float* grad_unaries, float* grad_q0, float* grad_compat, void* workspace, size_t workspace_bytes);

const char* fslic_hip_last_error(void);
const char* fslic_hip_version(void);

#ifdef __cplusplus
}
#endif
#endif
```

Before: 65560 megapixels/sec.

## Skip label stores in fused assign iterations, with uncovered-pixel redo fallback

Adds a label-free mode for the fused assign-and-sum passes: they skip writing per-pixel labels and the s_klab table, since the final full assign pass rewrites every label anyway. The final pass unconditionally writes 0xFFFF for any pixel with no candidate and raises a new uncovered-pixel flag. When the flag is seen, the frame is redone with label-storing passes, and the slot stays in storing mode for matching shapes and params. This removes a large share of label write traffic per iteration. In exchange it adds a redo path, extra kernel instantiations and a new graph-cache key field.

Result: faster. 69300 megapixels/sec, median of 6 (+5.7%).

```diff
diff --git a/fast_slic_amd/_binding.py b/fast_slic_amd/_binding.py
--- a/fast_slic_amd/_binding.py
+++ b/fast_slic_amd/_binding.py
@@ -36,7 +36,7 @@
     "fslic_hip_last_device_times", "fslic_hip_set_launch_timing", "fslic_hip_last_assign_loop", "fslic_hip_last_group_frames", "fslic_hip_last_path", "fslic_hip_last_launch_mode", "fslic_hip_group_done", "fslic_hip_last_error", "fslic_hip_version",
     "fslic_hip_get_connectivity", "fslic_hip_knn_connectivity", "fslic_hip_get_mask_density", "fslic_hip_cluster_density_to_mask",
     "fslic_hip_pipeline_submit", "fslic_hip_pipeline_drain", "fslic_hip_pipeline_batching", "fslic_hip_last_host_topk_frames",
-    "fslic_hip_separate_pass_redos", "fslic_hip_copy_bandwidth", "fslic_hip_last_recorder_report",
+    "fslic_hip_separate_pass_redos", "fslic_hip_uncovered_redos", "fslic_hip_copy_bandwidth", "fslic_hip_last_recorder_report",
     "fslic_hip_crf_new", "fslic_hip_crf_free", "fslic_hip_crf_copy", "fslic_hip_crf_get_params", "fslic_hip_crf_set_params",
     "fslic_hip_crf_set_compat", "fslic_hip_crf_get_compat", "fslic_hip_crf_num_classes", "fslic_hip_crf_first_time",
     "fslic_hip_crf_last_time", "fslic_hip_crf_num_frames", "fslic_hip_crf_pop_frame", "fslic_hip_crf_push_frame", "fslic_hip_crf_frame",
@@ -111,6 +111,8 @@
         lib.fslic_hip_pipeline_batching.argtypes = [vp, i32]
         lib.fslic_hip_last_host_topk_frames.argtypes = [vp, i32]
         lib.fslic_hip_separate_pass_redos.argtypes = [vp, i32]
+        if hasattr(lib, "fslic_hip_uncovered_redos"):
+            lib.fslic_hip_uncovered_redos.argtypes = [vp, i32]
         if hasattr(lib, "fslic_hip_copy_bandwidth"):
             lib.fslic_hip_copy_bandwidth.argtypes = [vp, C.c_size_t, i32, C.POINTER(C.c_double)]
         lib.fslic_hip_group_done.argtypes = [vp, i32]
@@ -350,6 +352,13 @@
     def separate_pass_redos(self):
         return sum(int(load_library().fslic_hip_separate_pass_redos(self._h, s)) for s in range(self.n_slots))
 
+    def uncovered_redos(self, slot=None):
+        lib = load_library()
+        if not hasattr(lib, "fslic_hip_uncovered_redos"):
+            return 0
+        slots = range(self.n_slots) if slot is None else [int(slot)]
+        return sum(int(lib.fslic_hip_uncovered_redos(self._h, s)) for s in slots)
+
     def copy_bandwidth(self, nbytes=1 << 30, reps=5):
         v = C.c_double()
         _check(load_library().fslic_hip_copy_bandwidth(self._h, C.c_size_t(int(nbytes)), int(reps), C.byref(v)))
diff --git a/fast_slic_amd/csrc/assign.hip b/fast_slic_amd/csrc/assign.hip
--- a/fast_slic_amd/csrc/assign.hip
+++ b/fast_slic_amd/csrc/assign.hip
@@ -422,17 +422,19 @@
 static inline BlkMap blk_map(dim3 g) { BlkMap m; m.gx = g.x; m.gy = g.y; return m; }
 static inline dim3 blk_grid(dim3 g) { return dim3(g.x, g.z, g.y); }
 
-template <int R, bool FUSE, int STRIDE, bool VT, bool FBIN = false, bool PRE = false>
+template <int R, bool FUSE, int STRIDE, bool VT, bool FBIN = false, bool PRE = false, bool NOLAB = false>
 static __device__ __forceinline__ void assign_blk2_body(FrameDev& f, int rem, int Hv, const BlkMap& bm) {
     static_assert(!FBIN || FUSE, "the cluster pass rides on the fused centroid sums");
     static_assert(!PRE || (FUSE && !FBIN), "preemptive mode: the fused pass with its own flush");
+    static_assert(!NOLAB || (!FBIN && !PRE), "label-free groups: the separate cluster pass only");
+    constexpr bool NOSTORE = NOLAB && FUSE, CLOSING = NOLAB && !FUSE;
     const uint32_t bxi = blockIdx.x, byi = blockIdx.z, bzi = blockIdx.y;
     extern __shared__ __attribute__((aligned(16))) uint32_t s_dyn[];
     __shared__ __attribute__((aligned(16))) uint4 s_raw[kWavesPerBlock][64];
     __shared__ __attribute__((aligned(16))) uint32_t s_part[64][4];
     __shared__ __attribute__((aligned(16))) uint32_t s_wcnt[4];
     __shared__ __attribute__((aligned(16))) uint32_t s_entry[FUSE ? 64 : 4];
-    __shared__ __attribute__((aligned(16))) uint16_t s_klab[64];
+    __shared__ __attribute__((aligned(16))) uint16_t s_klab[NOSTORE ? 2 : 64];
     __shared__ __attribute__((aligned(16))) unsigned long long s_acc[FUSE ? 64 * kBlkCopies * 2 : 2];
     static_assert(R % 2 == 0, "rows are processed in pairs");
     constexpr int BH = kWavesPerBlock * R;
@@ -566,11 +568,11 @@
         bn = c0 + c1 + c2 + c3;
         if (bn > 64) {
             if (tid == 0) atomicOr(f.err_flag, kFlagListOverflow);
-            if constexpr (!FBIN) {
+            if constexpr (!FBIN && !NOSTORE) {
                 if (okx) {
                     uint16_t* rowp = f.labels + (size_t)yw_lo * W + (uint32_t)x;
                     for (int r = 0; r < nrows; ++r, rowp += (size_t)STRIDE * W)
-                        if (FUSE ? f.fv_mod == 1 : f.first_visit(yw_lo + r * STRIDE)) st_stream(rowp, (uint16_t)0xFFFFu);
+                        if (CLOSING || (FUSE ? f.fv_mod == 1 : f.first_visit(yw_lo + r * STRIDE))) st_stream(rowp, (uint16_t)0xFFFFu);
                 }
             }
             return;
@@ -592,7 +594,7 @@
         const uint4 pr = *reinterpret_cast<const uint4*>(s_part[lane]);
         rank_j = pr.x + pr.y + pr.z + pr.w;
     }
-    if (lane < bn) s_klab[(int)rank_j] = (uint16_t)(mine.z & 0xFFFFu);
+    if constexpr (!NOSTORE) { if (lane < bn) s_klab[(int)rank_j] = (uint16_t)(mine.z & 0xFFFFu); }
     uint32_t fin_nx = 0, fin_ny = 0, fin_b0 = 0;
     if (PRE && wave == 0) {
         if (lane < bn) s_entry[rank_j] = mine.z & 0xFFFFu;
@@ -862,19 +864,21 @@
             ASG_MARK("labels");
             epilogue_done = true;
             if (okx) {
-                uint32_t kk[R];
-                const char* const ktab = reinterpret_cast<const char*>(s_klab);
-#pragma unroll
-                for (int q = 0; q < R / 2; ++q) {
-                    const uint32_t b = __builtin_bit_cast(uint32_t, best[q]) & 0x003F003Fu;
-                    kk[2 * q] = *reinterpret_cast<const uint16_t*>(ktab + ((b & 0xFFu) << 1));
-                    kk[2 * q + 1] = *reinterpret_cast<const uint16_t*>(ktab + (((b >> 16) & 0xFFu) << 1));
-                }
-                const __amdgpu_buffer_rsrc_t ws = __builtin_amdgcn_make_buffer_rsrc(f.labels, 0, (int)((uint32_t)f.N * 2u), kRawBuffer);
-                const uint32_t so0 = (uint32_t)yw_lo * (uint32_t)W * 2u, pitch2 = (uint32_t)(STRIDE * W) * 2u;
-#pragma unroll
-                for (int r = 0; r < R; ++r)
-                    __builtin_amdgcn_raw_buffer_store_b16((uint16_t)kk[r], ws, (int)((uint32_t)x * 2u), (int)(so0 + (uint32_t)r * pitch2), kAuxSc1);
+                if constexpr (!NOSTORE) {
+                    uint32_t kk[R];
+                    const char* const ktab = reinterpret_cast<const char*>(s_klab);
+#pragma unroll
+                    for (int q = 0; q < R / 2; ++q) {
+                        const uint32_t b = __builtin_bit_cast(uint32_t, best[q]) & 0x003F003Fu;
+                        kk[2 * q] = *reinterpret_cast<const uint16_t*>(ktab + ((b & 0xFFu) << 1));
+                        kk[2 * q + 1] = *reinterpret_cast<const uint16_t*>(ktab + (((b >> 16) & 0xFFu) << 1));
+                    }
+                    const __amdgpu_buffer_rsrc_t ws = __builtin_amdgcn_make_buffer_rsrc(f.labels, 0, (int)((uint32_t)f.N * 2u), kRawBuffer);
+                    const uint32_t so0 = (uint32_t)yw_lo * (uint32_t)W * 2u, pitch2 = (uint32_t)(STRIDE * W) * 2u;
+#pragma unroll
+                    for (int r = 0; r < R; ++r)
+                        __builtin_amdgcn_raw_buffer_store_b16((uint16_t)kk[r], ws, (int)((uint32_t)x * 2u), (int)(so0 + (uint32_t)r * pitch2), kAuxSc1);
+                }
                 ASG_STAMP(5, wave == 0);
                 ASG_MARK("sums");
                 if (FUSE) {
@@ -931,15 +935,24 @@
         uint32_t slot[R];
         uint16_t* rowp = f.labels + (size_t)yw_lo * W;
         const uint32_t xo = (uint32_t)x;
+        [[maybe_unused]] bool uncovered = false;
 #pragma unroll
         for (int r = 0; r < R; ++r) {
             const bool ok = okx && r < nrows;
             const uint32_t key = (r & 1) ? (uint32_t)best[r / 2].y : (uint32_t)best[r / 2].x;
             const bool found = key != 0xFFFFu;
             slot[r] = kNoSlot;
+            if constexpr (NOSTORE) {
+                if (ok && found) slot[r] = key & 63u;
+                uncovered = uncovered || (ok && !found);
+                continue;
+            }
             if (ok && found) st_stream(rowp + xo, s_klab[key & 63u]);
-            const bool unlabelled = !FBIN && ok && !found && (FUSE ? f.fv_mod == 1 : f.first_visit(yw_lo + r * STRIDE));
-            if (unlabelled) st_stream(rowp + xo, (uint16_t)0xFFFFu);
+            const bool unlabelled = !FBIN && ok && !found && (CLOSING || (FUSE ? f.fv_mod == 1 : f.first_visit(yw_lo + r * STRIDE)));
+            if (unlabelled) {
+                st_stream(rowp + xo, (uint16_t)0xFFFFu);
+                if constexpr (CLOSING) atomicOr(f.err_flag, kFlagUncoveredPixel);
+            }
             bool summed = FUSE && ok && !unlabelled;
             if constexpr (PRE) summed = summed && in_update(f, yw_lo + r * STRIDE, x);
             if (summed) {
@@ -953,6 +966,9 @@
                 }
             }
             rowp += (size_t)STRIDE * W;
+        }
+        if constexpr (NOSTORE) {
+            if (ballot(uncovered) != 0ull && lane == 0) atomicOr(f.err_flag, kFlagUncoveredPixel);
         }
         ASG_STAMP(5, wave == 0);
         if (FUSE) {
@@ -1020,17 +1036,17 @@
     ASG_STAMP(8, wave == 0);
 }
 
-template <int R, bool FUSE, int STRIDE, bool VT>
+template <int R, bool FUSE, int STRIDE, bool VT, bool NOLAB = false>
 __global__ __launch_bounds__(256) __attribute__((amdgpu_num_sgpr(80), amdgpu_waves_per_eu(7, 8))) void k_assign_blk2(FrameDev f, int rem, int Hv, BlkMap bm) {
-    assign_blk2_body<R, FUSE, STRIDE, VT>(f, rem, Hv, bm);
-}
-template <int R, bool FUSE, int STRIDE, bool VT>
+    assign_blk2_body<R, FUSE, STRIDE, VT, false, false, NOLAB>(f, rem, Hv, bm);
+}
+template <int R, bool FUSE, int STRIDE, bool VT, bool NOLAB = false>
 __global__ __launch_bounds__(256) __attribute__((amdgpu_num_sgpr(80), amdgpu_waves_per_eu(8, 8))) void k_assign_blk2_w8(FrameDev f, int rem, int Hv, BlkMap bm) {
-    assign_blk2_body<R, FUSE, STRIDE, VT>(f, rem, Hv, bm);
-}
-template <int R, bool FUSE, int STRIDE, bool VT>
+    assign_blk2_body<R, FUSE, STRIDE, VT, false, false, NOLAB>(f, rem, Hv, bm);
+}
+template <int R, bool FUSE, int STRIDE, bool VT, bool NOLAB = false>
 __global__ __launch_bounds__(256) __attribute__((amdgpu_num_sgpr(80), amdgpu_waves_per_eu(6, 8))) void k_assign_blk2_w6(FrameDev f, int rem, int Hv, BlkMap bm) {
-    assign_blk2_body<R, FUSE, STRIDE, VT>(f, rem, Hv, bm);
+    assign_blk2_body<R, FUSE, STRIDE, VT, false, false, NOLAB>(f, rem, Hv, bm);
 }
 
 template <int R, int STRIDE, bool VT>
@@ -1052,7 +1068,7 @@
     return f;
 }
 
-template <int R, bool FUSE, int STRIDE>
+template <int R, bool FUSE, int STRIDE, bool NOLAB = false>
 static void launch_assign_blk_t(const FrameDev& f_, int nframes, int rem, int Hv, hipStream_t st) {
     FrameDev f = FUSE ? with_subsampled_table(f_) : f_;
     if (FUSE && R == 16 && !f.tab_vmode) { f.tab = f.tabs16; f.tab_words = f.tabs16_words; f.tab_dyoff = f.tabs16_dyoff; f.tab_nrpad = f.tabs16_nrpad; }
@@ -1061,16 +1077,16 @@
     const size_t lds2 = ((size_t)f.tab_words * sizeof(uint32_t) + 1023) / 1024 * 1024;
     if constexpr (R == 32) {
         static_assert(!FUSE, "32 rows per wavefront: full pass only");
-        launch((k_assign_blk2_w6<R, FUSE, STRIDE, true>), blk_grid(grid), dim3(256), lds2, st, f, rem, Hv, blk_map(grid));
+        launch((k_assign_blk2_w6<R, FUSE, STRIDE, true, NOLAB>), blk_grid(grid), dim3(256), lds2, st, f, rem, Hv, blk_map(grid));
     } else if constexpr (R == 16 && !FUSE) {
-        if (f.tab_vmode) launch((k_assign_blk2_w8<R, FUSE, STRIDE, true>), blk_grid(grid), dim3(256), lds2, st, f, rem, Hv, blk_map(grid));
-        else launch((k_assign_blk2_w8<R, FUSE, STRIDE, false>), blk_grid(grid), dim3(256), lds2, st, f, rem, Hv, blk_map(grid));
+        if (f.tab_vmode) launch((k_assign_blk2_w8<R, FUSE, STRIDE, true, NOLAB>), blk_grid(grid), dim3(256), lds2, st, f, rem, Hv, blk_map(grid));
+        else launch((k_assign_blk2_w8<R, FUSE, STRIDE, false, NOLAB>), blk_grid(grid), dim3(256), lds2, st, f, rem, Hv, blk_map(grid));
     } else if constexpr (R == 16 && FUSE) {
-        if (f.tab_vmode) launch((k_assign_blk2_w6<R, FUSE, STRIDE, true>), blk_grid(grid), dim3(256), lds2, st, f, rem, Hv, blk_map(grid));
-        else launch((k_assign_blk2_w6<R, FUSE, STRIDE, false>), blk_grid(grid), dim3(256), lds2, st, f, rem, Hv, blk_map(grid));
+        if (f.tab_vmode) launch((k_assign_blk2_w6<R, FUSE, STRIDE, true, NOLAB>), blk_grid(grid), dim3(256), lds2, st, f, rem, Hv, blk_map(grid));
+        else launch((k_assign_blk2_w6<R, FUSE, STRIDE, false, NOLAB>), blk_grid(grid), dim3(256), lds2, st, f, rem, Hv, blk_map(grid));
     } else {
-        if (f.tab_vmode) launch((k_assign_blk2<R, FUSE, STRIDE, true>), blk_grid(grid), dim3(256), lds2, st, f, rem, Hv, blk_map(grid));
-        else launch((k_assign_blk2<R, FUSE, STRIDE, false>), blk_grid(grid), dim3(256), lds2, st, f, rem, Hv, blk_map(grid));
+        if (f.tab_vmode) launch((k_assign_blk2<R, FUSE, STRIDE, true, NOLAB>), blk_grid(grid), dim3(256), lds2, st, f, rem, Hv, blk_map(grid));
+        else launch((k_assign_blk2<R, FUSE, STRIDE, false, NOLAB>), blk_grid(grid), dim3(256), lds2, st, f, rem, Hv, blk_map(grid));
     }
 }
 
@@ -1151,7 +1167,20 @@
     }
 }
 
-PassGeom launch_assign(const FrameDev& f_, int nframes, int rem, int stride, int buf, int sbuf, bool fuse_update, hipStream_t st, int obuf) {
+template <int R>
+static void launch_assign_fused_t(const FrameDev& f, int nframes, int rem, int stride, int Hv, bool label_free, hipStream_t st) {
+    if (label_free) {
+        if (stride == 1) launch_assign_blk_t<R, true, 1, true>(f, nframes, rem, Hv, st);
+        else if (stride == 2) launch_assign_blk_t<R, true, 2, true>(f, nframes, rem, Hv, st);
+        else launch_assign_blk_t<R, true, 3, true>(f, nframes, rem, Hv, st);
+    } else {
+        if (stride == 1) launch_assign_blk_t<R, true, 1>(f, nframes, rem, Hv, st);
+        else if (stride == 2) launch_assign_blk_t<R, true, 2>(f, nframes, rem, Hv, st);
+        else launch_assign_blk_t<R, true, 3>(f, nframes, rem, Hv, st);
+    }
+}
+
+PassGeom launch_assign(const FrameDev& f_, int nframes, int rem, int stride, int buf, int sbuf, bool fuse_update, hipStream_t st, int obuf, bool label_free) {
     const FrameDev f = rotated(f_, buf, sbuf, obuf);
     const int Hv = visited_rows(f.H, rem, stride);
     PassGeom pg;
@@ -1160,6 +1189,12 @@
     if (blk_kernel_applies(f, stride)) {
         if (!fuse_update && stride == 1) {
             const int rpw = assign_rows_per_wave(f, nframes, Hv, false);
+            if (label_free) {
+                if (rpw == 32) launch_assign_blk_t<32, false, 1, true>(f, nframes, rem, Hv, st);
+                else if (rpw == 16) launch_assign_blk_t<16, false, 1, true>(f, nframes, rem, Hv, st);
+                else launch_assign_blk_t<8, false, 1, true>(f, nframes, rem, Hv, st);
+                return pg;
+            }
             if (rpw == 32) launch_assign_blk_t<32, false, 1>(f, nframes, rem, Hv, st);
             else if (rpw == 16) launch_assign_blk_t<16, false, 1>(f, nframes, rem, Hv, st);
             else launch_assign_blk_t<8, false, 1>(f, nframes, rem, Hv, st);
@@ -1171,14 +1206,10 @@
             const bool r16 = (f.tab_vmode && fblocks8 > 3072) || (!f.tab_vmode && f.tabs16_words > 0 && fblocks8 > 2048);
             if (r16) {
                 pg.BH = kWavesPerBlock * 16;
-                if (stride == 1) launch_assign_blk_t<16, true, 1>(f, nframes, rem, Hv, st);
-                else if (stride == 2) launch_assign_blk_t<16, true, 2>(f, nframes, rem, Hv, st);
-                else launch_assign_blk_t<16, true, 3>(f, nframes, rem, Hv, st);
+                launch_assign_fused_t<16>(f, nframes, rem, stride, Hv, label_free, st);
                 return pg;
             }
-            if (stride == 1) launch_assign_blk_t<8, true, 1>(f, nframes, rem, Hv, st);
-            else if (stride == 2) launch_assign_blk_t<8, true, 2>(f, nframes, rem, Hv, st);
-            else launch_assign_blk_t<8, true, 3>(f, nframes, rem, Hv, st);
+            launch_assign_fused_t<8>(f, nframes, rem, stride, Hv, label_free, st);
             return pg;
         }
     }
diff --git a/fast_slic_amd/csrc/capi.cpp b/fast_slic_amd/csrc/capi.cpp
--- a/fast_slic_amd/csrc/capi.cpp
+++ b/fast_slic_amd/csrc/capi.cpp
@@ -276,6 +276,11 @@
     return __atomic_load_n(&e->slots[slot].n_separate_redo, __ATOMIC_RELAXED);
 }
 
+int fslic_hip_uncovered_redos(fslic_engine* e, int slot) {
+    if (!e || slot < 0 || slot >= (int)e->slots.size()) return -1;
+    return __atomic_load_n(&e->slots[slot].n_uncovered_redo, __ATOMIC_RELAXED);
+}
+
 #define CRF_LOCK(crf) std::lock_guard<std::mutex> crf_lock__((crf)->mu)
 
 static fslic_crf_frame* crf_frame_at(fslic_crf* crf, int time) {
diff --git a/fast_slic_amd/csrc/engine_internal.h b/fast_slic_amd/csrc/engine_internal.h
--- a/fast_slic_amd/csrc/engine_internal.h
+++ b/fast_slic_amd/csrc/engine_internal.h
@@ -157,6 +157,11 @@
     int last_path = 0;
     int n_host_topk = 0;
     int n_separate_redo = 0;
+    int n_uncovered_redo = 0;
+    bool store_labels = false;
+    bool store_seen_credit = false;
+    int store_H = 0, store_W = 0, store_K = 0;
+    fslic_params store_p{};
     bool have_pre = false;
     bool busy = false;
     bool pending = false;
diff --git a/fast_slic_amd/csrc/group.cpp b/fast_slic_amd/csrc/group.cpp
--- a/fast_slic_amd/csrc/group.cpp
+++ b/fast_slic_amd/csrc/group.cpp
@@ -191,6 +191,8 @@
     return fuse_wanted && !separate_cluster_pass && plain_slic && !generic && every_pass_has_rows && blk_kernel_applies(f, stride);
 }
 
+static bool label_free_allowed(const Slot& s) { return !s.store_labels; }
+
 static int min_size_threshold(const Slot& s) { return (int)round((double)(s.S * s.S) * (double)s.p.min_size_factor); }
 
 constexpr int kRecWords = 16;
@@ -208,7 +210,7 @@
     return L;
 }
 
-int enqueue_frames(fslic_engine* e, Slot& s, int i0, int n, bool generic, bool timed, bool separate_cluster_pass = false) {
+int enqueue_frames(fslic_engine* e, Slot& s, int i0, int n, bool generic, bool timed, bool separate_cluster_pass = false, bool store_labels = false) {
     const fslic_params* p = &s.p;
     const int K = s.K, S = s.S;
     FrameDev f = s.f;
@@ -244,6 +246,7 @@
     f.gen_base = s.d_gen;
     const bool fusebin = cluster_pass_fused(f, *p, n, s.W, s.H, generic, separate_cluster_pass);
     const bool lazy_labels = p->variant == FSLIC_VARIANT_SLIC && !generic && p->preemptive == 0 && !fusebin;
+    const bool label_free = lazy_labels && !store_labels && label_free_allowed(s) && p->max_iter >= 1 && !s.recording && blk_kernel_applies(f, p->subsample_stride);
     launch_rgb_to_lab(f, n, p->convert_to_lab, e->tables, !lazy_labels, s.st, s.gen_step,
                       s.at(s.zero_block, i0), s.zero_bytes, f.cl_n, 2 * (size_t)K, s.h_cl + (size_t)i0 * 4 * K, 4 * (size_t)K);
     if (timed) HIPCHK(hipEventRecord(s.ev[1], s.st));
@@ -356,7 +359,7 @@
         f.fv_mod = lazy_labels && it < stride ? 1 : 0; f.fv_from = 0;
         if (rec) launch_assign_generic(f, n, rem, stride, it & 1, it & 1, true, s.st, static_cast<uint16_t*>(rec_dist(it + 1)));
         else if (generic || (pre && !launch_assign_pre(f, n, rem, stride, it & 1, it & 1, s.st))) launch_assign_generic(f, n, rem, stride, it & 1, it & 1, true, s.st);
-        else if (!pre) pg = launch_assign(f, n, rem, stride, it & 1, it & 1, true, s.st);
+        else if (!pre) pg = launch_assign(f, n, rem, stride, it & 1, it & 1, true, s.st, -1, label_free);
         if (tme) HIPCHK(hipEventRecord(s.ev_it[2 * it + 1], s.st));
         f.gen_off++;
         f.cl_yx = yx_cur; f.cl_yx_out = (yx_cur == yx_a) ? yx_b : yx_a;
@@ -375,12 +378,13 @@
     }
     if (timed) HIPCHK(hipEventRecord(s.ev[2], s.st));
     f.fv_mod = lazy_labels && p->max_iter < stride ? stride : 0; f.fv_from = p->max_iter < stride ? std::max(p->max_iter, 0) : 0;
+    if (label_free) { f.fv_mod = 1; f.fv_from = 0; }
     f.fv_rcp = f.fv_mod > 1 ? 0xFFFFFFFFu / (uint32_t)f.fv_mod : 0u;
     if (lsc) { f.cl_yx = yx_cur; launch_lsc_assign(f, l, n, 0, 1, full_buf, 0, false, s.st); }
     else if (noq) { f.cl_yx = yx_cur; launch_noq_assign(f, noq_coef, noq_manhattan, n, 0, 1, full_buf, 0, false, s.st); }
     else if (rd) { f.cl_yx = yx_cur; launch_rd_assign(f, s.d_patchf, rd_l2, n, 0, 1, full_buf, 0, false, s.st); }
     else if (generic) launch_assign_generic(f, n, 0, 1, full_buf, 0, false, s.st);
-    else (void)launch_assign(f, n, 0, 1, full_buf, 0, false, s.st, full_obuf);
+    else (void)launch_assign(f, n, 0, 1, full_buf, 0, false, s.st, full_obuf, label_free);
     if (timed) HIPCHK(hipEventRecord(s.ev[3], s.st));
     const CcaDev c = cca_view(s, i0, s.f.labels, fb, K, min_size_threshold(s));
     ExportDev ex{};
@@ -417,7 +421,7 @@
     if (!knobs().use_graphs || s.launch_timing) return enqueue_frames(e, s, 0, n, s.generic, true);
     std::vector<unsigned char> key;
     auto put = [&](const void* p, size_t bytes) { const unsigned char* b = (const unsigned char*)p; key.insert(key.end(), b, b + bytes); };
-    const int hdr[8] = {s.H, s.W, s.K, s.S, n, s.generic ? 1 : 0, (int)s.gen_step, s.sp_patch_uploaded ? 1 : 0};
+    const int hdr[9] = {s.H, s.W, s.K, s.S, n, s.generic ? 1 : 0, (int)s.gen_step, s.sp_patch_uploaded ? 1 : 0, label_free_allowed(s) ? 1 : 0};
     const void* const ptrs[9] = {s.h_cl, s.h_misc, s.d_ptrs, s.h_patch, s.d_gen, s.lsc_zero, s.d_patchf, s.h_clf, s.h_upd};
     put(hdr, sizeof hdr); put(ptrs, sizeof ptrs); put(&s.p, sizeof s.p); put(&s.f, sizeof s.f); put(&s.c, sizeof s.c);
     if (s.p.variant == FSLIC_VARIANT_LSC) put(&s.l, sizeof s.l);
@@ -432,6 +436,8 @@
         s.graphs.emplace_back();
         ge = &s.graphs.back();
         ge->key = key;
+        if (s.store_seen_credit && s.store_labels) ge->seen = 1;
+        s.store_seen_credit = false;
     }
     if (!ge->exec) {
         if (ge->failed || ge->seen++ == 0) return enqueue_frames(e, s, 0, n, s.generic, true);
@@ -471,6 +477,7 @@
     if (rc) return rc;
     const int cap_frames = s.cap_frames;
     s.H = H; s.W = W; s.K = K; s.S = S; s.p = *p; s.nframes = n;
+    if (s.store_labels && !(H == s.store_H && W == s.store_W && K == s.store_K && memcmp(&s.store_p, p, sizeof(fslic_params)) == 0)) { s.store_labels = false; s.store_seen_credit = false; }
     std::copy(job.clusters, job.clusters + n, s.clusters);
     rc = configure_spatial(s, S, p);
     if (rc) return rc;
@@ -563,17 +570,23 @@
         n_host_topk += hm[kStSelect] == kSelectHost;
         for (int attempt = 0; attempt < 2 && !s.generic && hm[kStFlags] != 0; attempt++) {
             const bool overflow = (hm[kStFlags] & kFlagListOverflow) != 0;
-            if (knobs().host_timing) fprintf(stderr, "[fslic host] frame %d redone with %s\n", i, overflow ? "the generic kernel (candidate-list overflow)" : "the separate cluster pass (stale pixel)");
+            const bool uncovered = (hm[kStFlags] & kFlagUncoveredPixel) != 0;
+            if (uncovered) {
+                if (!s.store_labels) s.store_seen_credit = true;
+                s.store_labels = true; s.store_H = H; s.store_W = W; s.store_K = K; s.store_p = s.p;
+                __atomic_fetch_add(&s.n_uncovered_redo, 1, __ATOMIC_RELAXED);
+            }
+            if (knobs().host_timing) fprintf(stderr, "[fslic host] frame %d redone with %s\n", i, overflow ? "the generic kernel (candidate-list overflow)" : uncovered ? "storing assign passes (uncovered pixel)" : "the separate cluster pass (stale pixel)");
             stage_group(e, s, i, 1, false);
             s.gen_step = s.gen_span_prev;
             s.gen_host += s.gen_step;
-            int rc = enqueue_frames(e, s, i, 1, overflow, false, true);
+            int rc = enqueue_frames(e, s, i, 1, overflow, false, true, true);
             if (rc) return rc;
             HIPCHK(hipStreamSynchronize(s.st));
             if (overflow) {
                 if (hm[kStFlags] != 0) return fail(FSLIC_E_INTERNAL, "generic path reported a candidate overflow");
                 s.last_path = 1;
-            } else {
+            } else if (!uncovered) {
                 __atomic_fetch_add(&s.n_separate_redo, 1, __ATOMIC_RELAXED);
             }
         }
diff --git a/fast_slic_amd/csrc/kernels.h b/fast_slic_amd/csrc/kernels.h
--- a/fast_slic_amd/csrc/kernels.h
+++ b/fast_slic_amd/csrc/kernels.h
@@ -40,6 +40,7 @@
 constexpr int kStatusWords = 16;
 constexpr uint32_t kFlagListOverflow = 1u;
 constexpr uint32_t kFlagStalePixel = 2u;
+constexpr uint32_t kFlagUncoveredPixel = 4u;
 constexpr uint32_t kSelectDone = 0u;
 constexpr uint32_t kSelectTie = 1u;
 constexpr uint32_t kSelectHost = 2u;
@@ -208,7 +209,8 @@
 void launch_bin_clusters_lsc(const FrameDev& f, const LscDev& l, int nframes, int buf, int sbuf, hipStream_t st);
 
 bool blk_kernel_applies(const FrameDev& f, int stride);
-PassGeom launch_assign(const FrameDev& f, int nframes, int rem, int stride, int buf, int sbuf, bool fuse_update, hipStream_t st, int obuf = -1);
+PassGeom launch_assign(const FrameDev& f, int nframes, int rem, int stride, int buf, int sbuf, bool fuse_update, hipStream_t st, int obuf = -1,
+                       bool label_free = false);
 void launch_assign_fused_bin(const FrameDev& f, int nframes, int rem, int stride, int it, hipStream_t st);
 void launch_assign_generic(const FrameDev& f, int nframes, int rem, int stride, int buf, int sbuf, bool fuse_update, hipStream_t st,
                            uint16_t* rec_dist = nullptr);
diff --git a/include/fslic_hip.h b/include/fslic_hip.h
--- a/include/fslic_hip.h
+++ b/include/fslic_hip.h
@@ -120,6 +120,8 @@
 int fslic_hip_last_host_topk_frames(fslic_engine* e, int slot);
 
 int fslic_hip_separate_pass_redos(fslic_engine* e, int slot);
+
+int fslic_hip_uncovered_redos(fslic_engine* e, int slot);
 
 int fslic_hip_copy_bandwidth(fslic_engine* e, size_t bytes, int reps, double* gb_per_s);
 
```
